# antoyang/TubeDETR

Hardware: AMD Instinct MI355X
Metric: training clips/sec (fwd+bwd) at T=100 k=4 res=352, 1/2/4/8 MI355X (higher is better)
Workload: dtype bf16

## Files before the change

include/tubedetr_hip.h:

```cpp
#ifndef TUBEDETR_HIP_H
#define TUBEDETR_HIP_H
#include <stddef.h>
#include <stdint.h>
#ifdef __cplusplus
extern "C" {
#endif

#define TD_F32 0
#define TD_BF16 1
#define TD_U8 2
#define TD_OK 0
#define TD_ERR_INVALID (-1)
#define TD_ERR_LAUNCH (-2)

typedef void* td_stream_t;

const char* td_last_error(void);
int td_abi_version(void);

int td_set_deterministic(int on);
int td_get_deterministic(void);


#define TD_PROF_GEMM_128x128 0
#define TD_PROF_GEMM_128x64 1
#define TD_PROF_WGRAD 2
#define TD_PROF_GEMM_64x128 3
#define TD_PROF_PW_RESIDENT 4
#define TD_PROF_GEMM_256 5
#define TD_PROF_GEMM_256_PW 6
#define TD_PROF_FUSED 7
#define TD_PROF_CROSS_Q1 8
#define TD_PROF_WGRAD_SINGLE 9
#define TD_PROF_CHAIN 10
#define TD_PROF_FAMILIES 11
int td_prof_enable(int on);
int td_prof_collect(int family, int dtype, long long* launches, double* ms, double* flops);
int td_prof_collect_bytes(int family, int dtype, double* bytes);
int td_prof_dump(const char* path);
int td_debug_set_stamp_buffer(unsigned long long* buf);

typedef struct td_conv_desc {
  int N, Hs, Ws, C;
  int Ho, Wo;
  int R, S, stride, pad;
  int mode;
  int Nc;
  int ldc;
  int out_sp;
  int out_H, out_W;
  int aniso;
  int stride_w, pad_w;
} td_conv_desc;

typedef struct td_epilogue {
  const float* bias;
  const void* residual;
  const void* mask_src;
  int relu;
  int sigmoid;
  float dropout_p;
  uint32_t dropout_seed;
  float alpha;
  const uint32_t* dropout_counter;
} td_epilogue;

int td_conv_gemm(const void* src, const void* wmat, void* out, const td_conv_desc* d, const td_epilogue* e,
                 int dtype, td_stream_t stream);

typedef struct td_linear_ex_desc {
  int M, N, K1, K2;
  int lda1, lda2, ldc, ldr;
  int w_shared;
  long long rows1, rows2;
  const int* a1_map;
  const int* a2_map;
  const int* out_map;
  const int* res_map;
} td_linear_ex_desc;
int td_linear_ex(const void* a1, const void* a2, const void* wmat, void* out, const td_linear_ex_desc* x, const td_epilogue* e,
                 int dtype, td_stream_t stream);

int td_conv_wgrad(const void* g, const void* src, float* dw, const td_conv_desc* d, int ldg, int dtype, int splits,
                  td_stream_t stream);
int td_conv_wgrad_bias(const void* g, const void* src, float* dw, float* dbias, const td_conv_desc* d, int ldg, int dtype,
                       int splits, td_stream_t stream);

typedef struct td_wgrad_job {
  const void* g;
  const void* src;
  float* dW;
  const float* scale;
  td_conv_desc d;
  int ldg;
  int ci_real;
  float* dbias;
  int accumulate;
  int prezeroed;
} td_wgrad_job;
size_t td_conv_wgrad_batch_table_bytes(int n_jobs);
int td_conv_wgrad_batch(const td_wgrad_job* jobs, int n_jobs, int dtype, void* table_host, void* table_dev, size_t table_bytes,
                        td_stream_t stream);

typedef struct td_frame_source {
  const void* data;
  int dtype;
  int n;
  const int* index;
  const int* valid_hw;
} td_frame_source;
int td_frames_to_nhwc(const td_frame_source* srcs, int n_srcs, int C, int H, int W, int Cpad, const float* mean,
                      const float* inv_std, void* y, int dtype, td_stream_t stream);

size_t td_resnet_fwd_ws_bytes(int N, int H, int W, const int* nblocks, int dtype, int save);
int td_resnet_num_convs(const int* nblocks);
int td_resnet_fwd(const td_frame_source* srcs, int n_srcs, const float* mean, const float* inv_std, int N, int H, int W,
                  const int* nblocks, const void* const* w_fwd, const float* const* bias, int save, void* ws, size_t ws_bytes,
                  void** feat, int* feat_hw, int stem_pairs, int first_train_stage, int dtype, td_stream_t stream);
int td_bottleneck_fused(const void* x, void* out, const void* w1, const float* b1, const void* w2, const float* b2, const void* w3,
                        const float* b3, const void* wd, const float* bd, int N, int H, int W, int Cin, int dtype, td_stream_t stream);
int td_pw_chain2(const void* y2, const void* w3, const float* b3, const void* residual, void* out, const void* w1, const float* b1,
                 void* h1, int M, int planes, int dtype, td_stream_t stream);
int td_stem_pair_weights(const void* w_fwd_8, void* w_pairs, int Co, int dtype, td_stream_t stream);
int td_stem_pool(const void* x_pairs, const void* w_pairs, const float* bias, void* pooled, int N, int H, int W, int dtype,
                 td_stream_t stream);
size_t td_resnet_bwd_ws_bytes(int N, int H, int W, const int* nblocks, int first_train_stage, int dtype);
size_t td_resnet_bwd_table_bytes(const int* nblocks, int first_train_stage);
int td_resnet_bwd(const void* dfeat, int N, int N_fwd, int H, int W, const int* nblocks, int first_train_stage,
                  const void* const* w_dgrad, const float* const* scale, float* const* dW, const void* fwd_ws, void* ws,
                  size_t ws_bytes, void* table_host, void* table_dev, size_t table_bytes, int dW_prezeroed, int dtype, int only_stage, td_stream_t stream);

int td_weight_prep(const float* W, const float* bn_w, const float* bn_b, const float* bn_rm, const float* bn_rv,
                   const float* bias, int Co, int Ci, int R, int S, int Cpad, void* w_fwd, void* w_dgrad,
                   float* bias_out, float* scale_out, int dtype, td_stream_t stream);

typedef struct td_prep_item {
  const float* W;
  const float *bn_w, *bn_b, *bn_rm, *bn_rv, *bias;
  void *w_fwd, *w_dgrad;
  float *bias_out, *scale_out;
  int Co, Ci, RS, Cpad, Co_alloc, blk0;
} td_prep_item;
int td_weight_prep_batch(const td_prep_item* items_dev, int n, int total_blocks, int dtype, td_stream_t stream);

int td_wgrad_finalize(const float* dw_k, const float* scale, float* dW, int Co, int Ci, int R, int S, int Cpad,
                      int accumulate, td_stream_t stream);

int td_nchw_to_nhwc(const float* x, void* y, int N, int C, int H, int W, int Cpad, int dtype, td_stream_t stream);
int td_nhwc_to_nchw(const void* x, float* y, int N, int C, int H, int W, int dtype, td_stream_t stream);
int td_cast(const void* x, void* y, size_t n, int src_dtype, int dst_dtype, td_stream_t stream);

int td_maxpool3x3s2(const void* x, void* y, int N, int H, int W, int C, int dtype, td_stream_t stream);

int td_add_layernorm_fwd(const void* x, const void* r, const float* gamma, const float* beta, void* y, void* s_out,
                         float* mean, float* rstd, int rows, int cols, float eps, int dtype, td_stream_t stream);
int td_add_layernorm_bwd(const void* dy, const void* s, const float* mean, const float* rstd, const float* gamma,
                         const void* extra, void* ds, float* dgamma, float* dbeta, int rows, int cols, int dtype,
                         td_stream_t stream);

int td_colsum(const void* g, float* out, int rows, int cols, int ld, int dtype, td_stream_t stream);
int td_add(const void* a, const void* b, void* y, size_t n, int dtype, td_stream_t stream);

int td_relu_bwd(const void* dy, const void* y, void* g, size_t n, float scale, int dtype, td_stream_t stream);

int td_gelu_fwd(const void* x, void* y, size_t n, int dtype, td_stream_t stream);
int td_gelu_bwd(const void* dy, const void* x, void* dx, size_t n, int dtype, td_stream_t stream);

int td_dropout(const void* x, void* y, size_t n, float p, uint32_t seed, const uint32_t* dropout_counter, int dtype,
               td_stream_t stream);

int td_pos_sine(const uint8_t* mask, void* pos, int N, int h, int w, int npf, float temperature, int rows_per_image, int dtype,
                td_stream_t stream);

int td_rows_copy(const void* src, const int* src_map, const void* add, void* dst, const int* dst_map, int n_rows, int cols, int ld_src,
                 int ld_add, int ld_dst, int dtype, td_stream_t stream);
int td_rows_segment_sum(const void* in, const int* idx, const int* ptr, void* out, const int* out_map, int n_out, int cols, int ld_in,
                        int ld_out, int dtype, td_stream_t stream);

int td_mha_fwd(const void* q, const void* k, const void* v, const uint8_t* key_pad, void* out, float* probs,
               float* wavg, int B, int H, int Lq, int Lk, int hd, int ldq, int ldk, int ldv, int ldo, float scale,
               float dropout_p, uint32_t dropout_seed, const uint32_t* dropout_counter, int dtype, td_stream_t stream);
int td_mha_bwd(const void* q, const void* k, const void* v, const void* dout, const float* probs, const float* dwavg,
               void* dq, void* dk, void* dv, float* ds_ws, int B, int H, int Lq, int Lk, int hd, int ldq, int ldk,
               int ldv, int ldo, float scale, float dropout_p, uint32_t dropout_seed, const uint32_t* dropout_counter,
               int dtype, td_stream_t stream);

int td_cross_q1_fwd(const void* u, const void* mem, const void* pos, const uint8_t* key_pad, float* probs, float* wavg, void* zext,
                    int F, int S, int H, int E, int ldz, float dropout_p, uint32_t dropout_seed, const uint32_t* dropout_counter,
                    int dtype, td_stream_t stream);
int td_cross_q1_bwd(const void* u, const void* mem, const void* pos, const float* probs, const void* d_zext, const float* dwavg,
                    void* d_u, float* d_mem, int accumulate, int F, int S, int H, int E, int ldz, float dropout_p, uint32_t dropout_seed,
                    const uint32_t* dropout_counter, int dtype, td_stream_t stream);
int td_cross_q1_bwd_coef(const void* u, const void* mem, const void* pos, const float* probs, const void* d_zext, const float* dwavg,
                         void* d_u, void* coef, int coef_ld, int coef_col, int F, int S, int H, int E, int ldz, float dropout_p,
                         uint32_t dropout_seed, const uint32_t* dropout_counter, int dtype, td_stream_t stream);
int td_cross_q1_dmem(const void* coef, int coef_ld, const void* const* u, const void* const* d_zext, int n_layers, void* d_mem, int F, int S,
                     int H, int E, int ldz, int dtype, td_stream_t stream);
int td_head_blocks_expand(const float* W, const float* bias, float alpha, void* w_n, void* w_t, int E, int H, int dtype, td_stream_t stream);
int td_head_blocks_extract(const float* G, float alpha, float* dW, float* db, int E, int H, td_stream_t stream);

size_t td_mha_lean_stats_bytes(int B, int H, int Lq);
int td_mha_lean_fwd(const void* q, const void* k, const void* v, const uint8_t* key_pad, void* out, float* stats, int B, int H,
                    int Lq, int Lk, int hd, int ldq, int ldk, int ldv, int ldo, float scale, float dropout_p,
                    uint32_t dropout_seed, const uint32_t* dropout_counter, int dtype, td_stream_t stream);
int td_mha_lean_bwd(const void* q, const void* k, const void* v, const uint8_t* key_pad, const void* out, const void* dout,
                    float* stats, void* dq, void* dk, void* dv, int B, int H, int Lq, int Lk, int hd, int ldq, int ldk, int ldv,
                    int ldo, float scale, float dropout_p, uint32_t dropout_seed, const uint32_t* dropout_counter, int dtype,
                    td_stream_t stream);


// ... 47 lines not shown
```

tubedetr_amd/_hip.py:

```python
from __future__ import annotations

import ctypes as C
import os

import torch

TD_F32, TD_BF16 = 0, 1
EXPECTED_ABI = 11
_LIB_PATH = os.environ.get("TD_HIP_LIB") or os.path.join(os.path.dirname(os.path.abspath(__file__)), "lib", "libtubedetr_hip.so")
_lib = None


class ConvDesc(C.Structure):
    _fields_ = [(n, C.c_int) for n in ("N", "Hs", "Ws", "C", "Ho", "Wo", "R", "S", "stride", "pad", "mode", "Nc", "ldc", "out_sp", "out_H", "out_W",
                                       "aniso", "stride_w", "pad_w")]


class PrepItem(C.Structure):
    _fields_ = [(n, C.c_void_p) for n in ("W", "bn_w", "bn_b", "bn_rm", "bn_rv", "bias", "w_fwd", "w_dgrad", "bias_out", "scale_out")] + \
               [(n, C.c_int) for n in ("Co", "Ci", "RS", "Cpad", "Co_alloc", "blk0")]


class WgradJob(C.Structure):
    _fields_ = [("g", C.c_void_p), ("src", C.c_void_p), ("dW", C.c_void_p), ("scale", C.c_void_p), ("d", ConvDesc), ("ldg", C.c_int), ("ci_real", C.c_int), ("dbias", C.c_void_p), ("accumulate", C.c_int), ("prezeroed", C.c_int)]


TD_U8 = 2


class FrameSource(C.Structure):
    _fields_ = [("data", C.c_void_p), ("dtype", C.c_int), ("n", C.c_int), ("index", C.c_void_p), ("valid_hw", C.c_void_p)]


class LinearExDesc(C.Structure):
    _fields_ = [(n, C.c_int) for n in ("M", "N", "K1", "K2", "lda1", "lda2", "ldc", "ldr", "w_shared")] + \
               [("rows1", C.c_longlong), ("rows2", C.c_longlong)] + [(n, C.c_void_p) for n in ("a1_map", "a2_map", "out_map", "res_map")]


class OptimSegment(C.Structure):
    _fields_ = [("begin", C.c_longlong), ("end", C.c_longlong), ("group", C.c_int), ("active", C.c_int)]


class ResampleJob(C.Structure):
    _fields_ = [("src", C.c_void_p), ("src_frame_stride", C.c_longlong)] + [(n, C.c_int) for n in ("src_pitch", "T", "sh", "sw", "flip", "rh", "rw", "wy", "wx", "wh", "ww")] + \
               [("dst", C.c_void_p)] + [(n, C.c_int) for n in ("planar", "frame_off", "H", "W")] + [("mask", C.c_void_p)]


class Epilogue(C.Structure):
    _fields_ = [
        ("bias", C.c_void_p),
        ("residual", C.c_void_p),
        ("mask_src", C.c_void_p),
        ("relu", C.c_int),
        ("sigmoid", C.c_int),
        ("dropout_p", C.c_float),
        ("dropout_seed", C.c_uint32),
        ("alpha", C.c_float),
        ("dropout_counter", C.c_void_p),
    ]


_P, _I, _F, _U32, _SZ = C.c_void_p, C.c_int, C.c_float, C.c_uint32, C.c_size_t
_SIGS = {
    "td_prof_enable": [_I],
    "td_prof_dump": [C.c_char_p],
    "td_debug_set_stamp_buffer": [_P],
    "td_prof_collect": [_I, _I, C.POINTER(C.c_longlong), C.POINTER(C.c_double), C.POINTER(C.c_double)],
    "td_prof_collect_bytes": [_I, _I, C.POINTER(C.c_double)],
    "td_conv_gemm": [_P, _P, _P, C.POINTER(ConvDesc), C.POINTER(Epilogue), _I, _P],
    "td_conv_wgrad": [_P, _P, _P, C.POINTER(ConvDesc), _I, _I, _I, _P],
    "td_conv_wgrad_bias": [_P, _P, _P, _P, C.POINTER(ConvDesc), _I, _I, _I, _P],
    "td_conv_wgrad_batch": [C.POINTER(WgradJob), _I, _I, _P, _P, _SZ, _P],
    "td_resnet_num_convs": [C.POINTER(C.c_int)],
    "td_resnet_fwd": [C.POINTER(FrameSource), _I, C.POINTER(C.c_float), C.POINTER(C.c_float), _I, _I, _I, C.POINTER(C.c_int), C.POINTER(_P), C.POINTER(_P), _I, _P, _SZ,
                      C.POINTER(_P), C.POINTER(C.c_int), _I, _I, _I, _P],
    "td_bottleneck_fused": [_P, _P, _P, _P, _P, _P, _P, _P, _P, _P, _I, _I, _I, _I, _I, _P],
    "td_stem_pair_weights": [_P, _P, _I, _I, _P],
    "td_stem_pool": [_P, _P, _P, _P, _I, _I, _I, _I, _P],
    "td_pw_chain2": [_P, _P, _P, _P, _P, _P, _P, _P, _I, _I, _I, _P],
    "td_set_deterministic": [_I],
    "td_get_deterministic": [],
    "td_frames_to_nhwc": [C.POINTER(FrameSource), _I, _I, _I, _I, _I, C.POINTER(C.c_float), C.POINTER(C.c_float), _P, _I, _P],
    "td_resnet_bwd": [_P, _I, _I, _I, _I, C.POINTER(C.c_int), _I, C.POINTER(_P), C.POINTER(_P), C.POINTER(_P), _P, _P, _SZ, _P, _P, _SZ, _I, _I, _I, _P],
    "td_weight_prep_batch": [_P, _I, _I, _I, _P],
    "td_weight_prep": [_P, _P, _P, _P, _P, _P, _I, _I, _I, _I, _I, _P, _P, _P, _P, _I, _P],
    "td_wgrad_finalize": [_P, _P, _P, _I, _I, _I, _I, _I, _I, _P],
    "td_nchw_to_nhwc": [_P, _P, _I, _I, _I, _I, _I, _I, _P],
    "td_nhwc_to_nchw": [_P, _P, _I, _I, _I, _I, _I, _P],
    "td_cast": [_P, _P, _SZ, _I, _I, _P],
    "td_maxpool3x3s2": [_P, _P, _I, _I, _I, _I, _I, _P],
    "td_add_layernorm_fwd": [_P, _P, _P, _P, _P, _P, _P, _P, _I, _I, _F, _I, _P],
    "td_add_layernorm_bwd": [_P, _P, _P, _P, _P, _P, _P, _P, _P, _I, _I, _I, _P],
    "td_colsum": [_P, _P, _I, _I, _I, _I, _P],
    "td_add": [_P, _P, _P, _SZ, _I, _P],
    "td_relu_bwd": [_P, _P, _P, _SZ, _F, _I, _P],
    "td_gelu_fwd": [_P, _P, _SZ, _I, _P],
    "td_gelu_bwd": [_P, _P, _P, _SZ, _I, _P],
    "td_dropout": [_P, _P, _SZ, _F, _U32, _P, _I, _P],
    "td_pos_sine": [_P, _P, _I, _I, _I, _I, _F, _I, _I, _P],
    "td_linear_ex": [_P, _P, _P, _P, C.POINTER(LinearExDesc), C.POINTER(Epilogue), _I, _P],
    "td_rows_copy": [_P, _P, _P, _P, _P, _I, _I, _I, _I, _I, _I, _P],
    "td_rows_segment_sum": [_P, _P, _P, _P, _P, _I, _I, _I, _I, _I, _P],
    "td_criterion_fwd": [_P, _P, _P, _P, _P, _P, _P, _P, _P, _F, _F, _I, _I, _I, _I, _P, _P, _P, _P, _P, _P],
    "td_criterion_bwd": [_P, _P, _P, _P, _P, _P, _P, _P, _I, _I, _I, _P],
    "td_sted_decode": [_P, _P, _I, _I, _P],
    "td_grad_norm_clip": [_P, _SZ, C.POINTER(OptimSegment), _I, _F, _P, _SZ, _P, _P, _P],
    "td_adamw_ema_step": [_P, _P, _P, _P, _P, _SZ, C.POINTER(OptimSegment), _I, _P, _P, _P, _F, _F, _F, _F, _F, _P],
    "td_mha_fwd": [_P, _P, _P, _P, _P, _P, _P, _I, _I, _I, _I, _I, _I, _I, _I, _I, _F, _F, _U32, _P, _I, _P],
    "td_mha_bwd": [_P, _P, _P, _P, _P, _P, _P, _P, _P, _P, _I, _I, _I, _I, _I, _I, _I, _I, _I, _F, _F, _U32, _P, _I, _P],
    "td_cross_q1_fwd": [_P, _P, _P, _P, _P, _P, _P, _I, _I, _I, _I, _I, _F, _U32, _P, _I, _P],
    "td_cross_q1_bwd": [_P, _P, _P, _P, _P, _P, _P, _P, _I, _I, _I, _I, _I, _I, _F, _U32, _P, _I, _P],
    "td_cross_q1_bwd_coef": [_P, _P, _P, _P, _P, _P, _P, _P, _I, _I, _I, _I, _I, _I, _I, _F, _U32, _P, _I, _P],
    "td_cross_q1_dmem": [_P, _I, _P, _P, _I, _P, _I, _I, _I, _I, _I, _I, _P],
    "td_head_blocks_expand": [_P, _P, _F, _P, _P, _I, _I, _I, _P],
    "td_head_blocks_extract": [_P, _F, _P, _P, _I, _I, _P],
    "td_mha_lean_fwd": [_P, _P, _P, _P, _P, _P, _I, _I, _I, _I, _I, _I, _I, _I, _I, _F, _F, _U32, _P, _I, _P],
    "td_mha_lean_bwd": [_P, _P, _P, _P, _P, _P, _P, _P, _P, _P, _I, _I, _I, _I, _I, _I, _I, _I, _I, _F, _F, _U32, _P, _I, _P],
    "td_clip_resample": [C.POINTER(ResampleJob), _I, _P, _P, _SZ, _P],
}
_SIZE_SIGS = {
    "td_grad_norm_ws_bytes": [],
    "td_mha_lean_stats_bytes": [_I, _I, _I],
    "td_conv_wgrad_batch_table_bytes": [_I],
    "td_clip_resample_table_bytes": [_I],
    "td_resnet_bwd_table_bytes": [C.POINTER(C.c_int), _I],
    "td_resnet_fwd_ws_bytes": [_I, _I, _I, C.POINTER(C.c_int), _I, _I],
    "td_resnet_bwd_ws_bytes": [_I, _I, _I, C.POINTER(C.c_int), _I, _I],
}
EXPORTS = ["td_last_error", "td_abi_version"] + list(_SIGS) + list(_SIZE_SIGS)


def lib_path() -> str:
    return _LIB_PATH


def lib() -> C.CDLL:
    global _lib
    if _lib is None:
        if not os.path.exists(_LIB_PATH):
            raise RuntimeError(
                f"{_LIB_PATH} is missing: build it with `python -m tubedetr_amd.build` (or __graft_entry__.build()); "
                "tubedetr_amd has no CPU / eager fallback"
            )
        L = C.CDLL(_LIB_PATH)
        L.td_last_error.restype = C.c_char_p
        L.td_last_error.argtypes = []
        L.td_abi_version.restype = C.c_int
        L.td_abi_version.argtypes = []
        got = L.td_abi_version()
        if got != EXPECTED_ABI:
            raise RuntimeError(f"{_LIB_PATH} has ABI version {got}, this binding needs {EXPECTED_ABI}: rebuild it with "
                               "`python -m tubedetr_amd.build --force`")
        for name, sig in _SIGS.items():
            fn = getattr(L, name)
            fn.restype = C.c_int
            fn.argtypes = sig
        for name, sig in _SIZE_SIGS.items():
            fn = getattr(L, name)
            fn.restype = C.c_size_t
            fn.argtypes = sig
        _lib = L
    return _lib


def check(rc: int, what: str = ""):
    if rc != 0:
        raise RuntimeError(f"libtubedetr_hip {what} failed ({rc}): {lib().td_last_error().decode()}")


def stream_ptr() -> int:
    return torch._C._cuda_getCurrentRawStream(torch._C._cuda_getDevice())


def dtype_code(dt: torch.dtype) -> int:
    if dt == torch.float32:
        return TD_F32
    if dt == torch.bfloat16:
        return TD_BF16
    raise TypeError(f"unsupported compute dtype {dt}")


def ptr(t) -> int:
    if t is None:
        return None
    assert t.is_cuda, "tubedetr_amd kernels only run on the GPU"
    return t.data_ptr()
```

tubedetr_amd/csrc/api.cpp:

```cpp
#include <stdarg.h>

#include <atomic>
#include <mutex>
#include <vector>

#include "td_common.h"

namespace td {

static thread_local char g_err[512] = "";

void set_error(const char* fmt, ...) {
  va_list ap;
  va_start(ap, fmt);
  vsnprintf(g_err, sizeof(g_err), fmt, ap);
  va_end(ap);
}

int check_launch(const char* what) {
  hipError_t e = hipGetLastError();
  if (e != hipSuccess) {
    set_error("%s: launch failed: %s", what, hipGetErrorString(e));
    return TD_ERR_LAUNCH;
  }
// ... 48 lines not shown
  return TD_OK;
}
extern "C" int td_get_deterministic(void) { return td::deterministic() ? 1 : 0; }

extern "C" int td_prof_enable(int on) {
  std::lock_guard<std::mutex> lk(td::g_prof_mu);
  td::g_prof.store(on != 0);
  if (on) {
    for (auto& r : td::g_recs) { td::g_pool.push_back(r.a); td::g_pool.push_back(r.b); }
    td::g_recs.clear();
  }
  return TD_OK;
}
extern "C" int td_prof_collect(int family, int dtype, long long* launches, double* ms, double* flops) {
  long long n = 0; double t = 0, f = 0;
  std::lock_guard<std::mutex> lk(td::g_prof_mu);
  for (auto& r : td::g_recs) {
    if (r.family != family || r.dtype != dtype) continue;
    if (hipEventSynchronize(r.b) != hipSuccess) { td::set_error("td_prof_collect: event sync failed"); return TD_ERR_LAUNCH; }
    float e = 0.f;
    hipEventElapsedTime(&e, r.a, r.b);
    n++; t += e; f += r.flops;
  }
  if (launches) *launches = n;
  if (ms) *ms = t;
  if (flops) *flops = f;
  return TD_OK;
}

extern "C" int td_prof_collect_bytes(int family, int dtype, double* bytes) {
  double b = 0;
  std::lock_guard<std::mutex> lk(td::g_prof_mu);
  for (auto& r : td::g_recs)
    if (r.family == family && r.dtype == dtype) b += r.bytes;
  if (bytes) *bytes = b;
  return TD_OK;
}

extern "C" int td_prof_dump(const char* path) {
  FILE* f = fopen(path, "w");
  if (!f) { td::set_error("td_prof_dump: cannot open %s", path); return TD_ERR_INVALID; }
  fprintf(f, "family,dtype,M,N,K,R,stride,mode,ms\n");
  std::lock_guard<std::mutex> lk(td::g_prof_mu);
  for (auto& r : td::g_recs) {
    hipEventSynchronize(r.b);
    float e = 0.f;
    hipEventElapsedTime(&e, r.a, r.b);
    fprintf(f, "%d,%d,%d,%d,%d,%d,%d,%d,%.5f\n", r.family, r.dtype, r.M, r.N, r.K, r.R, r.stride, r.mode, e);
  }
  fclose(f);
  return TD_OK;
}

extern "C" const char* td_last_error(void) { return td::g_err; }
extern "C" int td_abi_version(void) { return 11; }
```

tubedetr_amd/csrc/elementwise.hip:

```cpp
#include "td_common.h"

namespace td {

template <typename T>
__global__ void maxpool3x3s2_kernel(const T* x, T* y, int N, int H, int W, int C, int Ho, int Wo) {
  constexpr int VEC = 16 / sizeof(T);
  const int cv = C / VEC;
  const size_t n = (size_t)N * Ho * Wo * cv;
  const size_t idx = (size_t)blockIdx.x * blockDim.x + threadIdx.x;
  if (idx >= n) return;
  int c = (idx % cv) * VEC;
  size_t t = idx / cv;
  int wo = t % Wo; t /= Wo;
  int ho = t % Ho;
  int img = t / Ho;
  float m[VEC];
#pragma unroll
  for (int i = 0; i < VEC; ++i) m[i] = -INFINITY;
  for (int r = 0; r < 3; ++r) {
    int h = ho * 2 - 1 + r;
    if ((unsigned)h >= (unsigned)H) continue;
    for (int s = 0; s < 3; ++s) {
      int w = wo * 2 - 1 + s;
      if ((unsigned)w >= (unsigned)W) continue;
// ... 69 lines not shown
}
static bool aligned8(const void* a, const void* b, const void* c, const void* d) {
  return (((uintptr_t)a | (uintptr_t)b | (uintptr_t)c | (uintptr_t)d) & 7) == 0;
}

template <int NJ>
__global__ __launch_bounds__(256) void add_layernorm_fwd_v4_kernel(const u16* __restrict__ x, const u16* __restrict__ r, const float* __restrict__ gamma,
                                                                   const float* __restrict__ beta, u16* __restrict__ y, u16* __restrict__ s_out,
                                                                   float* __restrict__ mean, float* __restrict__ rstd, int rows, float eps) {
  constexpr int cols = NJ * 256;
  const int lane = threadIdx.x & 63;
  const int row = blockIdx.x * 4 + (threadIdx.x >> 6);
  if (row >= rows) return;
  const size_t base = (size_t)row * cols + lane * 4;
  float v[NJ][4];
  float sum = 0.f;
#pragma unroll
  for (int j = 0; j < NJ; ++j) {
    unpack4v(*(const uint2*)(x + base + 256 * j), v[j]);
    if (r) {
      float a[4];
      unpack4v(*(const uint2*)(r + base + 256 * j), a);
#pragma unroll
      for (int e = 0; e < 4; ++e) v[j][e] += a[e];
    }
#pragma unroll
    for (int e = 0; e < 4; ++e) sum += v[j][e];
  }
  const float mu = wave_sum(sum) * (1.f / cols);
  float var = 0.f;
#pragma unroll
  for (int j = 0; j < NJ; ++j)
#pragma unroll
    for (int e = 0; e < 4; ++e) {
      const float d = v[j][e] - mu;
      var += d * d;
    }
  var = wave_sum(var) * (1.f / cols);
  const float rs = rsqrtf(var + eps);
  if (lane == 0) {
    if (mean) mean[row] = mu;
    if (rstd) rstd[row] = rs;
  }
#pragma unroll
  for (int j = 0; j < NJ; ++j) {
    const float4 gm = *(const float4*)(gamma + lane * 4 + 256 * j), bt = *(const float4*)(beta + lane * 4 + 256 * j);
    if (s_out) *(uint2*)(s_out + base + 256 * j) = pack4_bf16(v[j]);
    float o[4] = {(v[j][0] - mu) * rs * gm.x + bt.x, (v[j][1] - mu) * rs * gm.y + bt.y, (v[j][2] - mu) * rs * gm.z + bt.z,
                  (v[j][3] - mu) * rs * gm.w + bt.w};
    *(uint2*)(y + base + 256 * j) = pack4_bf16(o);
  }
}

template <int NJ>
__global__ __launch_bounds__(256) void add_layernorm_bwd_v4_kernel(const u16* __restrict__ dy, const u16* __restrict__ s, const float* __restrict__ mean,
                                                                   const float* __restrict__ rstd, const float* __restrict__ gamma,
                                                                   const u16* __restrict__ extra, u16* __restrict__ ds, float* dgamma, float* dbeta,
                                                                   int rows) {
  constexpr int cols = NJ * 256;
  const int lane = threadIdx.x & 63;
  const int wid = blockIdx.x * 4 + (threadIdx.x >> 6);
  const int nw = gridDim.x * 4;
  float pg[NJ][4], pb[NJ][4], gm[NJ][4];
#pragma unroll
  for (int j = 0; j < NJ; ++j) {
    const float4 g4 = *(const float4*)(gamma + lane * 4 + 256 * j);
    gm[j][0] = g4.x; gm[j][1] = g4.y; gm[j][2] = g4.z; gm[j][3] = g4.w;
#pragma unroll
    for (int e = 0; e < 4; ++e) pg[j][e] = pb[j][e] = 0.f;
  }
  for (int row = wid; row < rows; row += nw) {
    const size_t base = (size_t)row * cols + lane * 4;
    const float mu = mean[row], rs = rstd[row];
    float xh[NJ][4], dg[NJ][4];
    float c1 = 0.f, c2 = 0.f;
#pragma unroll
    for (int j = 0; j < NJ; ++j) {
      float d[4], sv[4];
      unpack4v(*(const uint2*)(dy + base + 256 * j), d);
      unpack4v(*(const uint2*)(s + base + 256 * j), sv);
#pragma unroll
      for (int e = 0; e < 4; ++e) {
        xh[j][e] = (sv[e] - mu) * rs;
        dg[j][e] = d[e] * gm[j][e];
        c1 += dg[j][e];
        c2 += dg[j][e] * xh[j][e];
        pg[j][e] += d[e] * xh[j][e];
        pb[j][e] += d[e];
      }
    }
    c1 = wave_sum(c1) * (1.f / cols);
    c2 = wave_sum(c2) * (1.f / cols);
#pragma unroll
    for (int j = 0; j < NJ; ++j) {
      float o[4];
#pragma unroll
      for (int e = 0; e < 4; ++e) o[e] = rs * (dg[j][e] - c1 - xh[j][e] * c2);
      if (extra) {
        float ex[4];
        unpack4v(*(const uint2*)(extra + base + 256 * j), ex);
#pragma unroll
        for (int e = 0; e < 4; ++e) o[e] += ex[e];
      }
      *(uint2*)(ds + base + 256 * j) = pack4_bf16(o);
    }
  }
  __shared__ float redg[4][cols], redb[4][cols];
  const int wv = threadIdx.x >> 6;
#pragma unroll
  for (int j = 0; j < NJ; ++j)
#pragma unroll
    for (int e = 0; e < 4; ++e) {
      redg[wv][lane * 4 + 256 * j + e] = pg[j][e];
      redb[wv][lane * 4 + 256 * j + e] = pb[j][e];
    }
  __syncthreads();
  for (int c = threadIdx.x; c < cols; c += 256) {
    if (dgamma) atomicAdd(dgamma + c, redg[0][c] + redg[1][c] + redg[2][c] + redg[3][c]);
    if (dbeta) atomicAdd(dbeta + c, redb[0][c] + redb[1][c] + redb[2][c] + redb[3][c]);
  }
}

template <typename T>
__global__ __launch_bounds__(256) void add_layernorm_bwd_kernel(const T* dy, const T* s, const float* mean, const float* rstd,
                                                                const float* gamma, const T* extra, T* ds, float* dgamma,
                                                                float* dbeta, int rows, int cols) {
  const int lane = threadIdx.x & 63;
  const int wid = blockIdx.x * 4 + (threadIdx.x >> 6);
  const int nw = gridDim.x * 4;
  const int nj = (cols + 63) / 64;
  float pg[LN_MAXJ], pb[LN_MAXJ];
#pragma unroll
  for (int j = 0; j < LN_MAXJ; ++j) pg[j] = pb[j] = 0.f;
  for (int row = wid; row < rows; row += nw) {
    const size_t base = (size_t)row * cols;
    const float mu = mean[row], rs = rstd[row];
    float xh[LN_MAXJ], dg[LN_MAXJ];
    float c1 = 0.f, c2 = 0.f;
#pragma unroll
    for (int j = 0; j < LN_MAXJ; ++j) {
      xh[j] = dg[j] = 0.f;
      int c = lane + 64 * j;
      if (j < nj && c < cols) {
        float d = Elem<T>::load(dy, base + c);
        xh[j] = (Elem<T>::load(s, base + c) - mu) * rs;
        dg[j] = d * gamma[c];
        c1 += dg[j];
        c2 += dg[j] * xh[j];
        pg[j] += d * xh[j];
        pb[j] += d;
      }
    }
    c1 = wave_sum(c1) / cols;
    c2 = wave_sum(c2) / cols;
#pragma unroll
    for (int j = 0; j < LN_MAXJ; ++j) {
      int c = lane + 64 * j;
// ... 226 lines not shown
      o.z = (uint32_t)f32_to_bf16(acc[4 % EPL]) | ((uint32_t)f32_to_bf16(acc[5 % EPL]) << 16);
      o.w = (uint32_t)f32_to_bf16(acc[6 % EPL]) | ((uint32_t)f32_to_bf16(acc[7 % EPL]) << 16);
    } else {
      o = make_uint4(__float_as_uint(acc[0]), __float_as_uint(acc[1]), __float_as_uint(acc[2]), __float_as_uint(acc[3]));
    }
    *(uint4*)(out + ((size_t)(out_map ? out_map[r] : r) * ld_out + (size_t)c * EPL) * sizeof(T)) = o;
  }
}

}
using namespace td;

static inline unsigned nblk(size_t n, int bs = 256) { return (unsigned)((n + bs - 1) / bs); }
#define TD_DISPATCH(dtype, CALL_BF16, CALL_F32, who)  \
  if (dtype == TD_BF16) { CALL_BF16; }                \
  else if (dtype == TD_F32) { CALL_F32; }             \
  else TD_REQUIRE(false, who ": bad dtype")

extern "C" int td_maxpool3x3s2(const void* x, void* y, int N, int H, int W, int C, int dtype, td_stream_t stream) {
  TD_REQUIRE(x && y, "td_maxpool3x3s2: null pointer");
  const int vec = dtype == TD_BF16 ? 8 : 4;
  TD_REQUIRE(C % vec == 0, "td_maxpool3x3s2: C must be a multiple of %d", vec);
  const int Ho = (H + 2 - 3) / 2 + 1, Wo = (W + 2 - 3) / 2 + 1;
  size_t n = (size_t)N * Ho * Wo * (C / vec);
  hipStream_t st = (hipStream_t)stream;
  TD_DISPATCH(dtype, (maxpool3x3s2_kernel<u16><<<nblk(n), 256, 0, st>>>((const u16*)x, (u16*)y, N, H, W, C, Ho, Wo)),
              (maxpool3x3s2_kernel<float><<<nblk(n), 256, 0, st>>>((const float*)x, (float*)y, N, H, W, C, Ho, Wo)),
              "td_maxpool3x3s2");
  return check_launch("td_maxpool3x3s2");
}

extern "C" int td_add_layernorm_fwd(const void* x, const void* r, const float* gamma, const float* beta, void* y,
                                    void* s_out, float* mean, float* rstd, int rows, int cols, float eps, int dtype,
                                    td_stream_t stream) {
  TD_REQUIRE(x && gamma && beta && y, "td_add_layernorm_fwd: null pointer");
  TD_REQUIRE(cols <= 64 * LN_MAXJ, "td_add_layernorm_fwd: cols > %d", 64 * LN_MAXJ);
  if (rows == 0) return TD_OK;
  hipStream_t st = (hipStream_t)stream;
  unsigned g = (rows + 3) / 4;
  if (dtype == TD_BF16 && (cols == 256 || cols == 768) && aligned8(x, r, y, s_out)) {
    if (cols == 256) add_layernorm_fwd_v4_kernel<1><<<g, 256, 0, st>>>((const u16*)x, (const u16*)r, gamma, beta, (u16*)y, (u16*)s_out, mean, rstd, rows, eps);
    else add_layernorm_fwd_v4_kernel<3><<<g, 256, 0, st>>>((const u16*)x, (const u16*)r, gamma, beta, (u16*)y, (u16*)s_out, mean, rstd, rows, eps);
    return check_launch("td_add_layernorm_fwd");
  }
  TD_DISPATCH(dtype,
              (add_layernorm_fwd_kernel<u16><<<g, 256, 0, st>>>((const u16*)x, (const u16*)r, gamma, beta, (u16*)y, (u16*)s_out, mean, rstd, rows, cols, eps)),
              (add_layernorm_fwd_kernel<float><<<g, 256, 0, st>>>((const float*)x, (const float*)r, gamma, beta, (float*)y, (float*)s_out, mean, rstd, rows, cols, eps)),
              "td_add_layernorm_fwd");
  return check_launch("td_add_layernorm_fwd");
}

extern "C" int td_add_layernorm_bwd(const void* dy, const void* s, const float* mean, const float* rstd,
                                    const float* gamma, const void* extra, void* ds, float* dgamma, float* dbeta,
                                    int rows, int cols, int dtype, td_stream_t stream) {
  TD_REQUIRE(dy && s && mean && rstd && gamma && ds, "td_add_layernorm_bwd: null pointer");
  TD_REQUIRE(cols <= 64 * LN_MAXJ, "td_add_layernorm_bwd: cols > %d", 64 * LN_MAXJ);
  if (rows == 0) return TD_OK;
  hipStream_t st = (hipStream_t)stream;
  unsigned g = (rows + 3) / 4;
  if (dtype == TD_BF16 && (cols == 256 || cols == 768) && aligned8(dy, s, ds, extra)) {
    unsigned gv = (rows + 31) / 32;
    if (gv > 1024) gv = 1024;
    if (deterministic()) gv = 1;
    if (cols == 256) add_layernorm_bwd_v4_kernel<1><<<gv, 256, 0, st>>>((const u16*)dy, (const u16*)s, mean, rstd, gamma, (const u16*)extra, (u16*)ds, dgamma, dbeta, rows);
    else add_layernorm_bwd_v4_kernel<3><<<gv, 256, 0, st>>>((const u16*)dy, (const u16*)s, mean, rstd, gamma, (const u16*)extra, (u16*)ds, dgamma, dbeta, rows);
    return check_launch("td_add_layernorm_bwd");
  }
  if (g > 256) g = 256;
  if (deterministic()) g = 1;
  TD_DISPATCH(dtype,
              (add_layernorm_bwd_kernel<u16><<<g, 256, 0, st>>>((const u16*)dy, (const u16*)s, mean, rstd, gamma, (const u16*)extra, (u16*)ds, dgamma, dbeta, rows, cols)),
              (add_layernorm_bwd_kernel<float><<<g, 256, 0, st>>>((const float*)dy, (const float*)s, mean, rstd, gamma, (const float*)extra, (float*)ds, dgamma, dbeta, rows, cols)),
              "td_add_layernorm_bwd");
  return check_launch("td_add_layernorm_bwd");
}

extern "C" int td_colsum(const void* g, float* out, int rows, int cols, int ld, int dtype, td_stream_t stream) {
  TD_REQUIRE(g && out, "td_colsum: null pointer");
  if (rows == 0 || cols == 0) return TD_OK;
  hipStream_t st = (hipStream_t)stream;
  const int vec = dtype == TD_BF16 ? 8 : 4;
  if (cols % vec == 0 && ld % vec == 0) {
    const int gx = (cols + 32 * vec - 1) / (32 * vec);
    int rpb = (int)(((long long)rows * gx + 511) / 512);
    if (rpb < 64) rpb = 64;
    if (deterministic()) rpb = rows;
    dim3 grid(gx, (rows + rpb - 1) / rpb);
    TD_DISPATCH(dtype, (colsum_vec_kernel<u16><<<grid, 256, 0, st>>>((const u16*)g, out, rows, cols, ld, rpb)),
                (colsum_vec_kernel<float><<<grid, 256, 0, st>>>((const float*)g, out, rows, cols, ld, rpb)), "td_colsum");
    return check_launch("td_colsum");
  }
  int rpb = (int)(((long long)rows * ((cols + 255) / 256) + 1023) / 1024);
  if (rpb < 8) rpb = 8;
  if (deterministic()) rpb = rows;
  dim3 grid((cols + 255) / 256, (rows + rpb - 1) / rpb);
  TD_DISPATCH(dtype, (colsum_kernel<u16><<<grid, 256, 0, st>>>((const u16*)g, out, rows, cols, ld, rpb)),
              (colsum_kernel<float><<<grid, 256, 0, st>>>((const float*)g, out, rows, cols, ld, rpb)), "td_colsum");
  return check_launch("td_colsum");
}

extern "C" int td_add(const void* a, const void* b, void* y, size_t n, int dtype, td_stream_t stream) {
  TD_REQUIRE(a && y, "td_add: null pointer");
  if (n == 0) return TD_OK;
  hipStream_t st = (hipStream_t)stream;
  unsigned g = nblk(n / 4 + 1);
  if (g > 4096) g = 4096;
  TD_REQUIRE(((uintptr_t)a | (uintptr_t)y | (uintptr_t)b) % 16 == 0, "td_add: pointers must be 16-byte aligned");
  TD_DISPATCH(dtype, (ew_kernel<u16, 0><<<g, 256, 0, st>>>((const u16*)a, (const u16*)b, (u16*)y, n, 1.f, 0, 0, nullptr)),
              (ew_kernel<float, 0><<<g, 256, 0, st>>>((const float*)a, (const float*)b, (float*)y, n, 1.f, 0, 0, nullptr)), "td_add");
  return check_launch("td_add");
}

extern "C" int td_relu_bwd(const void* dy, const void* y, void* g, size_t n, float scale, int dtype, td_stream_t stream) {
  TD_REQUIRE(dy && y && g, "td_relu_bwd: null pointer");
  if (n == 0) return TD_OK;
  hipStream_t st = (hipStream_t)stream;
// ... 100 lines not shown
```

tubedetr_amd/csrc/gemm_conv.hip:

```cpp
#include <stdlib.h>

#include <type_traits>

#include "td_common.h"
#include <algorithm>
#include <vector>

#ifndef TD_WGRAD_EARLY_ISSUE
#define TD_WGRAD_EARLY_ISSUE 1
#endif
#ifndef TD_BIG_XCD_CONTIG
#define TD_BIG_XCD_CONTIG 1
#endif
namespace td {

struct GemmParams {
  const char* src;
  const char* w;
  char* out;
  td_conv_desc d;
  int M, K;
  uint32_t src_bytes, w_bytes;
  unsigned long long* dbg;
  const float* bias;
  const char* residual;
  const char* mask_src;
  int relu, sigmoid;
  float alpha;
  uint32_t drop_thresh;
  float drop_scale;
  uint32_t seed;
  const uint32_t* seed_dev;
  const char* src2;
  uint32_t src2_bytes;
  int K1, lda1, lda2, ldr;
  int w_shared;
  const int* a1_map;
  const int* a2_map;
  const int* out_map;
  const int* res_map;
  int tap_inner;
  int w_ld;
  int wtap[4];
  int use_wtap;
};

template <typename T>
struct Mfma;
template <>
struct Mfma<u16> {
  static __device__ __forceinline__ void run(const uint4& wf, const uint4& af, f32x4& acc) {
    acc = __builtin_amdgcn_mfma_f32_16x16x32_bf16(*(const bf16x8*)&wf, *(const bf16x8*)&af, acc, 0, 0, 0);
  }
};
template <>
struct Mfma<float> {
  static __device__ __forceinline__ void run(const uint4& wf, const uint4& af, f32x4& acc) {
    const float* a = (const float*)&wf;
    const float* b = (const float*)&af;
#pragma unroll
    for (int s = 0; s < 4; ++s) acc = __builtin_amdgcn_mfma_f32_16x16x4f32(a[s], b[s], acc, 0, 0, 0);
  }
};

template <typename T>
__device__ __forceinline__ void load4(const char* base, size_t off, float (&o)[4]);
template <>
__device__ __forceinline__ void load4<float>(const char* base, size_t off, float (&o)[4]) {
  float4 v = *(const float4*)(base + off * 4);
  o[0] = v.x; o[1] = v.y; o[2] = v.z; o[3] = v.w;
}
template <>
__device__ __forceinline__ void load4<u16>(const char* base, size_t off, float (&o)[4]) {
  uint2 v = *(const uint2*)(base + off * 2);
  o[0] = __uint_as_float(v.x << 16); o[1] = __uint_as_float(v.x & 0xffff0000u);
  o[2] = __uint_as_float(v.y << 16); o[3] = __uint_as_float(v.y & 0xffff0000u);
}
template <typename T, typename V>
__device__ __forceinline__ void unpack4(const V& v, float (&o)[4]);
template <>
__device__ __forceinline__ void unpack4<float, float4>(const float4& v, float (&o)[4]) {
  o[0] = v.x; o[1] = v.y; o[2] = v.z; o[3] = v.w;
}
template <>
__device__ __forceinline__ void unpack4<u16, uint2>(const uint2& v, float (&o)[4]) {
  o[0] = __uint_as_float(v.x << 16); o[1] = __uint_as_float(v.x & 0xffff0000u);
  o[2] = __uint_as_float(v.y << 16); o[3] = __uint_as_float(v.y & 0xffff0000u);
}
typedef __bf16 bf16x2_t __attribute__((ext_vector_type(2)));
__device__ __forceinline__ uint32_t pack_bf16x2(float lo, float hi) {
  bf16x2_t v = {(__bf16)lo, (__bf16)hi};
  return *(uint32_t*)&v;
}
template <typename T>
// ... 224 lines not shown
        while (kc >= d.C) {
          kc -= d.C;
          if (++ks_ == d.S) { ks_ = 0; ++kr; }
        }
      }
    }
  };

  const int wy = wave >> 1, wx = wave & 1;
  const int lr = lane & 15, lg = lane >> 4;

  f32x4 acc[TN][TM];
#pragma unroll
  for (int i = 0; i < TN; ++i)
#pragma unroll
    for (int j = 0; j < TM; ++j) acc[i][j] = f32x4{0.f, 0.f, 0.f, 0.f};

  auto compute_tile = [&](const char* stage) {
    const char* stA = stage;
    const char* stB = stage + BM * 128;
#pragma unroll
    for (int ks = 0; ks < 2; ++ks) {
      const int cidx = ks * 4 + lg;
      uint4 af[TM], wf[TN];
#pragma unroll
      for (int j = 0; j < TM; ++j) {
        int row = wy * WM + j * 16 + lr;
        af[j] = *(const uint4*)(stA + row * 128 + ((cidx ^ (row & 7)) << 4));
      }
#pragma unroll
      for (int i = 0; i < TN; ++i) {
        int row = wx * WN + i * 16 + lr;
        wf[i] = *(const uint4*)(stB + row * 128 + ((cidx ^ (row & 7)) << 4));
      }
#pragma unroll
      for (int i = 0; i < TN; ++i)
#pragma unroll
        for (int j = 0; j < TM; ++j) Mfma<T>::run(wf[i], af[j], acc[i][j]);
    }
  };

  constexpr int CPRW = WN / 4;
  constexpr int EPL = 16 / ES;
  constexpr int LPR = WN / EPL;
  constexpr int RPI = 64 / LPR;
  constexpr int NIT = WM / RPI;
  static_assert(2 * WM * WN * 4 <= (BM + BN) * 128, "staging region does not fit the stage buffer");
  const int cc = lane % LPR, rsub = lane / LPR;
  const int n = n0 + wx * WN + cc * EPL;
  const bool vec_ok = ((d.ldc % EPL) == 0) && (!GX || (p.ldr % EPL) == 0) && (n + EPL - 1 < d.Nc);
  size_t offs[NIT];
  size_t roffs[GX ? NIT : 1];
  bool live[NIT];
  uint4 res[NIT], msk[NIT];
  auto fetch_epilogue_operands = [&]() {
#pragma unroll
    for (int it = 0; it < NIT; ++it) {
      const int m = m0 + wy * WM + it * RPI + rsub;
      live[it] = (m < p.M) && (n < d.Nc);
      size_t orow = live[it] ? m : 0;
      if (!PW && d.out_sp > 1) {
        int ni = (int)orow / HoWo;
        int rem = (int)orow - ni * HoWo;
        int ho = rem / d.Wo, wo = rem - ho * d.Wo;
        orow = ((size_t)ni * d.out_H + (size_t)ho * d.out_sp) * d.out_W + (size_t)wo * d.out_sp;
      }
      if constexpr (GX) {
        const size_t mm = orow;
        if (p.out_map) orow = (size_t)p.out_map[mm];
        roffs[it] = (p.res_map ? (size_t)p.res_map[mm] : orow) * (size_t)p.ldr + n;
      }
      offs[it] = orow * d.ldc + n;
      if (vec_ok && live[it]) {
        if (p.residual) res[it] = ld16(p.residual + (GX ? roffs[it] : offs[it]) * ES);
        if (p.mask_src) msk[it] = ld16(p.mask_src + offs[it] * ES);
      }
    }
  };

  const int nk = (p.K + BK - 1) / BK;
#define TD_STAMP(i) do { if (p.dbg && t == 0) p.dbg[(size_t)blockIdx.x * 8 + (i)] = __builtin_readcyclecounter(); } while (0)
  TD_STAMP(0);
  if constexpr (NST == 2) {
    issue_tile(smem0);
    for (int kt = 0; kt < nk; kt += 2) {
      __syncthreads();
      if (kt == 0) TD_STAMP(1);
      if (kt + 1 < nk) issue_tile(smem1);
      compute_tile(smem0);
      if (kt + 1 >= nk) break;
      __syncthreads();
      if (kt + 2 < nk) issue_tile(smem0);
      compute_tile(smem1);
    }
    TD_STAMP(2);
    fetch_epilogue_operands();
  } else {
#define TD_CG_STEP(cur, nxt, j)                                                     \
  asm volatile("s_waitcnt vmcnt(%0)" ::"n"(AI + BI) : "memory");                    \
  __builtin_amdgcn_s_barrier();                                                     \
  issue_tile(nxt);                                                                  \
  if ((j) >= 0) compute_tile(cur);
    for (int it = -2; it < nk; it += 3) {
      TD_CG_STEP(smem1, smem0, it)
      if (it + 1 >= nk) break;
      TD_CG_STEP(smem2, smem1, it + 1)
      if (it + 2 >= nk) break;
      TD_CG_STEP(smem0, smem2, it + 2)
    }
#undef TD_CG_STEP
    asm volatile("s_waitcnt vmcnt(0)" ::: "memory");
    TD_STAMP(2);
    fetch_epilogue_operands();
  }

  asm volatile("s_waitcnt lgkmcnt(0)" ::: "memory");
  __builtin_amdgcn_s_barrier();
  TD_STAMP(3);
  float* stg = (float*)((wave < 2 ? smem0 : smem1) + (wave & 1) * (WM * WN * 4));
  const float alpha = p.alpha;
#pragma unroll
  for (int j = 0; j < TM; ++j) {
    const int row = j * 16 + lr;
#pragma unroll
    for (int i = 0; i < TN; ++i) {
      const int c = (i * 4 + lg) ^ (row & (CPRW - 1));
      f32x4 a = acc[i][j];
      *(float4*)(stg + row * WN + c * 4) = make_float4(a[0] * alpha, a[1] * alpha, a[2] * alpha, a[3] * alpha);
    }
  }
  asm volatile("s_waitcnt lgkmcnt(0)" ::: "memory");
  float bias[EPL];
#pragma unroll
  for (int r = 0; r < EPL; ++r) bias[r] = (p.bias && n + r < d.Nc) ? p.bias[n + r] : 0.f;
  TD_STAMP(4);
  const uint32_t eff_seed = effective_seed(p.seed, p.drop_thresh ? p.seed_dev : nullptr);
#pragma unroll
  for (int it = 0; it < NIT; ++it) {
    if (!live[it]) continue;
    const int row = it * RPI + rsub;
    const int sw = row & (CPRW - 1);
    float v[EPL];
#pragma unroll
    for (int q = 0; q < EPL / 4; ++q) {
      float4 f = *(const float4*)(stg + row * WN + (((cc * (EPL / 4) + q) ^ sw) * 4));
      v[4 * q + 0] = f.x + bias[4 * q + 0]; v[4 * q + 1] = f.y + bias[4 * q + 1];
      v[4 * q + 2] = f.z + bias[4 * q + 2]; v[4 * q + 3] = f.w + bias[4 * q + 3];
    }
    const size_t off = offs[it];
    if (vec_ok) {
      if (p.residual) {
        float r8[EPL];
        unpack16<T>(res[it], r8);
#pragma unroll
        for (int r = 0; r < EPL; ++r) v[r] += r8[r];
      }
      if (p.relu) {
#pragma unroll
        for (int r = 0; r < EPL; ++r) v[r] = fmaxf(v[r], 0.f);
      }
      if (p.sigmoid) {
#pragma unroll
        for (int r = 0; r < EPL; ++r) v[r] = sigmoidf_(v[r]);
      }
      if (p.mask_src) {
        float m8[EPL];
        unpack16<T>(msk[it], m8);
#pragma unroll
        for (int r = 0; r < EPL; ++r) v[r] = m8[r] > 0.f ? v[r] : 0.f;
      }
      if (p.drop_thresh) {
#pragma unroll
        for (int r = 0; r < EPL; ++r) v[r] = dropout_keep(eff_seed, (uint32_t)(off + r), p.drop_thresh) ? v[r] * p.drop_scale : 0.f;
      }
      st16(p.out + off * ES, pack16<T>(v));
    } else {
      const int cnt = min(EPL, d.Nc - n);
      for (int r = 0; r < cnt; ++r) {
        float x = v[r];
        if (p.residual) x += Elem<T>::load(p.residual, (GX ? roffs[it] : off) + r);
        if (p.relu) x = fmaxf(x, 0.f);
        if (p.sigmoid) x = sigmoidf_(x);
        if (p.mask_src) x = Elem<T>::load(p.mask_src, off + r) > 0.f ? x : 0.f;
        if (p.drop_thresh) x = dropout_keep(eff_seed, (uint32_t)(off + r), p.drop_thresh) ? x * p.drop_scale : 0.f;
        Elem<T>::store(p.out, off + r, x);
      }
    }
  }
  TD_STAMP(5);
#undef TD_STAMP
}

#ifndef TD_ABL
#define TD_ABL 0
#endif
template <int OFF>
__device__ __forceinline__ u32x4_t lds_read16(uint32_t addr) {
  u32x4_t r;
#if TD_ABL & 4
  asm volatile("" : "=v"(r) : "v"(addr));
#else
  asm volatile("ds_read_b128 %0, %1 offset:%2" : "=v"(r) : "v"(addr), "n"(OFF));
#endif
  return r;
}
template <int N>
__device__ __forceinline__ void wait_vmcnt() {
  asm volatile("s_waitcnt vmcnt(%0)" ::"n"(N) : "memory");
}
template <int I>
using ic = std::integral_constant<int, I>;

#ifndef TD_BIG8_AUX_W
#define TD_BIG8_AUX_W 0
#endif
#ifndef TD_BIG8_AUX_X
#define TD_BIG8_AUX_X 0
#endif
template <bool TU, bool RES>
__global__ __launch_bounds__(512, 1) void conv_gemm_big8_kernel(GemmParams p) {
  using T = u16;
  constexpr int ES = 2, BM = 256, BN = 256, BK = 64, NW = 8, VEC = 8;
  constexpr int WM = 128, WN = 64, TM = 8, TN = 4;
  constexpr int STAGE = (BM + BN) * 128, WREG = BM * 128;
  constexpr uint32_t OOB = 0xFFFFFFF0u;
  constexpr int MAXT = 160;
  constexpr int STG = 16 * WN * ES;
  __shared__ __attribute__((aligned(16))) char smem[2 * STAGE];
  __shared__ __attribute__((aligned(16))) uint4 ktab[MAXT];
  __shared__ __attribute__((aligned(16))) char stg_all[NW * STG];

  const td_conv_desc& d = p.d;
  const int t = threadIdx.x;
  const int wave = __builtin_amdgcn_readfirstlane(t >> 6), lane = t & 63;
  const int NT = d.Nc / BN;
  const int lrow = lane >> 3;
  const int chunk = (lane & 7) ^ lrow;
  const int HoWo = d.Ho * d.Wo;
  const __amdgpu_buffer_rsrc_t rs_src = __builtin_amdgcn_make_buffer_rsrc((void*)p.src, 0, p.src_bytes, 0x00020000);
  const __amdgpu_buffer_rsrc_t rs_w = __builtin_amdgcn_make_buffer_rsrc((void*)p.w, 0, p.w_bytes, 0x00020000);
  const uint32_t out_bytes = (uint32_t)p.M * (uint32_t)d.ldc * ES;
  const __amdgpu_buffer_rsrc_t rs_out = __builtin_amdgcn_make_buffer_rsrc((void*)p.out, 0, out_bytes, 0x00020000);
  const int wy = wave >> 2, wx = wave & 3;
  const int RS = d.R * d.S;
  const int lane_c = chunk * VEC;
  const int nk = p.K / BK;
  const bool tap_inner = TU && p.tap_inner;
  if (t < nk + 4) {
    uint32_t xo, tap = 0, wo;
    if constexpr (TU) {
      const int cpt = d.C / BK;
      const int chunkc = tap_inner ? t / RS : t % cpt;
      tap = tap_inner ? t - chunkc * RS : t / cpt;
      const int r = (int)tap / d.S, sx = (int)tap - r * d.S;
      const int pix = d.mode == 0 ? r * d.Ws + sx : -(r * d.Ws + sx);
      xo = (uint32_t)(pix * d.C + chunkc * BK) * ES;
      wo = (uint32_t)((int)tap * d.C + chunkc * BK) * ES;
    } else {
      xo = wo = (uint32_t)t * BK * ES;
    }
    ktab[t] = make_uint4(xo, t < nk ? tap : 0u, wo, t < nk ? 0xFFFFFFFFu : 0u);
  }
#if TD_ABL & 16
  for (int i = t; i < 2 * STAGE / 4; i += 512) ((uint32_t*)smem)[i] = 0x3F803F80u ^ (mix32((uint32_t)i * 0x9E3779B1u + blockIdx.x) & 0x007F007Fu);
#endif
  const int nvb = 8 * ((cdiv(p.M, BM) + 7) / 8) * NT;
  const float rcp_howo = 1.f / (float)HoWo, rcp_wo = 1.f / (float)d.Wo;
  auto divmod = [](int a, int dv, float rcp, int& q, int& r) {
    q = (int)((float)a * rcp);
    r = a - q * dv;
    const int up = r >= dv, dn = r < 0;
    q += up - dn;
// ... 93 lines not shown
      wreg[0][2] = lds_read16<2 * 2048>(wa[S][0]); wreg[0][3] = lds_read16<3 * 2048>(wa[S][0]);
    }
    xreg[0][0] = lds_read16<(2 * P + 0) * 2048>(xa[S][0]);
    xreg[1][0] = lds_read16<(2 * P + 1) * 2048>(xa[S][0]);
    if constexpr (P == 0) {
      wreg[1][0] = lds_read16<0 * 2048>(wa[S][1]); wreg[1][1] = lds_read16<1 * 2048>(wa[S][1]);
      wreg[1][2] = lds_read16<2 * 2048>(wa[S][1]); wreg[1][3] = lds_read16<3 * 2048>(wa[S][1]);
    }
    xreg[0][1] = lds_read16<(2 * P + 0) * 2048>(xa[S][1]);
    xreg[1][1] = lds_read16<(2 * P + 1) * 2048>(xa[S][1]);
    if constexpr (P == 0) { ew = lds_read16<0>(taddr); taddr += 16; issue_x(oth, 0, ex); issue_x(oth, 1, ex); wait_vmcnt<8>(); }
    if constexpr (P == 1) { issue_x(oth, 2, ex); issue_x(oth, 3, ex); wait_vmcnt<9>(); }
    if constexpr (P == 2) { issue_w(cur, 0, ew); issue_w(cur, 1, ew); wait_vmcnt<10>(); }
    if constexpr (P == 3) { issue_w(cur, 2, ew); issue_w(cur, 3, ew); wait_vmcnt<7>(); }
    __builtin_amdgcn_s_barrier();
    asm volatile("s_waitcnt lgkmcnt(0)" ::: "memory");
    __builtin_amdgcn_sched_barrier(0);
#if !(TD_ABL & 8)
    __builtin_amdgcn_s_setprio(1);
#endif
#pragma unroll
    for (int ks = 0; ks < 2; ++ks)
#pragma unroll
      for (int j = 0; j < 2; ++j)
#pragma unroll
        for (int i = 0; i < TN; ++i)
          asm volatile("v_mfma_f32_16x16x32_bf16 %0, %1, %2, %0" : "+v"(acc[i][2 * P + j]) : "v"(wreg[ks][i]), "v"(xreg[j][ks]));
#if !(TD_ABL & 8)
    __builtin_amdgcn_s_setprio(0);
#endif
    __builtin_amdgcn_sched_barrier(0);
    __builtin_amdgcn_s_barrier();
  };
  auto prologue_issue = [&]() {
    u32x4_t e0 = lds_read16<0>(tab0);
    ea = lds_read16<16>(tab0);
    asm volatile("s_waitcnt lgkmcnt(0)" : "+v"(e0), "+v"(ea) : : "memory");
    __builtin_amdgcn_sched_barrier(0);
#pragma unroll
    for (int i = 0; i < 4; ++i) issue_w(smem, i, e0);
#pragma unroll
    for (int q = 0; q < 4; ++q) issue_x(smem, q, e0);
#pragma unroll
    for (int i = 0; i < 4; ++i) issue_w(smem + STAGE, i, ea);
  };

  const uint32_t stg0 = (uint32_t)(uintptr_t)(lds_ptr_t)stg_all + (uint32_t)wave * STG;
  uint32_t swa[TN];
#pragma unroll
  for (int i = 0; i < TN; ++i) swa[i] = stg0 + (uint32_t)(lr * 128 + (((2 * i + (lg >> 1)) ^ (lr & 7)) << 4) + (lg & 1) * 8);
  const int cc = lane & 7, rsub = lane >> 3;
  const uint32_t sra = stg0 + (uint32_t)(rsub * 128 + ((cc ^ rsub) << 4));
  const float alpha = p.alpha;

#define TD_STAMP(i) do { if (p.dbg && t == 0) p.dbg[(size_t)vb * 8 + (i)] = __builtin_readcyclecounter(); } while (0)
  int vb = blockIdx.x;
  if (!tile_ok(vb)) return;
  tile_addr(tile_m0(vb), tile_n0(vb));
  asm volatile("s_waitcnt lgkmcnt(0)" ::: "memory");
  __builtin_amdgcn_s_barrier();
  prologue_issue();
#pragma unroll 1
  for (;;) {
    const int m0 = tile_m0(vb), n0 = tile_n0(vb);
    TD_STAMP(0);
    if (p.dbg && t == 0) p.dbg[(size_t)vb * 8 + 6] = wall_clock64();
#pragma unroll
    for (int i = 0; i < TN; ++i)
#pragma unroll
      for (int j = 0; j < TM; ++j) acc[i][j] = f32x4{0.f, 0.f, 0.f, 0.f};
    taddr = tab0 + 2 * 16;
    f32x4 bs[TN];
#pragma unroll
    for (int i = 0; i < TN; ++i) bs[i] = p.bias ? *(const f32x4*)(p.bias + n0 + wx * WN + i * 16 + lg * 4) : f32x4{0.f, 0.f, 0.f, 0.f};
    wait_vmcnt<7>();
    __builtin_amdgcn_s_barrier();
    if (wy == 1) __builtin_amdgcn_s_barrier();
    TD_STAMP(1);
    const int npair = (nk + 1) / 2;
#pragma unroll 1
    for (int it = 0; it < npair; ++it) {
      phase(ic<0>{}, ic<0>{}); phase(ic<0>{}, ic<1>{}); phase(ic<0>{}, ic<2>{}); phase(ic<0>{}, ic<3>{});
      phase(ic<1>{}, ic<0>{}); phase(ic<1>{}, ic<1>{}); phase(ic<1>{}, ic<2>{}); phase(ic<1>{}, ic<3>{});
    }
    if (wy == 0) __builtin_amdgcn_s_barrier();
    TD_STAMP(2);
    asm volatile("s_waitcnt vmcnt(0) lgkmcnt(0)" ::: "memory");
    asm volatile("s_nop 15\n\ts_nop 15" ::: "memory");
#pragma unroll
    for (int i = 0; i < TN; ++i)
#pragma unroll
      for (int j = 0; j < TM; ++j) asm volatile("" : "+v"(acc[i][j]));
#pragma unroll
    for (int i = 0; i < TN; ++i) asm volatile("" : "+v"(bs[i]));
    const int vb_next = vb + (int)gridDim.x;
    const bool more = tile_ok(vb_next);
    if (more) {
      tile_addr(tile_m0(vb_next), tile_n0(vb_next));
      prologue_issue();
    }
    TD_STAMP(3);
    uint4 mk[2][2];
    auto seg_off = [&](int j, int h) -> uint32_t {
      const int m = m0 + wy * WM + j * 16 + h * 8 + rsub;
      return m < p.M ? ((uint32_t)m * (uint32_t)d.ldc + (uint32_t)(n0 + wx * WN + cc * 8)) * ES : OOB;
    };
    auto fetch_mask = [&](int j, int b) {
#pragma unroll
      for (int h = 0; h < 2; ++h) {
        const uint32_t off = seg_off(j, h);
        mk[b][h] = off != OOB ? ld16(p.mask_src + off) : make_uint4(0, 0, 0, 0);
      }
    };
    auto put = [&](int j) {
#pragma unroll
      for (int i = 0; i < TN; ++i) {
        const f32x4 a = acc[i][j];
        float v[4] = {a[0] * alpha + bs[i][0], a[1] * alpha + bs[i][1], a[2] * alpha + bs[i][2], a[3] * alpha + bs[i][3]};
        if constexpr (RES) {
          const int m = m0 + wy * WM + j * 16 + lr;
          if (m < p.M) {
            const uint2 rr = *(const uint2*)(p.residual + ((size_t)m * d.ldc + n0 + wx * WN + i * 16 + lg * 4) * ES);
            v[0] += __uint_as_float(rr.x << 16); v[1] += __uint_as_float(rr.x & 0xffff0000u);
            v[2] += __uint_as_float(rr.y << 16); v[3] += __uint_as_float(rr.y & 0xffff0000u);
          }
        }
        if (p.relu) {
#pragma unroll
          for (int r = 0; r < 4; ++r) v[r] = fmaxf(v[r], 0.f);
        }
        const uint32_t lo = pack_bf16x2(v[0], v[1]), hi = pack_bf16x2(v[2], v[3]);
        asm volatile("ds_write_b64 %0, %1" ::"v"(swa[i]), "v"(u32x2_t{lo, hi}) : "memory");
      }
    };
    if (p.mask_src) fetch_mask(0, 0);
    put(0);
    u32x4_t o0, o1;
    asm volatile("ds_read_b128 %0, %1" : "=v"(o0) : "v"(sra) : "memory");
    asm volatile("ds_read_b128 %0, %1 offset:1024" : "=v"(o1) : "v"(sra) : "memory");
#pragma unroll
    for (int j = 0; j < TM; ++j) {
      const int b = j & 1;
      if (j + 1 < TM) {
        if (p.mask_src) fetch_mask(j + 1, b ^ 1);
        put(j + 1);
        asm volatile("s_waitcnt lgkmcnt(4)" : "+v"(o0), "+v"(o1) : : "memory");
      } else {
        asm volatile("s_waitcnt lgkmcnt(0)" : "+v"(o0), "+v"(o1) : : "memory");
      }
      u32x4_t s0 = o0, s1 = o1;
      if (j + 1 < TM) {
        asm volatile("ds_read_b128 %0, %1" : "=v"(o0) : "v"(sra) : "memory");
        asm volatile("ds_read_b128 %0, %1 offset:1024" : "=v"(o1) : "v"(sra) : "memory");
      }
      if (p.mask_src) {
        float x8[8], m8[8];
        unpack16<T>(make_uint4(s0.x, s0.y, s0.z, s0.w), x8);
        unpack16<T>(mk[b][0], m8);
#pragma unroll
        for (int r = 0; r < 8; ++r) x8[r] = m8[r] > 0.f ? x8[r] : 0.f;
        const uint4 q0 = pack16<T>(x8);
        s0 = u32x4_t{q0.x, q0.y, q0.z, q0.w};
        unpack16<T>(make_uint4(s1.x, s1.y, s1.z, s1.w), x8);
        unpack16<T>(mk[b][1], m8);
#pragma unroll
        for (int r = 0; r < 8; ++r) x8[r] = m8[r] > 0.f ? x8[r] : 0.f;
        const uint4 q1 = pack16<T>(x8);
        s1 = u32x4_t{q1.x, q1.y, q1.z, q1.w};
      }
      __builtin_amdgcn_raw_buffer_store_b128(s0, rs_out, (int)seg_off(j, 0), 0, 0);
      __builtin_amdgcn_raw_buffer_store_b128(s1, rs_out, (int)seg_off(j, 1), 0, 0);
    }
    TD_STAMP(5);
    if (p.dbg && t == 0) p.dbg[(size_t)vb * 8 + 7] = wall_clock64();
    if (!more) break;
    vb = vb_next;
  }
#undef TD_STAMP
}

template <bool TU>
__global__ __launch_bounds__(512, 1) void conv_gemm_big8n_kernel(GemmParams p) {
  using T = u16;
  constexpr int ES = 2, BM = 256, BN = 128, BK = 64, NW = 8, VEC = 8;
  constexpr int WM = 64, WN = 64, TM = 4, TN = 4;
  constexpr int WREG = BM * 128, STAGE = (BM + BN) * 128;
  constexpr uint32_t OOB = 0xFFFFFFF0u;
  constexpr int MAXT = 160;
  __shared__ __attribute__((aligned(16))) char smem[3 * STAGE];
  __shared__ __attribute__((aligned(16))) uint4 ktab[MAXT];

  const td_conv_desc& d = p.d;
  const int t = threadIdx.x;
  const int wave = __builtin_amdgcn_readfirstlane(t >> 6), lane = t & 63;
  const int NT = d.Nc / BN;
  const int xcd = blockIdx.x & 7, seq = blockIdx.x >> 3;
#if TD_BIG_XCD_CONTIG
  const int mtx = (cdiv(p.M, BM) + 7) / 8;
  const int mt = xcd * mtx + seq / NT, nt = seq - (seq / NT) * NT;
#else
  const int mt = (seq / NT) * 8 + xcd, nt = seq - (seq / NT) * NT;
#endif
  const int m0 = mt * BM, n0 = nt * BN;
  if (m0 >= p.M) return;
  const int lrow = lane >> 3;
  const int chunk = (lane & 7) ^ lrow;
  const int lane_c = chunk * VEC;
  const int HoWo = d.Ho * d.Wo;
  const int RS = d.R * d.S;
  const __amdgpu_buffer_rsrc_t rs_src = __builtin_amdgcn_make_buffer_rsrc((void*)p.src, 0, p.src_bytes, 0x00020000);
  const __amdgpu_buffer_rsrc_t rs_w = __builtin_amdgcn_make_buffer_rsrc((void*)p.w, 0, p.w_bytes, 0x00020000);
  const int wy = wave >> 1, wx = wave & 1;
  const int grp = wave >> 2;

  uint32_t a_off[4], a_mask[4];
  const float rcp_howo = 1.f / (float)HoWo, rcp_wo = 1.f / (float)d.Wo;
  auto divmod = [](int a, int dv, float rcp, int& q, int& r) {
    q = (int)((float)a * rcp);
    r = a - q * dv;
    const int up = r >= dv, dn = r < 0;
    q += up - dn;
    r += (dn - up) * dv;
  };
#pragma unroll
  for (int q = 0; q < 4; ++q) {
    const int m = m0 + (wave >> 1) * WM + (q >> 1) * 32 + ((wave & 1) * 2 + (q & 1)) * 8 + lrow;
    const bool ok = m < p.M;
    if constexpr (!TU) {
      a_off[q] = ((uint32_t)m * (uint32_t)p.K + (uint32_t)lane_c) * ES;
      a_mask[q] = ok ? 1u : 0u;
    } else {
      const int mm = ok ? m : 0;
      int n, rem, ho, wo;
      divmod(mm, HoWo, rcp_howo, n, rem);
// ... 52 lines not shown
  for (int s_ = 0; s_ < 3; ++s_) {
    xa[s_][0] = xa0 + s_ * STAGE; xa[s_][1] = (xa0 ^ 64u) + s_ * STAGE;
    wa[s_][0] = wa0 + s_ * STAGE; wa[s_][1] = (wa0 ^ 64u) + s_ * STAGE;
  }
  u32x4_t wreg[2][TN], xreg[2][2];
  const uint32_t tab0 = (uint32_t)(uintptr_t)(lds_ptr_t)ktab;
  uint32_t taddr = tab0 + 3 * 16;
  u32x4_t e[3];
  auto phase = [&](auto S_, auto P_) {
    constexpr int S = decltype(S_)::value, P = decltype(P_)::value, S2 = (S + 2) % 3;
    char* const nxt = smem + S2 * STAGE;
    if constexpr (P == 0) {
      wreg[0][0] = lds_read16<0 * 2048>(wa[S][0]); wreg[0][1] = lds_read16<1 * 2048>(wa[S][0]);
      wreg[0][2] = lds_read16<2 * 2048>(wa[S][0]); wreg[0][3] = lds_read16<3 * 2048>(wa[S][0]);
    }
    xreg[0][0] = lds_read16<(2 * P + 0) * 2048>(xa[S][0]);
    xreg[1][0] = lds_read16<(2 * P + 1) * 2048>(xa[S][0]);
    if constexpr (P == 0) {
      wreg[1][0] = lds_read16<0 * 2048>(wa[S][1]); wreg[1][1] = lds_read16<1 * 2048>(wa[S][1]);
      wreg[1][2] = lds_read16<2 * 2048>(wa[S][1]); wreg[1][3] = lds_read16<3 * 2048>(wa[S][1]);
    }
    xreg[0][1] = lds_read16<(2 * P + 0) * 2048>(xa[S][1]);
    xreg[1][1] = lds_read16<(2 * P + 1) * 2048>(xa[S][1]);
    if constexpr (P == 0) {
      issue_w(nxt, 0, e[S2]); issue_w(nxt, 1, e[S2]); issue_x(nxt, 0, e[S2]); issue_x(nxt, 1, e[S2]);
      wait_vmcnt<10>();
    } else {
      e[S] = lds_read16<0>(taddr);
      taddr += 16;
      issue_x(nxt, 2, e[S2]); issue_x(nxt, 3, e[S2]);
      wait_vmcnt<8>();
    }
    __builtin_amdgcn_s_barrier();
    asm volatile("s_waitcnt lgkmcnt(0)" ::: "memory");
    __builtin_amdgcn_sched_barrier(0);
    __builtin_amdgcn_s_setprio(1);
#pragma unroll
    for (int ks = 0; ks < 2; ++ks)
#pragma unroll
      for (int j = 0; j < 2; ++j)
#pragma unroll
        for (int i = 0; i < TN; ++i)
          asm volatile("v_mfma_f32_16x16x32_bf16 %0, %1, %2, %0" : "+v"(acc[i][2 * P + j]) : "v"(wreg[ks][i]), "v"(xreg[j][ks]));
    __builtin_amdgcn_s_setprio(0);
    __builtin_amdgcn_sched_barrier(0);
    __builtin_amdgcn_s_barrier();
  };

  constexpr int CR = 16, NCH = WM / CR, EPL = 8, LPR = WN / EPL, RPI = 64 / LPR, NIT = CR / RPI, CPRW = WN / 4;
  const int cc = lane % LPR, rsub = lane / LPR;
  const int n = n0 + wx * WN + cc * EPL;
  uint32_t offs[2][NIT];
  bool live[2][NIT];
  uint4 res[2][NIT], msk[2][NIT];
  auto fetch_chunk = [&](int c, int b) {
#pragma unroll
    for (int it = 0; it < NIT; ++it) {
      const int m = m0 + wy * WM + c * CR + it * RPI + rsub;
      live[b][it] = m < p.M;
      offs[b][it] = (uint32_t)min(m, p.M - 1) * (uint32_t)d.ldc + (uint32_t)n;
      if (p.residual) res[b][it] = ld16(p.residual + offs[b][it] * ES);
      if (p.mask_src) msk[b][it] = ld16(p.mask_src + offs[b][it] * ES);
    }
  };

#define TD_STAMP(i) do { if (p.dbg && t == 0) p.dbg[(size_t)blockIdx.x * 8 + (i)] = __builtin_readcyclecounter(); } while (0)
  TD_STAMP(0);
  __syncthreads();
  {
    const u32x4_t e0 = lds_read16<0>(tab0);
    const u32x4_t e1 = lds_read16<16>(tab0);
    e[2] = lds_read16<32>(tab0);
    asm volatile("s_waitcnt lgkmcnt(0)" ::: "memory");
    __builtin_amdgcn_sched_barrier(0);
    issue_w(smem, 0, e0); issue_w(smem, 1, e0); issue_x(smem, 0, e0); issue_x(smem, 1, e0); issue_x(smem, 2, e0); issue_x(smem, 3, e0);
    issue_w(smem + STAGE, 0, e1); issue_w(smem + STAGE, 1, e1); issue_x(smem + STAGE, 0, e1); issue_x(smem + STAGE, 1, e1);
    issue_x(smem + STAGE, 2, e1); issue_x(smem + STAGE, 3, e1);
  }
  wait_vmcnt<8>();
  __builtin_amdgcn_s_barrier();
  if (grp == 1) __builtin_amdgcn_s_barrier();
  TD_STAMP(1);
  const int ntri = (nk + 2) / 3;
#pragma unroll 1
  for (int it = 0; it < ntri; ++it) {
    phase(ic<0>{}, ic<0>{}); phase(ic<0>{}, ic<1>{});
    phase(ic<1>{}, ic<0>{}); phase(ic<1>{}, ic<1>{});
    phase(ic<2>{}, ic<0>{}); phase(ic<2>{}, ic<1>{});
  }
  if (grp == 0) __builtin_amdgcn_s_barrier();
  TD_STAMP(2);
  asm volatile("s_waitcnt vmcnt(0) lgkmcnt(0)" ::: "memory");
  asm volatile("s_nop 15\n\ts_nop 15" ::: "memory");
#pragma unroll
  for (int i = 0; i < TN; ++i)
#pragma unroll
    for (int j = 0; j < TM; ++j) asm volatile("" : "+v"(acc[i][j]));
  fetch_chunk(0, 0);
  __builtin_amdgcn_s_barrier();
  TD_STAMP(3);
  float* stg = (float*)(smem + wave * (CR * WN * 4));
  const float alpha = p.alpha;
  float bias[EPL];
#pragma unroll
  for (int r = 0; r < EPL; ++r) bias[r] = p.bias ? p.bias[n + r] : 0.f;
#pragma unroll
  for (int c = 0; c < NCH; ++c) {
    const int b = c & 1;
    {
      const int row = lr;
#pragma unroll
      for (int i = 0; i < TN; ++i) {
        const int cx = (i * 4 + lg) ^ (row & (CPRW - 1));
        const f32x4 a = acc[i][c];
        *(float4*)(stg + row * WN + cx * 4) = make_float4(a[0] * alpha, a[1] * alpha, a[2] * alpha, a[3] * alpha);
      }
    }
    if (c + 1 < NCH) fetch_chunk(c + 1, b ^ 1);
    asm volatile("s_waitcnt lgkmcnt(0)" ::: "memory");
#pragma unroll
    for (int it = 0; it < NIT; ++it) {
      const int row = it * RPI + rsub;
      const int sw = row & (CPRW - 1);
      float v[EPL];
#pragma unroll
      for (int q = 0; q < EPL / 4; ++q) {
        const float4 f = *(const float4*)(stg + row * WN + (((cc * (EPL / 4) + q) ^ sw) * 4));
        v[4 * q + 0] = f.x + bias[4 * q + 0]; v[4 * q + 1] = f.y + bias[4 * q + 1];
        v[4 * q + 2] = f.z + bias[4 * q + 2]; v[4 * q + 3] = f.w + bias[4 * q + 3];
      }
      if (p.residual) {
        float r8[EPL];
        unpack16<T>(res[b][it], r8);
#pragma unroll
        for (int r = 0; r < EPL; ++r) v[r] += r8[r];
      }
      if (p.relu) {
#pragma unroll
        for (int r = 0; r < EPL; ++r) v[r] = fmaxf(v[r], 0.f);
      }
      if (p.mask_src) {
        float m8[EPL];
        unpack16<T>(msk[b][it], m8);
#pragma unroll
        for (int r = 0; r < EPL; ++r) v[r] = m8[r] > 0.f ? v[r] : 0.f;
      }
      if (live[b][it]) st16(p.out + offs[b][it] * ES, pack16<T>(v));
    }
    asm volatile("s_waitcnt lgkmcnt(0)" ::: "memory");
  }
  TD_STAMP(5);
#undef TD_STAMP
}

template <int NKT, bool RES, bool MSK>
__global__ __launch_bounds__(256, 2) void pw_resident2_kernel(GemmParams p, int MT, int P) {
  using T = u16;
  constexpr int ES = 2;
  constexpr uint32_t OOB = 0xFFFFFFF0u;
  constexpr int WM = 32, WN = 64, TM = 2, TN = 4;
  constexpr int CPRW = WN / 4, EPL = 8, LPR = WN / EPL, RPI = 64 / LPR, NIT = WM / RPI;
  constexpr int NOPS = NIT * ((RES ? 1 : 0) + (MSK ? 1 : 0));
  constexpr bool AHEAD = NOPS > 0 && !(RES && MSK && NKT == 4);
  constexpr int NA = 2 * NKT;
  constexpr int AUX_NT = (TD_NT & 2) ? 2 : 0;
  __shared__ __attribute__((aligned(16))) char sA0[32768];
  __shared__ __attribute__((aligned(16))) char sA1[32768];
  __shared__ __attribute__((aligned(16))) char sT[4 * 16 * WN * 4];
  const td_conv_desc& d = p.d;
  const int t = threadIdx.x;
  const int wave = __builtin_amdgcn_readfirstlane(t >> 6), lane = t & 63;
  const int NT = d.Nc >> 7;
  const int xcd = blockIdx.x & 7, local = blockIdx.x >> 3;
  const int GPX = P / NT;
  const int nt = local % NT, gl = local / NT;
  if (gl >= GPX) return;
  const int gid = xcd * GPX + gl, G = 8 * GPX;
  const int lrow = lane >> 3, chunk = (lane & 7) ^ lrow;
  const uint32_t out_bytes = (uint32_t)p.M * (uint32_t)d.ldc * ES;
  const __amdgpu_buffer_rsrc_t rs_src = __builtin_amdgcn_make_buffer_rsrc((void*)p.src, 0, p.src_bytes, 0x00020000);
  const __amdgpu_buffer_rsrc_t rs_out = __builtin_amdgcn_make_buffer_rsrc((void*)p.out, 0, out_bytes, 0x00020000);
  const __amdgpu_buffer_rsrc_t rs_res = __builtin_amdgcn_make_buffer_rsrc((void*)(RES ? p.residual : p.out), 0, out_bytes, 0x00020000);
  const __amdgpu_buffer_rsrc_t rs_msk = __builtin_amdgcn_make_buffer_rsrc((void*)(MSK ? p.mask_src : p.out), 0, out_bytes, 0x00020000);
  const int n0 = nt * 128;
  const int HoWo = d.Ho * d.Wo;
  const bool strided = d.stride != 1;
  auto issue_A = [&](char* buf, int mt) {
    const int m0 = mt * 64;
    uint32_t row[2];
#pragma unroll
    for (int i = 0; i < 2; ++i) {
      const int m = m0 + (i * 4 + wave) * 8 + lrow;
      int src_row = m;
      if (strided) {
        const int img = m / HoWo, rem = m - img * HoWo;
        const int ho = rem / d.Wo, wo = rem - ho * d.Wo;
        src_row = (img * d.Hs + ho * d.stride) * d.Ws + wo * d.stride;
      }
      row[i] = (mt < MT && m < p.M) ? (uint32_t)src_row * (uint32_t)p.K * ES : OOB;
    }
#pragma unroll
    for (int kt = 0; kt < NKT; ++kt)
#pragma unroll
      for (int i = 0; i < 2; ++i) {
        const uint32_t off = row[i] != OOB ? row[i] + (uint32_t)(kt * 64 + chunk * 8) * ES : OOB;
        __builtin_amdgcn_raw_ptr_buffer_load_lds(rs_src, (lds_ptr_t)(buf + kt * 8192 + (i * 4 + wave) * 1024), 16, off, 0, 0, 0);
      }
  };
  const int wy = wave >> 1, wx = wave & 1;
  const int lr = lane & 15, lg = lane >> 4;
  const int cc = lane % LPR, rsub = lane / LPR;
  const int n = n0 + wx * WN + cc * EPL;
  float bias[EPL];
#pragma unroll
  for (int r = 0; r < EPL; ++r) bias[r] = p.bias ? p.bias[n + r] : 0.f;
  uint4 wfr[NKT][2][TN];
#pragma unroll
  for (int kt = 0; kt < NKT; ++kt)
#pragma unroll
    for (int ks = 0; ks < 2; ++ks)
#pragma unroll
      for (int i = 0; i < TN; ++i)
        wfr[kt][ks][i] = *(const uint4*)(p.w + ((size_t)(n0 + wx * WN + i * 16 + lr) * p.K + kt * 64 + ks * 32 + lg * 8) * ES);
  const uint32_t drop_seed = p.drop_thresh ? effective_seed(p.seed, p.seed_dev) : 0u;
  float* const stg = (float*)(sT + wave * (16 * WN * 4));

  auto seg_off = [&](int mt, int it) -> uint32_t {
    const int m = mt * 64 + wy * WM + it * RPI + rsub;
    return (mt < MT && m < p.M) ? ((uint32_t)m * (uint32_t)d.ldc + (uint32_t)n) * ES : OOB;
  };
  u32x4_t res[2][NIT], msk[2][NIT];
  auto fetch_ops = [&](int mt, int b) {
#pragma unroll
    for (int it = 0; it < NIT; ++it) {
      const uint32_t off = seg_off(mt, it);
      if constexpr (RES) asm volatile("buffer_load_dwordx4 %0, %1, %2, 0 offen nt" : "=v"(res[b][it]) : "v"(off), "s"(rs_res) : "memory");
      if constexpr (MSK) asm volatile("buffer_load_dwordx4 %0, %1, %2, 0 offen nt" : "=v"(msk[b][it]) : "v"(off), "s"(rs_msk) : "memory");
    }
  };

  auto step = [&](char* cur, char* nxt, int mt, auto B_) {
    constexpr int B = decltype(B_)::value;
    if constexpr (NOPS > 0 && !AHEAD) fetch_ops(mt, 0);
    wait_vmcnt<NA + NOPS>();
    __builtin_amdgcn_s_barrier();
    f32x4 acc[TN][TM];
#pragma unroll
    for (int i = 0; i < TN; ++i)
#pragma unroll
      for (int j = 0; j < TM; ++j) acc[i][j] = f32x4{0.f, 0.f, 0.f, 0.f};
#pragma unroll
    for (int kt = 0; kt < NKT; ++kt)
#pragma unroll
      for (int ks = 0; ks < 2; ++ks) {
        const int cidx = ks * 4 + lg;
        uint4 af[TM];
#pragma unroll
        for (int j = 0; j < TM; ++j) {
          const int row = wy * WM + j * 16 + lr;
          af[j] = *(const uint4*)(cur + kt * 8192 + row * 128 + ((cidx ^ (row & 7)) << 4));
        }
#pragma unroll
        for (int i = 0; i < TN; ++i)
#pragma unroll
          for (int j = 0; j < TM; ++j) Mfma<T>::run(wfr[kt][ks][i], af[j], acc[i][j]);
      }
    asm volatile("s_waitcnt lgkmcnt(0)" ::: "memory");
    __builtin_amdgcn_s_barrier();
    issue_A(cur, mt + 2 * G);
    if constexpr (AHEAD) fetch_ops(mt + G, B ^ 1);
    if constexpr (NOPS > 0) {
      wait_vmcnt<NA + (AHEAD ? NOPS : 0)>();
      __builtin_amdgcn_sched_barrier(0);
    }
    constexpr int RB = AHEAD ? B : 0;
#pragma unroll
    for (int j = 0; j < TM; ++j) {
#pragma unroll
      for (int i = 0; i < TN; ++i) {
        const int c = (i * 4 + lg) ^ (lr & (CPRW - 1));
        const f32x4 a = acc[i][j];
        *(float4*)(stg + lr * WN + c * 4) = make_float4(a[0], a[1], a[2], a[3]);
      }
      asm volatile("s_waitcnt lgkmcnt(0)" ::: "memory");
#pragma unroll
      for (int h = 0; h < 16 / RPI; ++h) {
        const int it = j * (16 / RPI) + h;
        const int row = h * RPI + rsub;
        const int sw = row & (CPRW - 1);
        float v[EPL];
#pragma unroll
        for (int q = 0; q < EPL / 4; ++q) {
          const float4 f = *(const float4*)(stg + row * WN + (((cc * (EPL / 4) + q) ^ sw) * 4));
          v[4 * q + 0] = f.x + bias[4 * q + 0]; v[4 * q + 1] = f.y + bias[4 * q + 1];
          v[4 * q + 2] = f.z + bias[4 * q + 2]; v[4 * q + 3] = f.w + bias[4 * q + 3];
        }
        const uint32_t off = seg_off(mt, it);
        if constexpr (RES) {
          float r8[EPL];
          unpack16<T>(make_uint4(res[RB][it].x, res[RB][it].y, res[RB][it].z, res[RB][it].w), r8);
#pragma unroll
          for (int r = 0; r < EPL; ++r) v[r] += r8[r];
        }
        if (p.relu) {
#pragma unroll
          for (int r = 0; r < EPL; ++r) v[r] = fmaxf(v[r], 0.f);
        }
        if constexpr (MSK) {
          float m8[EPL];
          unpack16<T>(make_uint4(msk[RB][it].x, msk[RB][it].y, msk[RB][it].z, msk[RB][it].w), m8);
#pragma unroll
          for (int r = 0; r < EPL; ++r) v[r] = m8[r] > 0.f ? v[r] : 0.f;
        }
        if (p.drop_thresh) {
#pragma unroll
          for (int r = 0; r < EPL; ++r) v[r] = dropout_keep(drop_seed, off / ES + (uint32_t)r, p.drop_thresh) ? v[r] * p.drop_scale : 0.f;
        }
        const uint4 o = pack16<T>(v);
        __builtin_amdgcn_raw_buffer_store_b128(u32x4_t{o.x, o.y, o.z, o.w}, rs_out, (int)off, 0, AUX_NT);
      }
      asm volatile("s_waitcnt lgkmcnt(0)" ::: "memory");
    }
  };

  int mt = gid;
  issue_A(sA0, mt);
  issue_A(sA1, mt + G);
  if constexpr (AHEAD) fetch_ops(mt, 0);
  while (mt < MT) {
    step(sA0, sA1, mt, ic<0>{});
    mt += G;
    if (mt >= MT) break;
    step(sA1, sA0, mt, ic<1>{});
    mt += G;
  }
  asm volatile("s_waitcnt vmcnt(0)" ::: "memory");
}

struct WgradParams {
  const char* g;
  const char* src;
  float* dw;
  const float* scale;
  float* dbias;
  td_conv_desc d;
  int M, K, ldg, mper;
  uint32_t g_bytes, src_bytes;
  int out_mode;
  int ci_real;
  int tn, tk, first;
  int cls;
  unsigned long long* stamps;
};

typedef __bf16 bf16x4 __attribute__((ext_vector_type(4)));

template <int ES>
__device__ __forceinline__ int wg_swz(int row) {
  return ES == 2 ? ((row & 3) | (((row >> 3) & 1) << 2)) : (row & 7);
}

template <typename T, int NSTG, bool PW>
__device__ __forceinline__ void wgrad_body(const WgradParams& p, const int bx, const int by, const int bz, const int lin) {
  constexpr int ES = sizeof(T);
  constexpr int VEC = 16 / ES;
  constexpr int MK = 128 / ES;
  constexpr int ROWB = 128 * ES;
  constexpr int CPR = ROWB / 16;
  constexpr int RPI = 64 / CPR;
  constexpr int LI = MK / (4 * RPI);
  constexpr int SWS = ES == 2 ? 1 : 2;
// ... 725 lines not shown

static int validate(const td_conv_desc* d, int dtype, const char* who) {
  const int vec = dtype == TD_BF16 ? 8 : 4;
  TD_REQUIRE(dtype == TD_F32 || dtype == TD_BF16, "%s: bad dtype %d", who, dtype);
  TD_REQUIRE(d->C % vec == 0, "%s: source channels C=%d must be a multiple of %d (pad them)", who, d->C, vec);
  TD_REQUIRE(d->N > 0 && d->Hs > 0 && d->Ws > 0 && d->Ho > 0 && d->Wo > 0 && d->R > 0 && d->S > 0 && d->stride > 0,
             "%s: bad geometry", who);
  TD_REQUIRE((double)d->N * d->Hs * d->Ws * d->C < 2147483647.0, "%s: source tensor exceeds 2^31 elements", who);
  TD_REQUIRE(!d->aniso || (d->mode == 0 && d->stride_w >= 1 && d->pad_w >= 0 && d->out_sp <= 1), "%s: anisotropic stride / padding is a forward-only geometry", who);
  return TD_OK;
}

}

using namespace td;

static thread_local unsigned long long* g_dbg = nullptr;
static int persist_min_tiles() {
  static const int v = [] { const char* e = getenv("TD_PW_PERSIST_MIN"); return e ? atoi(e) : 4; }();
  return v;
}
extern "C" int td_debug_set_stamp_buffer(unsigned long long* buf) { g_dbg = buf; return TD_OK; }

struct WeightSubset {
  int w_ld;
  int ntap;
  int wtap[4];
  size_t w_bytes;
};
static int conv_gemm_launch(const void* src, const void* wmat, void* out, const td_conv_desc* d, const td_epilogue* e, int dtype,
                            td_stream_t stream, const WeightSubset* sub);

static int conv_dgrad_s2_by_parity(const void* g, const void* w_dgrad, void* dx, const td_conv_desc* d, const td_epilogue* e, int dtype,
                                   td_stream_t stream) {
  const int Hg = d->Hs, Wg = d->Ws, Co = d->C, H = d->Ho, W = d->Wo;
  const size_t es = 2, wbytes = (size_t)d->Nc * 9 * Co * es;
  for (int ph = 0; ph < 2; ++ph)
    for (int pw = 0; pw < 2; ++pw) {
      const int nr = ph ? 2 : 1, ns = pw ? 2 : 1;
      const int rmap[2] = {ph ? 2 : 1, 0}, smap[2] = {pw ? 2 : 1, 0};
      td_conv_desc c = {d->N, Hg, Wg, Co, Hg, Wg, nr, ns, 1, 0, 0, d->Nc, d->ldc, 2, H, W};
      WeightSubset sub;
      memset(&sub, 0, sizeof(sub));
      sub.w_ld = 9 * Co;
      sub.ntap = nr * ns;
      for (int r = 0; r < nr; ++r)
        for (int s_ = 0; s_ < ns; ++s_) sub.wtap[r * ns + s_] = rmap[r] * 3 + smap[s_];
      const size_t ooff = ((size_t)ph * W + pw) * d->ldc * es;
      td_epilogue ec;
      memset(&ec, 0, sizeof(ec));
      if (e) ec = *e;
      if (ec.residual) ec.residual = (const char*)ec.residual + ooff;
      if (ec.mask_src) ec.mask_src = (const char*)ec.mask_src + ooff;
      const char* wp = (const char*)w_dgrad;
      if (sub.ntap == 1) {
        wp += (size_t)sub.wtap[0] * Co * es;
        sub.wtap[0] = 0;
      }
      sub.w_bytes = wbytes - (size_t)(wp - (const char*)w_dgrad);
      const int rc = conv_gemm_launch(g, wp, (char*)dx + ooff, &c, &ec, dtype, stream, &sub);
      if (rc) return rc;
    }
  return TD_OK;
}

extern "C" int td_conv_gemm(const void* src, const void* wmat, void* out, const td_conv_desc* d, const td_epilogue* e,
                            int dtype, td_stream_t stream) {
  TD_REQUIRE(src && wmat && out && d, "td_conv_gemm: null pointer");
  static const int parity = [] { const char* e_ = getenv("TD_DGRAD_S2_PARITY"); return e_ ? atoi(e_) : 1; }();
  if (parity && dtype == TD_BF16 && d->mode == 1 && d->stride == 2 && d->R == 3 && d->S == 3 && d->pad == 1 && !d->aniso && d->out_sp <= 1 &&
      d->Ho == 2 * d->Hs && d->Wo == 2 * d->Ws && d->C % 64 == 0 && d->ldc >= d->Nc && !(e && (e->dropout_p > 0.f || e->sigmoid))) {
    int rc = validate(d, dtype, "td_conv_gemm");
    if (rc) return rc;
    return conv_dgrad_s2_by_parity(src, wmat, out, d, e, dtype, stream);
  }
  return conv_gemm_launch(src, wmat, out, d, e, dtype, stream, nullptr);
}

static int conv_gemm_launch(const void* src, const void* wmat, void* out, const td_conv_desc* d, const td_epilogue* e, int dtype,
                            td_stream_t stream, const WeightSubset* sub) {
  TD_REQUIRE(src && wmat && out && d, "td_conv_gemm: null pointer");
  int rc = validate(d, dtype, "td_conv_gemm");
  if (rc) return rc;
  GemmParams p;
  memset(&p, 0, sizeof(p));
  p.src = (const char*)src;
  p.w = (const char*)wmat;
  p.out = (char*)out;
  p.d = *d;
  if (p.d.out_sp < 1) p.d.out_sp = 1;
  p.M = d->N * d->Ho * d->Wo;
  p.K = d->R * d->S * d->C;
  {
    const double es = dtype == TD_BF16 ? 2.0 : 4.0;
    const double sb = (double)d->N * d->Hs * d->Ws * d->C * es, wb = (double)d->Nc * p.K * es;
    TD_REQUIRE(sb < 4294967000.0 && wb < 4294967000.0, "td_conv_gemm: operand exceeds the 4 GiB buffer-descriptor range");
    p.src_bytes = (uint32_t)sb;
    p.w_bytes = (uint32_t)wb;
  }
  if (sub) {
    p.w_ld = sub->w_ld;
    p.w_bytes = (uint32_t)sub->w_bytes;
    p.use_wtap = sub->ntap > 1;
    for (int i = 0; i < 4; ++i) p.wtap[i] = sub->wtap[i];
  }
  p.alpha = 1.f;
  p.dbg = g_dbg;
  if (e) {
    p.bias = e->bias;
    p.residual = (const char*)e->residual;
    p.mask_src = (const char*)e->mask_src;
    p.relu = e->relu;
    p.sigmoid = e->sigmoid;
    if (e->alpha != 0.f) p.alpha = e->alpha;
    if (e->dropout_p > 0.f) {
      TD_REQUIRE(e->dropout_p < 1.f, "td_conv_gemm: dropout_p must be < 1");
      p.drop_thresh = (uint32_t)((double)e->dropout_p * 4294967296.0);
      if (p.drop_thresh == 0) p.drop_thresh = 1;
      p.drop_scale = 1.f / (1.f - e->dropout_p);
      p.seed = e->dropout_seed;
      p.seed_dev = e->dropout_counter;
    }
  }
  TD_REQUIRE(d->ldc >= d->Nc, "td_conv_gemm: ldc < Nc");
  hipStream_t st = (hipStream_t)stream;
  static const int n_cu = [] {
    int dev = 0, cus = 256;
    if (hipGetDevice(&dev) == hipSuccess) (void)hipDeviceGetAttribute(&cus, hipDeviceAttributeMultiprocessorCount, dev);
    return cus;
  }();
  {
    static const int persist = [] { const char* e_ = getenv("TD_PW_PERSIST"); return e_ ? atoi(e_) : 1; }();
    static const int persist_dropout = [] { const char* e_ = getenv("TD_PW_PERSIST_DROPOUT"); return e_ ? atoi(e_) : 1; }();
    const bool pw0 = d->R == 1 && d->S == 1 && d->pad == 0 && p.d.out_sp == 1 && !d->aniso &&
                     ((d->stride == 1 && d->Hs == d->Ho && d->Ws == d->Wo) ||
                      (d->stride > 1 && d->mode == 0 && (d->Ho - 1) * d->stride < d->Hs && (d->Wo - 1) * d->stride < d->Ws));
    const int NTp = d->Nc / 128, Pp = 2 * n_cu / 8;
    const bool shape_ok = pw0 && !p.w_ld && dtype == TD_BF16 && p.K % 64 == 0 && p.K <= 256 && d->Nc % 128 == 0 &&
                          (NTp == 1 || NTp == 2 || NTp == 4 || NTp == 8 || NTp == 16) && Pp >= NTp && d->ldc % 8 == 0 && !p.sigmoid &&
                          p.alpha == 1.f && n_cu % 8 == 0 && (!p.drop_thresh || persist_dropout) && (double)p.M * d->ldc < 2147483000.0;
    const int MTp = cdiv(p.M, 64);
    const int groups = shape_ok ? 8 * (Pp / NTp) : 1;
    if (persist && shape_ok && MTp >= persist_min_tiles() * groups && !(persist == 2 && p.mask_src) && !(persist == 3 && d->mode != 0)) {
      const bool prof_ = prof_on();
      if (prof_) {
        prof_begin(TD_PROF_PW_RESIDENT, dtype, 2.0 * p.M * d->Nc * p.K, st, p.M, d->Nc, p.K, d->R, d->stride, d->mode);
        const double es_ = 2.0;
        double by = ((double)p.M * p.K + (double)d->Nc * p.K + (double)p.M * d->Nc) * es_;
        if (p.residual) by += (double)p.M * d->Nc * es_;
        if (p.mask_src) by += (double)p.M * d->Nc * es_;
        prof_set_bytes(by);
      }
      const int nkt = p.K / 64;
      const bool hr = p.residual != nullptr, hm = p.mask_src != nullptr;
      dim3 g2(2 * n_cu);
#define TD_PWR(NK)                                                                               \
  do {                                                                                           \
    if (hr && hm) pw_resident2_kernel<NK, true, true><<<g2, 256, 0, st>>>(p, MTp, Pp);          \
    else if (hr) pw_resident2_kernel<NK, true, false><<<g2, 256, 0, st>>>(p, MTp, Pp);          \
    else if (hm) pw_resident2_kernel<NK, false, true><<<g2, 256, 0, st>>>(p, MTp, Pp);          \
    else pw_resident2_kernel<NK, false, false><<<g2, 256, 0, st>>>(p, MTp, Pp);                 \
  } while (0)
      if (nkt == 1) TD_PWR(1);
      else if (nkt == 2) TD_PWR(2);
      else if (nkt == 3) TD_PWR(3);
      else TD_PWR(4);
#undef TD_PWR
      if (prof_) prof_end(st);
      return check_launch("td_conv_gemm(pw_resident)");
    }
  }
  const bool narrow = d->Nc <= 64;
  const int tiles128 = cdiv(p.M, 128) * cdiv(d->Nc, 128);
  const bool small_m = !narrow && (tiles128 < 512 || p.K <= 512);
  const int BMsel = small_m ? 64 : 128, BNsel = narrow ? 64 : 128;
  const int MT = cdiv(p.M, BMsel), NTl = cdiv(d->Nc, BNsel);
  dim3 grid(8 * cdiv(MT, 8) * NTl);
  const bool prof = prof_on();
  const bool pw = d->R == 1 && d->S == 1 && d->stride == 1 && d->pad == 0 && p.d.out_sp == 1 && d->Hs == d->Ho && d->Ws == d->Wo;
  static const int tu_on = [] { const char* e_ = getenv("TD_CONV_TAP_UNIFORM"); return e_ ? atoi(e_) : 1; }();
  const int bk = dtype == TD_BF16 ? 64 : 32;
  const bool tu = (tu_on || p.use_wtap) && !pw && !d->aniso && (d->R * d->S > 1 || (d->stride > 1 && d->mode == 0)) && d->R * d->S <= 32 && d->C % bk == 0 &&
                  (p.d.out_sp == 1 || d->mode == 0) && (d->mode == 0 || d->stride == 1);
  TD_REQUIRE(tu || !p.use_wtap, "td_conv_gemm: a weight-column subset needs the tap-uniform addressing (C %% %d == 0, at most 32 taps)", bk);
  {
    static const int big_on = [] { const char* e_ = getenv("TD_CONV_BIG"); return e_ ? atoi(e_) : 1; }();
    static const int big_min = [] { const char* e_ = getenv("TD_CONV_BIG_MIN_WG"); return e_ ? atoi(e_) : 160; }();
    const int bnb = d->Nc % 256 == 0 ? 256 : 128;
    const int wgs = cdiv(p.M, 256) * (d->Nc / bnb);
    if (big_on && dtype == TD_BF16 && (pw || tu) && p.d.out_sp == 1 && !p.use_wtap && !p.w_ld && d->Nc % 128 == 0 && p.K % 64 == 0 && p.K >= 512 && d->ldc % 8 == 0 && !p.sigmoid &&
        !p.drop_thresh && wgs >= big_min && (double)p.M * d->ldc < 2147483000.0 &&
        p.K <= 64 * 154 && p.M < (1 << 24)) {
      if (prof) {
        prof_begin(tu ? TD_PROF_GEMM_256 : TD_PROF_GEMM_256_PW, dtype, 2.0 * p.M * d->Nc * p.K, st, p.M, d->Nc, p.K, d->R, d->stride, d->mode);
        double by = ((double)d->N * d->Hs * d->Ws * d->C + (double)d->Nc * p.K + (double)p.M * d->Nc) * 2.0;
        if (p.residual) by += (double)p.M * d->Nc * 2.0;
        if (p.mask_src) by += (double)p.M * d->Nc * 2.0;
        prof_set_bytes(by);
      }
      static const int tap_inner = [] { const char* e_ = getenv("TD_CONV_TAP_INNER"); return e_ ? atoi(e_) : 1; }();
      p.tap_inner = tu && tap_inner && d->R * d->S > 1;
      dim3 gb(8 * cdiv(cdiv(p.M, 256), 8) * (d->Nc / bnb));
      static const int persist8 = [] { const char* e_ = getenv("TD_CONV_BIG_PERSIST"); return e_ ? atoi(e_) : 1; }();
      if (bnb == 256) {
        const dim3 gp(persist8 && n_cu % 8 == 0 ? std::min((unsigned)n_cu, gb.x) : gb.x);
        if (tu && p.residual) conv_gemm_big8_kernel<true, true><<<gp, 512, 0, st>>>(p);
        else if (tu) conv_gemm_big8_kernel<true, false><<<gp, 512, 0, st>>>(p);
        else if (p.residual) conv_gemm_big8_kernel<false, true><<<gp, 512, 0, st>>>(p);
        else conv_gemm_big8_kernel<false, false><<<gp, 512, 0, st>>>(p);
      } else {
        if (tu) conv_gemm_big8n_kernel<true><<<gb, 512, 0, st>>>(p);
        else conv_gemm_big8n_kernel<false><<<gb, 512, 0, st>>>(p);
      }
      if (prof) prof_end(st);
      return check_launch("td_conv_gemm(256-row tiles)");
    }
  }
  if (prof) prof_begin(narrow ? TD_PROF_GEMM_128x64 : (small_m ? TD_PROF_GEMM_64x128 : TD_PROF_GEMM_128x128), dtype, 2.0 * p.M * d->Nc * p.K, st, p.M, d->Nc, p.K, d->R, d->stride, d->mode);
  if (prof) {
    const double es = dtype == TD_BF16 ? 2.0 : 4.0;
    const double rows_out = d->out_sp > 1 ? (double)d->N * d->out_H * d->out_W : (double)p.M;
    double by = ((double)d->N * d->Hs * d->Ws * d->C + (double)d->Nc * p.K + (double)p.M * d->Nc) * es;
    if (e && e->residual) by += rows_out * d->Nc * es;
    if (e && e->mask_src) by += rows_out * d->Nc * es;
    prof_set_bytes(by);
  }
#define TD_LAUNCH(TT, BMv, BNv)                                                                   \
  do {                                                                                            \
    if (pw) conv_gemm_kernel<TT, BMv, BNv, 2, true><<<grid, 256, 0, st>>>(p);                    \
    else if (tu) conv_gemm_kernel<TT, BMv, BNv, 2, false, true><<<grid, 256, 0, st>>>(p);        \
    else conv_gemm_kernel<TT, BMv, BNv, 2, false><<<grid, 256, 0, st>>>(p);                      \
  } while (0)
  static const int deep = [] { const char* e_ = getenv("TD_CONV_DEEP"); return e_ ? atoi(e_) : 1; }();
  const bool deep_ok = deep && small_m && (int)grid.x <= 2 * 256 && p.K >= 1024;
  if (dtype == TD_BF16) {
    if (narrow) TD_LAUNCH(u16, 128, 64);
    else if (deep_ok && pw) conv_gemm_kernel<u16, 64, 128, 3, true><<<grid, 256, 0, st>>>(p);
    else if (deep_ok && tu) conv_gemm_kernel<u16, 64, 128, 3, false, true><<<grid, 256, 0, st>>>(p);
    else if (deep_ok) conv_gemm_kernel<u16, 64, 128, 3, false><<<grid, 256, 0, st>>>(p);
    else if (small_m) TD_LAUNCH(u16, 64, 128);
    else TD_LAUNCH(u16, 128, 128);
  } else {
    if (narrow) TD_LAUNCH(float, 128, 64);
    else if (small_m) TD_LAUNCH(float, 64, 128);
    else TD_LAUNCH(float, 128, 128);
  }
#undef TD_LAUNCH
  if (prof) prof_end(st);
  return check_launch("td_conv_gemm");
}

extern "C" int td_linear_ex(const void* a1, const void* a2, const void* wmat, void* out, const td_linear_ex_desc* x, const td_epilogue* e,
                            int dtype, td_stream_t stream) {
  TD_REQUIRE(a1 && wmat && out && x, "td_linear_ex: null pointer");
  TD_REQUIRE(dtype == TD_F32 || dtype == TD_BF16, "td_linear_ex: bad dtype %d", dtype);
  const int vec = dtype == TD_BF16 ? 8 : 4, bk = dtype == TD_BF16 ? 64 : 32;
  const int es = dtype == TD_BF16 ? 2 : 4;
  const int K2 = a2 ? x->K2 : 0;
  TD_REQUIRE(x->M >= 1 && x->N >= 1 && x->K1 >= vec && K2 >= 0, "td_linear_ex: bad sizes");
  TD_REQUIRE(x->K1 % vec == 0 && K2 % vec == 0 && x->lda1 % vec == 0 && (!a2 || x->lda2 % vec == 0), "td_linear_ex: K1 / K2 / lda must be multiples of %d", vec);
  TD_REQUIRE(!a2 || x->K1 % bk == 0, "td_linear_ex: with a second source K1=%d must be a multiple of the K tile (%d)", x->K1, bk);
  TD_REQUIRE(x->lda1 >= x->K1 && (!a2 || x->lda2 >= K2) && x->ldc >= x->N, "td_linear_ex: row stride smaller than the row");
  TD_REQUIRE(x->rows1 >= 1 && (!a2 || x->rows2 >= 1) && (x->a1_map || x->rows1 >= x->M) && (!a2 || x->a2_map || x->rows2 >= x->M),
             "td_linear_ex: source has fewer rows than M and no row map");
  GemmParams p;
  memset(&p, 0, sizeof(p));
  p.src = (const char*)a1;
  p.src2 = (const char*)a2;
  p.w = (const char*)wmat;
  p.out = (char*)out;
  p.M = x->M;
  p.K = x->K1 + K2;
  p.K1 = x->K1;
  p.lda1 = x->lda1;
  p.lda2 = a2 ? x->lda2 : 0;
  p.ldr = x->ldr > 0 ? x->ldr : x->ldc;
  p.w_shared = (a2 && x->w_shared) ? 1 : 0;
  TD_REQUIRE(!p.w_shared || K2 == x->K1, "td_linear_ex: a shared weight needs K2 == K1");
  p.a1_map = x->a1_map;
  p.a2_map = a2 ? x->a2_map : nullptr;
  p.out_map = x->out_map;
  p.res_map = x->res_map;
  td_conv_desc d;
  memset(&d, 0, sizeof(d));
  d.N = 1; d.Hs = x->M; d.Ws = 1; d.C = p.K; d.Ho = x->M; d.Wo = 1; d.R = d.S = 1; d.stride = 1; d.Nc = x->N; d.ldc = x->ldc; d.out_sp = 1;
  p.d = d;
  {
    const double b1 = (double)x->rows1 * x->lda1 * es, b2 = a2 ? (double)x->rows2 * x->lda2 * es : 16.0, wb = (double)x->N * (p.w_shared ? x->K1 : p.K) * es;
    TD_REQUIRE(b1 < 4294967000.0 && b2 < 4294967000.0 && wb < 4294967000.0, "td_linear_ex: operand exceeds the 4 GiB buffer-descriptor range");
    p.src_bytes = (uint32_t)b1;
    p.src2_bytes = (uint32_t)b2;
    p.w_bytes = (uint32_t)wb;
  }
  p.alpha = 1.f;
  if (e) {
    p.bias = e->bias;
    p.residual = (const char*)e->residual;
    p.mask_src = (const char*)e->mask_src;
    p.relu = e->relu;
    p.sigmoid = e->sigmoid;
    if (e->alpha != 0.f) p.alpha = e->alpha;
    if (e->dropout_p > 0.f) {
      TD_REQUIRE(e->dropout_p < 1.f, "td_linear_ex: dropout_p must be < 1");
      p.drop_thresh = (uint32_t)((double)e->dropout_p * 4294967296.0);
      if (p.drop_thresh == 0) p.drop_thresh = 1;
      p.drop_scale = 1.f / (1.f - e->dropout_p);
      p.seed = e->dropout_seed;
      p.seed_dev = e->dropout_counter;
    }
  }
  hipStream_t st = (hipStream_t)stream;
  const bool narrow = x->N <= 64;
  const int tiles128 = cdiv(p.M, 128) * cdiv(x->N, 128);
  const bool small_m = !narrow && (tiles128 < 512 || p.K <= 512);
  const int BMsel = small_m ? 64 : 128, BNsel = narrow ? 64 : 128;
  dim3 grid(8 * cdiv(cdiv(p.M, BMsel), 8) * cdiv(x->N, BNsel));
  const bool prof = prof_on();
  if (prof) {
    prof_begin(narrow ? TD_PROF_GEMM_128x64 : (small_m ? TD_PROF_GEMM_64x128 : TD_PROF_GEMM_128x128), dtype, 2.0 * p.M * x->N * p.K, st, p.M, x->N, p.K, 1, 1, 2);
    double by = ((double)p.M * p.K + (double)x->N * p.K + (double)p.M * x->N) * es;
    if (p.residual) by += (double)p.M * x->N * es;
    if (p.mask_src) by += (double)p.M * x->N * es;
    prof_set_bytes(by);
  }
#define TD_LX(TT)                                                                                     \
  do {                                                                                                \
    if (narrow) conv_gemm_kernel<TT, 128, 64, 2, true, false, true><<<grid, 256, 0, st>>>(p);         \
    else if (small_m) conv_gemm_kernel<TT, 64, 128, 2, true, false, true><<<grid, 256, 0, st>>>(p);   \
    else conv_gemm_kernel<TT, 128, 128, 2, true, false, true><<<grid, 256, 0, st>>>(p);               \
  } while (0)
  if (dtype == TD_BF16) TD_LX(u16);
  else TD_LX(float);
#undef TD_LX
  if (prof) prof_end(st);
  return check_launch("td_linear_ex");
}

static int wgrad_stages() {
  static const int nstg = [] { const char* e = getenv("TD_WGRAD_STAGES"); return (e && atoi(e) == 2) ? 2 : 4; }();
  return nstg;
}

static int wgrad_fill(WgradParams& p, const void* g, const void* src, const td_conv_desc* d, int ldg, int dtype, int* splits_io,
                      int auto_mode, const char* who) {
  int rc = validate(d, dtype, who);
  if (rc) return rc;
  const int vec = dtype == TD_BF16 ? 8 : 4;
  TD_REQUIRE(d->mode == 0 && !d->aniso, "%s: isotropic forward geometry expected", who);
  TD_REQUIRE(d->Nc % vec == 0 && ldg % vec == 0, "%s: Nc=%d / ldg=%d must be multiples of %d", who, d->Nc, ldg, vec);
  memset(&p, 0, sizeof(p));
  p.g = (const char*)g;
  p.src = (const char*)src;
  p.d = *d;
  p.M = d->N * d->Ho * d->Wo;
  p.K = d->R * d->S * d->C;
  p.ldg = ldg;
  p.ci_real = d->C;
  {
    const double es = dtype == TD_BF16 ? 2.0 : 4.0;
    const double gb = (double)p.M * ldg * es, sb = (double)d->N * d->Hs * d->Ws * d->C * es;
    TD_REQUIRE(gb < 4294967000.0 && sb < 4294967000.0, "%s: operand exceeds the 4 GiB buffer-descriptor range", who);
    p.g_bytes = (uint32_t)gb;
    p.src_bytes = (uint32_t)sb;
  }
  const int mk = dtype == TD_BF16 ? 64 : 32;
  p.tn = cdiv(d->Nc, 128);
  p.tk = cdiv(p.K, 128);
  int splits = *splits_io;
  if (splits < 1) {
    if (auto_mode == 0) {
      static const int target_blocks = [] { const char* e = getenv("TD_WGRAD_BLOCKS"); return e ? atoi(e) : 256; }();
      const int tiles = p.tn * p.tk;
      splits = wgrad_stages() == 4 ? target_blocks / tiles : cdiv(target_blocks, tiles);
      const int maxs = cdiv(p.M, 8 * mk);
      if (splits > maxs) splits = maxs;
// ... 215 lines not shown
```

tubedetr_amd/functional.py:

```python
from __future__ import annotations

import math
from typing import Optional

import torch
from torch.autograd import Function

from . import ops

Tensor = torch.Tensor

_EPOCH = [0]


def invalidate_prepared():
    _EPOCH[0] += 1


class _PrepEntry:
    __slots__ = ("base_ref", "offset", "shape", "bn", "dtype", "need_dgrad", "cpad", "co_alloc", "res", "ver", "dims")


class _PrepRegistry:

# ... 229 lines not shown

    @staticmethod
    def backward(ctx, dy):
        _arm()
        x, y, wd = ctx.saved_tensors
        relu, p, seed, N, Np, has_b = ctx.cfg
        dy = dy.contiguous()
        if Np != N:
            g = dy.new_zeros((dy.shape[0], Np))
            g[:, :N] = dy
            dy = g
        if relu:
            g = ops.relu_bwd(dy, y, 1.0 / (1.0 - p) if p > 0 else 1.0)
        elif p > 0:
            g = ops.dropout(dy, p, seed)
        else:
            g = dy
        dx = ops.linear_fwd(g, wd) if ctx.needs_input_grad[0] else None
        want_w, want_b = ctx.needs_input_grad[1], has_b and ctx.needs_input_grad[2]
        dW = db = None
        if want_w:
            dW_full, db_full = _wgrad(g, x, _can_defer(*ctx.params), want_bias=want_b)
            dW = dW_full[:N]
            db = db_full[:N] if want_b else None
        elif want_b:
            db = ops.colsum(g)[:N]
        return dx, dW, db, None, None, None


def linear(x, W, b=None, relu=False, dropout_p=0.0, training=False):
    p = dropout_p if training else 0.0
    return LinearFn.apply(x, W, b, relu, p, _seed() if p > 0 else 0)


class FFNFn(Function):

    @staticmethod
    def forward(ctx, x, W1, b1, W2, b2, p: float, seed1: int, seed2: int):
        _note_use(ctx.needs_input_grad[1], W1, b1, W2, b2)
        w1f, w1d, _, _ = prepared(W1, x.dtype)
        w2f, w2d, _, _ = prepared(W2, x.dtype)
        h = ops.linear_fwd(x, w1f, b1.detach(), relu=True, dropout_p=p, seed=seed1)
        y = ops.linear_fwd(h, w2f, b2.detach(), dropout_p=p, seed=seed2)
        ctx.save_for_backward(x, h, w1d, w2d)
        ctx.cfg = (p, seed1, seed2)
        ctx.params = (W1, b1, W2, b2)
        return y

    @staticmethod
    def backward(ctx, dy):
        _arm()
        x, h, w1d, w2d = ctx.saved_tensors
        p, seed1, seed2 = ctx.cfg
        defer = _can_defer(*ctx.params)
        g2 = ops.dropout(dy.contiguous(), p, seed2) if p > 0 else dy.contiguous()
        dW2, db2 = _wgrad(g2, h, defer, want_bias=True)
        dh = ops.linear_fwd(g2, w2d, mask_src=h, alpha=1.0 / (1.0 - p) if p > 0 else 1.0)
        dW1, db1 = _wgrad(dh, x, defer, want_bias=True)
        dx = ops.linear_fwd(dh, w1d) if ctx.needs_input_grad[0] else None
        return dx, dW1, db1, dW2, db2, None, None, None


def ffn(x, W1, b1, W2, b2, dropout_p=0.0, training=False):
    p = dropout_p if training else 0.0
    return FFNFn.apply(x, W1, b1, W2, b2, p, _seed() if p > 0 else 0, _seed() if p > 0 else 0)


class AddLayerNormFn(Function):

    @staticmethod
    def forward(ctx, x, r, gamma, beta, eps: float):
        y, s, mean, rstd = ops.add_layernorm_fwd(x, r, gamma.detach(), beta.detach(), eps)
        ctx.save_for_backward(s, mean, rstd, gamma.detach())
        ctx.has_r = r is not None
        return y

    @staticmethod
    def backward(ctx, dy):
        s, mean, rstd, gamma = ctx.saved_tensors
        ds, dg, db = ops.add_layernorm_bwd(dy.contiguous(), s, mean, rstd, gamma)
        return ds, (ds if ctx.has_r else None), dg, db, None


def add_layernorm(x, r, gamma, beta, eps=1e-5):
    return AddLayerNormFn.apply(x, r, gamma, beta, eps)


class AddFn(Function):

    @staticmethod
    def forward(ctx, a, b):
        return ops.add(a, b)

    @staticmethod
    def backward(ctx, g):
        return g, g


class MHAFn(Function):

    @staticmethod
    def forward(ctx, q_in, q_pos, k_in, v_in, W_in, b_in, W_out, b_out, key_pad, B, Lq, Lk, H, need_w, p_attn, seed_attn, p_out, seed_out):
        _note_use(ctx.needs_input_grad[4], W_in, b_in, W_out, b_out)
        E = q_in.shape[1]
        dt = q_in.dtype
        same_qk = k_in is None
        bi = b_in.detach()

        def proj(x_, w_, b_):
            return ops.linear_ex(x_, w_, b_, a2=q_pos, w_shared=True) if q_pos is not None else ops.linear_fwd(x_, w_, b_)

        if same_qk:
            wqk_f, wqk_d, _, _ = prepared(W_in[: 2 * E], dt)
            qk = proj(q_in, wqk_f, bi[: 2 * E]).view(B, Lq, 2 * E)
            q, k = qk[..., :E], qk[..., E:]
            wd_list = (wqk_d,)
        else:
            wq_f, wq_d, _, _ = prepared(W_in[:E], dt)
            wk_f, wk_d, _, _ = prepared(W_in[E : 2 * E], dt)
            q = proj(q_in, wq_f, bi[:E]).view(B, Lq, E)
            k = ops.linear_fwd(k_in, wk_f, bi[E : 2 * E]).view(B, Lk, E)
            wd_list = (wq_d, wk_d)
        wv_f, wv_d, _, _ = prepared(W_in[2 * E :], dt)
        v = ops.linear_fwd(v_in, wv_f, bi[2 * E :]).view(B, Lk, E)
        scale = 1.0 / math.sqrt(E // H)
        lean = not need_w and ops.mha_lean_ok(q, k, v, H)
        if lean:
            ctxv, probs, kp = ops.mha_lean_fwd(q, k, v, key_pad, H, scale, dropout_p=p_attn, seed=seed_attn)
            wavg = None
        else:
            ctxv, probs, wavg = ops.mha_fwd(q, k, v, key_pad, H, scale, need_wavg=need_w, dropout_p=p_attn, seed=seed_attn)
            kp = None
        wo_f, wo_d, _, _ = prepared(W_out, dt)
        out = ops.linear_fwd(ctxv.view(B * Lq, E), wo_f, b_out.detach(), dropout_p=p_out, seed=seed_out)
        ctx.save_for_backward(q_in, q_pos, k_in, v_in, q, k, v, probs, ctxv, wv_d, wo_d, *wd_list)
        ctx.lean, ctx.kp = lean, kp
        ctx.cfg = (B, Lq, Lk, H, E, same_qk, scale, p_attn, seed_attn, p_out, seed_out)
        ctx.params = (W_in, b_in, W_out, b_out)
        return out, (wavg if need_w else None)

    @staticmethod
    def backward(ctx, dout, dwavg):
        _arm()
        q_in, q_pos, k_in, v_in, q, k, v, probs, ctxv, wv_d, wo_d, *wd_list = ctx.saved_tensors
        B, Lq, Lk, H, E, same_qk, scale, p_attn, seed_attn, p_out, seed_out = ctx.cfg
        dt = q_in.dtype
        dev = q_in.device
        defer = _can_defer(*ctx.params)
        g = ops.dropout(dout.contiguous(), p_out, seed_out) if p_out > 0 else dout.contiguous()
        if defer:
            dW_in = torch.empty((3 * E, E), dtype=torch.float32, device=dev)
            db_in = torch.empty(3 * E, dtype=torch.float32, device=dev)
        else:
            dW_in = ops.zeros_f32((3 * E, E), dev)
            db_in = ops.zeros_f32(3 * E, dev)
        dW_out, db_out = _wgrad(g, ctxv.view(B * Lq, E), defer, want_bias=True)
        dctx = ops.linear_fwd(g, wo_d).view(B, Lq, E)
        if same_qk:
            dqk = torch.empty((B, Lq, 2 * E), dtype=dt, device=dev)
            dq, dk = dqk[..., :E], dqk[..., E:]
        else:
            dq = torch.empty((B, Lq, E), dtype=dt, device=dev)
            dk = torch.empty((B, Lk, E), dtype=dt, device=dev)
        dv = torch.empty((B, Lk, E), dtype=dt, device=dev)
        dwa = dwavg.contiguous().float() if dwavg is not None else None
        if ctx.lean:
            ops.mha_lean_bwd(q, k, v, ctx.kp, ctxv, dctx, probs, H, scale, dq, dk, dv, dropout_p=p_attn, seed=seed_attn)
        else:
            ops.mha_bwd(q, k, v, dctx, probs, dwa, H, scale, dq, dk, dv, dropout_p=p_attn, seed=seed_attn)
        dv2 = dv.view(B * Lk, E)
        _wgrad(dv2, v_in, defer, want_bias=True, out=dW_in[2 * E :], dbias=db_in[2 * E :])
        d_v_in = ops.linear_fwd(dv2, wv_d) if ctx.needs_input_grad[3] else None
        d_q_in = d_k_in = None
        need_q = ctx.needs_input_grad[0] or (q_pos is not None and ctx.needs_input_grad[1])
        if same_qk:
            dqk2 = dqk.view(B * Lq, 2 * E)
            _wgrad(dqk2, q_in, defer, want_bias=True, out=dW_in[: 2 * E], dbias=db_in[: 2 * E], x2=q_pos)
            if need_q:
                d_q_in = ops.linear_fwd(dqk2, wd_list[0])
        else:
            dq2, dk2 = dq.view(B * Lq, E), dk.view(B * Lk, E)
            _wgrad(dq2, q_in, defer, want_bias=True, out=dW_in[:E], dbias=db_in[:E], x2=q_pos)
            _wgrad(dk2, k_in, defer, want_bias=True, out=dW_in[E : 2 * E], dbias=db_in[E : 2 * E])
            if need_q:
                d_q_in = ops.linear_fwd(dq2, wd_list[0])
            if ctx.needs_input_grad[2]:
                d_k_in = ops.linear_fwd(dk2, wd_list[1])
        return (d_q_in if ctx.needs_input_grad[0] else None, d_q_in if (q_pos is not None and ctx.needs_input_grad[1]) else None, d_k_in, d_v_in,
                dW_in, db_in, dW_out, db_out) + (None,) * 10


class _CrossKVShared:

    def __init__(self, mem, pos, n_layers, E):
        self.mem, self.pos, self.n_layers, self.E = mem, pos, n_layers, E
        self.dK = self.dV = None
        self.written = set()
        self.wk_d = self.wv_d = None

    def grads(self, like):
        if self.dK is None:
            self.dK = torch.empty((self.mem.shape[0], self.n_layers * self.E), dtype=like.dtype, device=like.device)
            self.dV = torch.empty_like(self.dK)
        return self.dK, self.dV


class CrossKVFn(Function):

    @staticmethod
    def forward(ctx, mem, pos, shared, *w_and_b):
        E, dt = shared.E, mem.dtype
        Ws, bs = w_and_b[0::2], w_and_b[1::2]
        kf, vf, kd, vd = [], [], [], []
        for W in Ws:
            f, d_, _, _ = prepared(W[E : 2 * E], dt)
            kf.append(f); kd.append(d_)
            f, d_, _, _ = prepared(W[2 * E :], dt)
            vf.append(f); vd.append(d_)
        bk = torch.cat([b.detach()[E : 2 * E] for b in bs])
        bv = torch.cat([b.detach()[2 * E :] for b in bs])
        wk = torch.cat(kf, dim=0)
        K_all = ops.linear_ex(mem, wk, bk, a2=pos, w_shared=True) if pos is not None else ops.linear_fwd(mem, wk, bk)
        V_all = ops.linear_fwd(mem, torch.cat(vf, dim=0), bv)
        shared.wk_d, shared.wv_d = torch.cat(kd, dim=1), torch.cat(vd, dim=1)
        ctx.shared = shared
        ctx.set_materialize_grads(False)
        return K_all, V_all

    @staticmethod
    def backward(ctx, gK, gV):
        sh = ctx.shared
        assert gK is None and gV is None, "the consumers of CrossKVFn hand their gradients over through the shared buffers"
        if sh.dK is None:
            return (None,) * (3 + 2 * sh.n_layers)
        for l in range(sh.n_layers):
            if l not in sh.written:
                sh.dK[:, l * sh.E : (l + 1) * sh.E].zero_()
                sh.dV[:, l * sh.E : (l + 1) * sh.E].zero_()
        d_mem = d_pos = None
        need_pos = sh.pos is not None and ctx.needs_input_grad[1]
        if ctx.needs_input_grad[0] or need_pos:
            d_k = ops.linear_fwd(sh.dK, sh.wk_d)
# ... 401 lines not shown
```

tubedetr_amd/models/transformer.py:

```python
from __future__ import annotations

import copy
import math
import os
from typing import List, Optional

import torch
from torch import Tensor, nn

from .. import functional as Fk
from .. import ops as _ops
from ..util.misc import LRUCache
from .position_encoding import TimeEmbeddingLearned, TimeEmbeddingSine

FAST_MODES_IN_HIP = ("",)
FAST_MODES = ("", "gating", "transformer", "pool", "noslow")


class MultiheadAttention(nn.Module):

    def __init__(self, embed_dim: int, num_heads: int, dropout: float = 0.0):
        super().__init__()
        self.embed_dim, self.num_heads, self.dropout = embed_dim, num_heads, dropout
        self.in_proj_weight = nn.Parameter(torch.empty(3 * embed_dim, embed_dim))
        self.in_proj_bias = nn.Parameter(torch.zeros(3 * embed_dim))
        self.out_proj = nn.Linear(embed_dim, embed_dim)
        nn.init.xavier_uniform_(self.in_proj_weight)
        nn.init.constant_(self.out_proj.bias, 0.0)

    def run_prekv(self, q_in, kv, layer, key_pad, B, Lq, Lk, need_weights, out_dropout, training, q_pos=None):
        return Fk.multihead_attention_prekv(q_in, kv, layer, self.in_proj_weight, self.in_proj_bias, self.out_proj.weight, self.out_proj.bias, key_pad,
                                            B, Lq, Lk, self.num_heads, need_weights, attn_dropout=self.dropout, out_dropout=out_dropout, training=training,
                                            q_pos=q_pos)

    def run_q1(self, q_in, anchor, key_pad, F, S, need_weights, out_dropout, training, q_pos=None):
        return Fk.multihead_attention_q1(q_in, anchor, self.in_proj_weight, self.in_proj_bias, self.out_proj.weight, self.out_proj.bias, key_pad,
                                         F, S, self.num_heads, need_weights, attn_dropout=self.dropout, out_dropout=out_dropout, training=training,
                                         q_pos=q_pos)

    def run(self, q_in, k_in, v_in, key_pad, B, Lq, Lk, need_weights, out_dropout, training, q_pos=None):
        return Fk.multihead_attention(q_in, k_in, v_in, self.in_proj_weight, self.in_proj_bias, self.out_proj.weight,
                                      self.out_proj.bias, key_pad, B, Lq, Lk, self.num_heads, need_weights,
                                      attn_dropout=self.dropout, out_dropout=out_dropout, training=training, q_pos=q_pos)


class TransformerEncoderLayer(nn.Module):
    def __init__(self, d_model, nhead, dim_feedforward=2048, dropout=0.1, activation="relu"):
        super().__init__()
        if activation != "relu":
            raise NotImplementedError("only the reference default activation (relu) is fused in the HIP FFN")
        self.self_attn = MultiheadAttention(d_model, nhead, dropout=dropout)
        self.linear1 = nn.Linear(d_model, dim_feedforward)
        self.linear2 = nn.Linear(dim_feedforward, d_model)
        self.norm1 = nn.LayerNorm(d_model)
        self.norm2 = nn.LayerNorm(d_model)
        self.p = dropout

    def forward(self, src: Tensor, pos: Optional[Tensor], key_pad: Optional[Tensor], B: int, S: int) -> Tensor:
        a, _ = self.self_attn.run(src, None, src, key_pad, B, S, S, False, self.p, self.training, q_pos=pos)
        src = Fk.add_layernorm(a, src, self.norm1.weight, self.norm1.bias, self.norm1.eps)
        f = Fk.ffn(src, self.linear1.weight, self.linear1.bias, self.linear2.weight, self.linear2.bias, self.p, self.training)
        return Fk.add_layernorm(f, src, self.norm2.weight, self.norm2.bias, self.norm2.eps)


class TransformerEncoder(nn.Module):
    def __init__(self, encoder_layer, num_layers, norm=None, return_weights=False):
        super().__init__()
        self.layers = nn.ModuleList([copy.deepcopy(encoder_layer) for _ in range(num_layers)])
        self.num_layers = num_layers
        self.norm = norm
        self.return_weights = return_weights

    def forward(self, src, key_pad, pos, B, S):
        out = src
        for layer in self.layers:
            out = layer(out, pos, key_pad, B, S)
        if self.norm is not None:
            out = Fk.add_layernorm(out, None, self.norm.weight, self.norm.bias, self.norm.eps)
        return out


class TransformerDecoderLayer(nn.Module):
    def __init__(self, d_model, nhead, dim_feedforward=2048, dropout=0.1, activation="relu", no_tsa=False):
        super().__init__()
        if activation != "relu":
            raise NotImplementedError("only relu")
        self.self_attn = MultiheadAttention(d_model, nhead, dropout=dropout)
        self.cross_attn_image = MultiheadAttention(d_model, nhead, dropout=dropout)
        self.linear1 = nn.Linear(d_model, dim_feedforward)
        self.linear2 = nn.Linear(dim_feedforward, d_model)
        self.norm1 = nn.LayerNorm(d_model)
        self.norm3 = nn.LayerNorm(d_model)
        self.norm4 = nn.LayerNorm(d_model)
        self.p = dropout
        self.no_tsa = no_tsa

    def forward(self, tgt, query_pos, mem, pos, query_mask, memory_mask, b: int, t: int, S: int, kv=None, index: int = 0):
        if self.no_tsa:
            a, w = self.self_attn.run(tgt, None, tgt, None, b * t, 1, 1, True, self.p, self.training, q_pos=query_pos)
        else:
            a, w = self.self_attn.run(tgt, None, tgt, query_mask, b, t, t, True, self.p, self.training, q_pos=query_pos)
        tgt = Fk.add_layernorm(a, tgt, self.norm1.weight, self.norm1.bias, self.norm1.eps)
        if isinstance(kv, tuple) and len(kv) == 2:
            a, cw = self.cross_attn_image.run_q1(tgt, kv, memory_mask, b * t, S, True, self.p, self.training, q_pos=query_pos)
        elif kv is not None:
            a, cw = self.cross_attn_image.run_prekv(tgt, kv, index, memory_mask, b * t, 1, S, True, self.p, self.training, q_pos=query_pos)
        else:
            mem_k = Fk.AddFn.apply(mem, pos) if pos is not None else mem
            a, cw = self.cross_attn_image.run(tgt, mem_k, mem, memory_mask, b * t, 1, S, True, self.p, self.training, q_pos=query_pos)
        tgt = Fk.add_layernorm(a, tgt, self.norm3.weight, self.norm3.bias, self.norm3.eps)
        f = Fk.ffn(tgt, self.linear1.weight, self.linear1.bias, self.linear2.weight, self.linear2.bias, self.p, self.training)
        tgt = Fk.add_layernorm(f, tgt, self.norm4.weight, self.norm4.bias, self.norm4.eps)
        return tgt, w, cw


class TransformerDecoder(nn.Module):
    def __init__(self, decoder_layer, num_layers, norm=None, return_intermediate=False, return_weights=False):
        super().__init__()
        self.layers = nn.ModuleList([copy.deepcopy(decoder_layer) for _ in range(num_layers)])
        self.num_layers = num_layers
        self.norm = norm
        self.return_intermediate = return_intermediate
        self.return_weights = return_weights

    def forward(self, tgt, query_pos, mem, pos, query_mask, memory_mask, b, t, S):
        inter, ws, cws = [], [], []
        out = tgt
        att = self.layers[0].cross_attn_image
        if (os.environ.get("TD_CROSS_Q1", "1") != "0" and att.embed_dim == 256 and att.num_heads == 8 and S <= 320
                and not (pos is not None and pos.requires_grad)):
            kv = Fk.cross_q1_memory(mem, pos)
        else:
            kv = Fk.cross_kv(mem, pos, [l.cross_attn_image for l in self.layers]) if os.environ.get("TD_KV_HOIST", "1") != "0" else None
        for i, layer in enumerate(self.layers):
            out, w, cw = layer(out, query_pos, mem, pos, query_mask, memory_mask, b, t, S, kv=kv, index=i)
            if self.return_intermediate:
                inter.append(Fk.add_layernorm(out, None, self.norm.weight, self.norm.bias, self.norm.eps))
                ws.append(w)
                cws.append(cw)
        if not self.return_intermediate:
            out = Fk.add_layernorm(out, None, self.norm.weight, self.norm.bias, self.norm.eps) if self.norm is not None else out
            return (out, w, cw) if self.return_weights else out
        hs = torch.stack(inter)
        if not self.return_weights:
            return hs
        return hs, torch.stack(ws), torch.stack(cws)


class FeatureResizer(nn.Module):

    def __init__(self, input_feat_size, output_feat_size, dropout, do_ln=True):
        super().__init__()
        self.do_ln = do_ln
        self.fc = nn.Linear(input_feat_size, output_feat_size, bias=True)
        self.layer_norm = nn.LayerNorm(output_feat_size, eps=1e-12)
        self.p = dropout

    def forward(self, rows: Tensor) -> Tensor:
        x = Fk.linear(rows, self.fc.weight, self.fc.bias)
        if self.do_ln:
            x = Fk.add_layernorm(x, None, self.layer_norm.weight, self.layer_norm.bias, self.layer_norm.eps)
        return Fk.dropout(x, self.p, self.training)


class HashTokenizer:
# ... 322 lines not shown
```

tubedetr_amd/ops.py:

```python
from __future__ import annotations

import os

import ctypes as C
from typing import Optional, Tuple

import torch

from . import _hip
from ._hip import ConvDesc, Epilogue, check, dtype_code, ptr, stream_ptr

Tensor = torch.Tensor


class _ZeroArena:

    def __init__(self, chunk: int):
        self.chunk = chunk
        self.buf = None
        self.off = 0

    def take(self, shape, device) -> torch.Tensor:
        n = 1
        for d_ in shape:
# ... 19 lines not shown


def zeros_f32(shape, device) -> torch.Tensor:
    if not _USE_ARENA:
        return torch.zeros(shape, dtype=torch.float32, device=device)
    shape = tuple(shape) if not isinstance(shape, int) else (shape,)
    if device.type == "cuda" and torch.cuda.is_current_stream_capturing():
        sp = stream_ptr()
        if sp not in _CAPTURE_ARENAS:
            _CAPTURE_ARENAS[sp] = _ZeroArena(256 * 1024)
        return _CAPTURE_ARENAS[sp].take(shape, device)
    if _CAPTURE_ARENAS:
        _CAPTURE_ARENAS.clear()
    key = (str(device), stream_ptr() if device.type == "cuda" else 0)
    arena = _ARENAS.get(key)
    if arena is None:
        arena = _ARENAS[key] = _ZeroArena(32 * 1024 * 1024)
    return arena.take(shape, device)


def vec_of(dt: torch.dtype) -> int:
    return 8 if dt == torch.bfloat16 else 4


def pad_to(n: int, m: int) -> int:
    return (n + m - 1) // m * m


def conv_out(h: int, k: int, stride: int, pad: int) -> int:
    return (h + 2 * pad - k) // stride + 1


def _desc(N, Hs, Ws, Cs, Ho, Wo, R, S, stride, pad, mode, Nc, ldc, out_sp=1, out_H=0, out_W=0, stride_w=None, pad_w=None) -> ConvDesc:
    if stride_w is None and pad_w is None:
        return ConvDesc(N, Hs, Ws, Cs, Ho, Wo, R, S, stride, pad, mode, Nc, ldc, out_sp, out_H, out_W)
    return ConvDesc(N, Hs, Ws, Cs, Ho, Wo, R, S, stride, pad, mode, Nc, ldc, out_sp, out_H, out_W, 1, stride if stride_w is None else stride_w,
                    pad if pad_w is None else pad_w)


_DROPOUT_COUNTER = [None]


def set_dropout_counter(counter: Optional[torch.Tensor]) -> None:
    if counter is not None:
        assert counter.is_cuda and counter.numel() == 1 and counter.element_size() == 4
    _DROPOUT_COUNTER[0] = counter


def _ctr():
    c = _DROPOUT_COUNTER[0]
    return c.data_ptr() if c is not None else None


def _epi(bias=None, residual=None, mask_src=None, relu=False, sigmoid=False, dropout_p=0.0, seed=0, alpha=1.0) -> Epilogue:
    return Epilogue(ptr(bias), ptr(residual), ptr(mask_src), int(relu), int(sigmoid), float(dropout_p), int(seed) & 0xFFFFFFFF, float(alpha),
                    _ctr() if dropout_p > 0 else None)


def conv_gemm_raw(src: Tensor, w: Tensor, out: Tensor, desc: ConvDesc, epi: Optional[Epilogue]):
    check(_hip.lib().td_conv_gemm(ptr(src), ptr(w), ptr(out), C.byref(desc), C.byref(epi) if epi is not None else None,
                                  dtype_code(src.dtype), stream_ptr()), "td_conv_gemm")


def conv_fwd(x: Tensor, w_fwd: Tensor, bias: Optional[Tensor], R: int, S: int, stride: int, pad: int, *,
             residual: Optional[Tensor] = None, relu: bool = False, out: Optional[Tensor] = None) -> Tensor:
    N, H, W, Cs = x.shape
    Co = w_fwd.shape[0]
    assert w_fwd.shape[1] == R * S * Cs and w_fwd.dtype == x.dtype and x.is_contiguous() and w_fwd.is_contiguous()
    Ho, Wo = conv_out(H, R, stride, pad), conv_out(W, S, stride, pad)
    y = out if out is not None else torch.empty((N, Ho, Wo, Co), dtype=x.dtype, device=x.device)
    conv_gemm_raw(x, w_fwd, y, _desc(N, H, W, Cs, Ho, Wo, R, S, stride, pad, 0, Co, Co), _epi(bias, residual, None, relu))
    return y


def conv_dgrad(g: Tensor, w_dgrad: Tensor, in_hw: Tuple[int, int], R: int, S: int, stride: int, pad: int, *,
               residual: Optional[Tensor] = None, mask_src: Optional[Tensor] = None, out: Optional[Tensor] = None) -> Tensor:
    N, Hg, Wg, Co = g.shape
    H, W = in_hw
    Ci = w_dgrad.shape[0]
    assert w_dgrad.shape[1] == R * S * Co and g.is_contiguous()
    dx = out if out is not None else torch.empty((N, H, W, Ci), dtype=g.dtype, device=g.device)
    conv_gemm_raw(g, w_dgrad, dx, _desc(N, Hg, Wg, Co, H, W, R, S, stride, pad, 1, Ci, Ci), _epi(None, residual, mask_src))
    return dx


def conv1x1s_dgrad_scatter(g: Tensor, w_dgrad: Tensor, dx: Tensor, stride: int, *, mask_src: Optional[Tensor] = None):
    N, Hg, Wg, Co = g.shape
    _, H, W, Ci = dx.shape
    d = _desc(N, Hg, Wg, Co, Hg, Wg, 1, 1, 1, 0, 0, Ci, Ci, stride, H, W)
    conv_gemm_raw(g, w_dgrad, dx, d, _epi(None, dx, mask_src))
    return dx


def conv_wgrad(g: Tensor, x: Tensor, R: int, S: int, stride: int, pad: int, *, out: Optional[Tensor] = None, splits: int = 0) -> Tensor:
    N, H, W, Cs = x.shape
    _, Ho, Wo, Co = g.shape
    dw = out if out is not None else zeros_f32((Co, R * S * Cs), x.device)
    d = _desc(N, H, W, Cs, Ho, Wo, R, S, stride, pad, 0, Co, Co)
    check(_hip.lib().td_conv_wgrad(ptr(g), ptr(x), ptr(dw), C.byref(d), Co, dtype_code(x.dtype), splits, stream_ptr()), "td_conv_wgrad")
    return dw


class _JobTables:

    RING = 12

    def __init__(self):
        self.slots, self.retired, self.cap, self.next = [], [], 0, 0

# ... 33 lines not shown


def conv_wgrad_batch(jobs) -> list:
    jobs = list(jobs)
    arr = (_hip.WgradJob * len(jobs))()
    outs = []
    for a, (g, x, R, S, stride, pad, scale, ci_real) in zip(arr, jobs):
        N, H, W, Cs = x.shape
        _, Ho, Wo, Co = g.shape
        assert g.is_contiguous() and x.is_contiguous() and g.dtype == x.dtype
        dw = torch.empty((Co, ci_real, R, S), dtype=torch.float32, device=x.device)
        outs.append(dw)
        a.g, a.src, a.dW, a.scale = g.data_ptr(), x.data_ptr(), dw.data_ptr(), (scale.data_ptr() if scale is not None else None)
        a.d = _desc(N, H, W, Cs, Ho, Wo, R, S, stride, pad, 0, Co, Co)
        a.ldg, a.ci_real, a.dbias = Co, ci_real, None
    nbytes = _hip.lib().td_conv_wgrad_batch_table_bytes(len(jobs))
    th, td_, done = job_tables.take(nbytes, jobs[0][0].device)
    check(_hip.lib().td_conv_wgrad_batch(arr, len(jobs), dtype_code(jobs[0][0].dtype), th.data_ptr(), td_.data_ptr(), nbytes, stream_ptr()),
          "td_conv_wgrad_batch")
    done()
    return outs


def linear_wgrad_batch(jobs) -> None:
    if not jobs:
        return
    key0 = (jobs[0][0].dtype, jobs[0][0].device)
    if any((j[0].dtype, j[0].device) != key0 for j in jobs):
        groups: dict = {}
        for j in jobs:
            groups.setdefault((j[0].dtype, j[0].device), []).append(j)
        for sub in groups.values():
            linear_wgrad_batch(sub)
        return
    arr = (_hip.WgradJob * len(jobs))()
    for a, job in zip(arr, jobs):
        g, x, dw_ptr, db_ptr = job[:4]
        M, K = x.shape
        Nn = g.shape[1]
        assert g.shape[0] == M and g.stride(1) == 1 and x.is_contiguous() and g.dtype == x.dtype
        a.g, a.src, a.dW, a.scale, a.dbias = g.data_ptr(), x.data_ptr(), dw_ptr, None, db_ptr
        a.d = _desc(1, M, 1, K, M, 1, 1, 1, 1, 0, 0, Nn, Nn)
        a.ldg, a.ci_real = g.stride(0), K
        a.accumulate = int(len(job) > 4 and bool(job[4]))
    nbytes = _hip.lib().td_conv_wgrad_batch_table_bytes(len(jobs))
    dev = jobs[0][0].device
    th, td_, done = job_tables.take(nbytes, dev)
    check(_hip.lib().td_conv_wgrad_batch(arr, len(jobs), dtype_code(jobs[0][0].dtype), th.data_ptr(), td_.data_ptr(), nbytes, stream_ptr()),
          "td_conv_wgrad_batch(linears)")
    done()


def linear_fwd(x: Tensor, w: Tensor, bias: Optional[Tensor] = None, *, residual=None, relu=False, sigmoid=False,
               mask_src=None, dropout_p=0.0, seed=0, alpha=1.0, out: Optional[Tensor] = None) -> Tensor:
    M, K = x.shape
    Nn = w.shape[0]
    assert w.shape[1] == K and w.dtype == x.dtype and x.is_contiguous() and w.is_contiguous()
    y = out if out is not None else torch.empty((M, Nn), dtype=x.dtype, device=x.device)
    conv_gemm_raw(x, w, y, _desc(1, M, 1, K, M, 1, 1, 1, 1, 0, 0, Nn, Nn), _epi(bias, residual, mask_src, relu, sigmoid, dropout_p, seed, alpha))
    return y


def pw_chain2(y2: Tensor, w3: Tensor, b3: Tensor, residual: Tensor, w1: Tensor, b1: Tensor, *, out: Optional[Tensor] = None,
              h1: Optional[Tensor] = None) -> Tuple[Tensor, Tensor]:
    M, P = y2.shape
    assert y2.dtype == torch.bfloat16 and w3.shape == (4 * P, P) and w1.shape == (P, 4 * P) and residual.shape == (M, 4 * P)
    assert y2.is_contiguous() and w3.is_contiguous() and w1.is_contiguous() and residual.is_contiguous()
    assert b3.dtype == torch.float32 and b1.dtype == torch.float32 and b3.numel() == 4 * P and b1.numel() == P
    out = out if out is not None else torch.empty((M, 4 * P), dtype=y2.dtype, device=y2.device)
    h1 = h1 if h1 is not None else torch.empty((M, P), dtype=y2.dtype, device=y2.device)
    check(_hip.lib().td_pw_chain2(ptr(y2), ptr(w3), ptr(b3), ptr(residual), ptr(out), ptr(w1), ptr(b1), ptr(h1), M, P, dtype_code(y2.dtype),
                                  stream_ptr()), "td_pw_chain2")
    return out, h1


def _rows2d(t: Tensor):
    assert t.dim() == 2 and t.stride(1) == 1, "row-major 2-D operand expected (unit column stride)"
    return t


def linear_ex(a1: Tensor, w: Tensor, bias: Optional[Tensor] = None, *, a2: Optional[Tensor] = None, a1_map: Optional[Tensor] = None,
              a2_map: Optional[Tensor] = None, w_shared: bool = False, out: Optional[Tensor] = None, out_map: Optional[Tensor] = None,
              out_rows: Optional[int] = None, residual: Optional[Tensor] = None, res_map: Optional[Tensor] = None, relu=False, mask_src=None,
              dropout_p=0.0, seed=0, alpha=1.0) -> Tensor:
    _rows2d(a1)
    K1 = a1.shape[1]
    K2 = _rows2d(a2).shape[1] if a2 is not None else 0
    M = int(a1_map.numel()) if a1_map is not None else a1.shape[0]
    Nn = w.shape[0]
    assert w.is_contiguous() and w.dtype == a1.dtype and w.shape[1] == (K1 if (w_shared or a2 is None) else K1 + K2)
    for m_ in (a1_map, a2_map, out_map, res_map):
        assert m_ is None or (m_.dtype == torch.int32 and m_.is_contiguous() and m_.numel() == M)
    if out is None:
        out = torch.empty((out_rows if out_rows is not None else M, Nn), dtype=a1.dtype, device=a1.device)
    _rows2d(out)
    x = _hip.LinearExDesc()
    x.M, x.N, x.K1, x.K2 = M, Nn, K1, K2
    x.lda1, x.lda2, x.ldc = a1.stride(0), (a2.stride(0) if a2 is not None else 0), out.stride(0)
    x.ldr = _rows2d(residual).stride(0) if residual is not None else 0
    x.w_shared = int(bool(w_shared and a2 is not None))
    x.rows1, x.rows2 = a1.shape[0], (a2.shape[0] if a2 is not None else 0)
    x.a1_map, x.a2_map, x.out_map, x.res_map = ptr(a1_map), ptr(a2_map), ptr(out_map), ptr(res_map)
    epi = _epi(bias, residual, mask_src, relu, False, dropout_p, seed, alpha)
    check(_hip.lib().td_linear_ex(ptr(a1), ptr(a2), ptr(w), ptr(out), C.byref(x), C.byref(epi), dtype_code(a1.dtype), stream_ptr()), "td_linear_ex")
    return out


def rows_copy(src: Tensor, src_map: Optional[Tensor], dst: Tensor, dst_map: Optional[Tensor], n_rows: int, add: Optional[Tensor] = None) -> Tensor:
    _rows2d(src), _rows2d(dst)
    cols = src.shape[1]
    assert dst.shape[1] == cols and dst.dtype == src.dtype and (add is None or (_rows2d(add).shape[1] == cols and add.dtype == src.dtype and add.shape[0] >= n_rows))
    for m_ in (src_map, dst_map):
        assert m_ is None or (m_.dtype == torch.int32 and m_.is_contiguous() and m_.numel() == n_rows)
    check(_hip.lib().td_rows_copy(ptr(src), ptr(src_map), ptr(add), ptr(dst), ptr(dst_map), n_rows, cols, src.stride(0), add.stride(0) if add is not None else 0,
                                  dst.stride(0), dtype_code(src.dtype), stream_ptr()), "td_rows_copy")
    return dst


def rows_segment_sum(inp: Tensor, idx: Tensor, seg_ptr: Tensor, out: Tensor, out_map: Optional[Tensor] = None) -> Tensor:
    _rows2d(inp), _rows2d(out)
    n_out = seg_ptr.numel() - 1
    assert idx.dtype == torch.int32 and seg_ptr.dtype == torch.int32 and out.dtype == inp.dtype and out.shape[1] == inp.shape[1]
    assert out_map is None or (out_map.dtype == torch.int32 and out_map.numel() == n_out)
    check(_hip.lib().td_rows_segment_sum(ptr(inp), ptr(idx), ptr(seg_ptr), ptr(out), ptr(out_map), n_out, inp.shape[1], inp.stride(0), out.stride(0),
                                         dtype_code(inp.dtype), stream_ptr()), "td_rows_segment_sum")
    return out


def linear_wgrad(g: Tensor, x: Tensor, *, out: Optional[Tensor] = None, splits: int = 0, dbias: Optional[Tensor] = None) -> Tensor:
    M, K = x.shape
    Nn = g.shape[1]
    dw = out if out is not None else zeros_f32((Nn, K), x.device)
    d = _desc(1, M, 1, K, M, 1, 1, 1, 1, 0, 0, Nn, Nn)
    if dbias is not None:
        assert dbias.dtype == torch.float32 and dbias.numel() == Nn and dbias.is_contiguous()
    assert g.stride(1) == 1 and x.is_contiguous()
    check(_hip.lib().td_conv_wgrad_bias(ptr(g), ptr(x), ptr(dw), ptr(dbias), C.byref(d), g.stride(0), dtype_code(x.dtype), splits, stream_ptr()),
          "td_conv_wgrad")
    return dw


def weight_prep(W: Tensor, dtype: torch.dtype, *, bn=None, bias: Optional[Tensor] = None, need_dgrad: bool = True, cpad: Optional[int] = None):
    if W.dim() == 2:
        Co, Ci = W.shape
        R = S = 1
    else:
        Co, Ci, R, S = W.shape
    cp = cpad if cpad is not None else pad_to(Ci, vec_of(dtype))
    dev = W.device
    wf = torch.empty((Co, R * S * cp), dtype=dtype, device=dev)
    wd = torch.empty((Ci, R * S * Co), dtype=dtype, device=dev) if need_dgrad else None
    b_out = torch.empty(Co, dtype=torch.float32, device=dev) if (bn is not None or bias is not None) else None
    sc = torch.empty(Co, dtype=torch.float32, device=dev) if bn is not None else None
    bw, bb, brm, brv = bn if bn is not None else (None, None, None, None)
    check(_hip.lib().td_weight_prep(ptr(W), ptr(bw), ptr(bb), ptr(brm), ptr(brv), ptr(bias), Co, Ci, R, S, cp, ptr(wf), ptr(wd),
                                    ptr(b_out), ptr(sc), dtype_code(dtype), stream_ptr()), "td_weight_prep")
    return wf, wd, b_out, sc


def wgrad_finalize(dw_k: Tensor, scale: Optional[Tensor], shape, cpad: int, out: Optional[Tensor] = None, accumulate: bool = False) -> Tensor:
    Co, Ci, R, S = shape
    dW = out if out is not None else torch.empty(shape, dtype=torch.float32, device=dw_k.device)
    check(_hip.lib().td_wgrad_finalize(ptr(dw_k), ptr(scale), ptr(dW), Co, Ci, R, S, cpad, int(accumulate), stream_ptr()), "td_wgrad_finalize")
    return dW


def nchw_to_nhwc(x: Tensor, dtype: torch.dtype, cpad: int) -> Tensor:
    N, Cc, H, W = x.shape
    assert x.dtype == torch.float32 and x.is_contiguous()
    y = torch.empty((N, H, W, cpad), dtype=dtype, device=x.device)
    check(_hip.lib().td_nchw_to_nhwc(ptr(x), ptr(y), N, Cc, H, W, cpad, dtype_code(dtype), stream_ptr()), "td_nchw_to_nhwc")
    return y


def nhwc_to_nchw(x: Tensor) -> Tensor:
    N, H, W, Cc = x.shape
    y = torch.empty((N, Cc, H, W), dtype=torch.float32, device=x.device)
    check(_hip.lib().td_nhwc_to_nchw(ptr(x), ptr(y), N, Cc, H, W, dtype_code(x.dtype), stream_ptr()), "td_nhwc_to_nchw")
    return y


def cast(x: Tensor, dtype: torch.dtype) -> Tensor:
    if x.dtype == dtype:
        return x
    y = torch.empty(x.shape, dtype=dtype, device=x.device)
    check(_hip.lib().td_cast(ptr(x.contiguous()), ptr(y), x.numel(), dtype_code(x.dtype), dtype_code(dtype), stream_ptr()), "td_cast")
    return y


def maxpool3x3s2(x: Tensor) -> Tensor:
    N, H, W, Cc = x.shape
    y = torch.empty((N, conv_out(H, 3, 2, 1), conv_out(W, 3, 2, 1), Cc), dtype=x.dtype, device=x.device)
    check(_hip.lib().td_maxpool3x3s2(ptr(x), ptr(y), N, H, W, Cc, dtype_code(x.dtype), stream_ptr()), "td_maxpool3x3s2")
    return y


def add_layernorm_fwd(x: Tensor, r: Optional[Tensor], gamma: Tensor, beta: Tensor, eps: float, save: bool = True):
    rows, cols = x.shape
    y = torch.empty_like(x)
    s = torch.empty_like(x) if (save and r is not None) else None
    mean = torch.empty(rows, dtype=torch.float32, device=x.device) if save else None
    rstd = torch.empty(rows, dtype=torch.float32, device=x.device) if save else None
    check(_hip.lib().td_add_layernorm_fwd(ptr(x), ptr(r), ptr(gamma), ptr(beta), ptr(y), ptr(s), ptr(mean), ptr(rstd), rows, cols, eps,
                                          dtype_code(x.dtype), stream_ptr()), "td_add_layernorm_fwd")
    return y, (s if r is not None else x), mean, rstd


def add_layernorm_bwd(dy: Tensor, s: Tensor, mean: Tensor, rstd: Tensor, gamma: Tensor, extra: Optional[Tensor] = None):
    rows, cols = dy.shape
    ds = torch.empty_like(dy)
    dgamma = zeros_f32(cols, dy.device)
    dbeta = zeros_f32(cols, dy.device)
    check(_hip.lib().td_add_layernorm_bwd(ptr(dy), ptr(s), ptr(mean), ptr(rstd), ptr(gamma), ptr(extra), ptr(ds), ptr(dgamma), ptr(dbeta),
                                          rows, cols, dtype_code(dy.dtype), stream_ptr()), "td_add_layernorm_bwd")
    return ds, dgamma, dbeta


def colsum(g: Tensor, out: Optional[Tensor] = None) -> Tensor:
    rows, cols = g.shape
    o = out if out is not None else zeros_f32(cols, g.device)
    check(_hip.lib().td_colsum(ptr(g), ptr(o), rows, cols, cols, dtype_code(g.dtype), stream_ptr()), "td_colsum")
    return o


def add(a: Tensor, b: Optional[Tensor]) -> Tensor:
    y = torch.empty_like(a)
    check(_hip.lib().td_add(ptr(a), ptr(b), ptr(y), a.numel(), dtype_code(a.dtype), stream_ptr()), "td_add")
    return y


def relu_bwd(dy: Tensor, y: Tensor, scale: float = 1.0) -> Tensor:
    g = torch.empty_like(dy)
    check(_hip.lib().td_relu_bwd(ptr(dy), ptr(y), ptr(g), dy.numel(), scale, dtype_code(dy.dtype), stream_ptr()), "td_relu_bwd")
    return g


def pos_sine(mask: Tensor, npf: int, dtype: torch.dtype, temperature: float = 10000.0, rows: Optional[int] = None) -> Tensor:
    N, h, w = mask.shape
    m8 = mask.to(torch.uint8).contiguous()
    rows = h * w if rows is None else int(rows)
    pos = torch.empty((N, rows, 2 * npf), dtype=dtype, device=mask.device)
    check(_hip.lib().td_pos_sine(ptr(m8), ptr(pos), N, h, w, npf, temperature, rows, dtype_code(dtype), stream_ptr()), "td_pos_sine")
    return pos


def mha_fwd(q: Tensor, k: Tensor, v: Tensor, key_pad: Optional[Tensor], H: int, scale: float, *, need_wavg: bool = False,
            dropout_p: float = 0.0, seed: int = 0):
    B, Lq, E = q.shape
    Lk = k.shape[1]
    hd = E // H
    for t_ in (q, k, v):
        assert t_.stride(2) == 1 and t_.stride(0) == t_.shape[1] * t_.stride(1)
    out = torch.empty((B, Lq, E), dtype=q.dtype, device=q.device)
    probs = torch.empty((B, H, Lq, Lk), dtype=torch.float32, device=q.device)
    wavg = torch.empty((B, Lq, Lk), dtype=torch.float32, device=q.device) if need_wavg else None
    kp = key_pad.to(torch.uint8).contiguous() if key_pad is not None else None
    check(_hip.lib().td_mha_fwd(ptr(q), ptr(k), ptr(v), ptr(kp), ptr(out), ptr(probs), ptr(wavg), B, H, Lq, Lk, hd, q.stride(1), k.stride(1),
                                v.stride(1), E, scale, dropout_p, seed & 0xFFFFFFFF, _ctr() if dropout_p > 0 else None, dtype_code(q.dtype), stream_ptr()),
          "td_mha_fwd")
    return out, probs, wavg


def mha_lean_ok(q: Tensor, k: Tensor, v: Tensor, H: int) -> bool:
    if os.environ.get("TD_MHA_LEAN", "1") == "0":
        return False
    E = q.shape[2]
    return (q.dtype == torch.bfloat16 and E // H == 32
            and all(t_.stride(1) % 8 == 0 and t_.data_ptr() % 16 == 0 for t_ in (q, k, v)))
# ... 135 lines not shown
```

Before: 106.4.

## Fuse attention/FFN with residual add-layernorm and add accumulate/dropout epilogues

Adds an accumulate operand to the GEMM epilogues (generic, big8, big8n, pw_resident) so a GEMM output can be summed with an existing tensor in the same kernel. It also adds an optional dropout-mask output to the add-layernorm backward kernel and a dropout epilogue to the big GEMM kernels. Encoder and decoder layers now call fused self-attention+add-layernorm and FFN+add-layernorm autograd paths. The aim is to remove separate elementwise add, dropout and layernorm-grad launches and the extra memory passes between them, at the cost of more kernel template variants and register pressure in epilogues.

```diff
diff --git a/include/tubedetr_hip.h b/include/tubedetr_hip.h
--- a/include/tubedetr_hip.h
+++ b/include/tubedetr_hip.h
@@ -17,6 +17,7 @@
 
 const char* td_last_error(void);
 int td_abi_version(void);
+int td_abi_revision(void);
 
 int td_set_deterministic(int on);
 int td_get_deterministic(void);
@@ -63,6 +64,8 @@
   uint32_t dropout_seed;
   float alpha;
   const uint32_t* dropout_counter;
+  const void* accum;
+  int ldacc;
 } td_epilogue;
 
 int td_conv_gemm(const void* src, const void* wmat, void* out, const td_conv_desc* d, const td_epilogue* e,
@@ -155,7 +158,8 @@
 int td_add_layernorm_fwd(const void* x, const void* r, const float* gamma, const float* beta, void* y, void* s_out,
                          float* mean, float* rstd, int rows, int cols, float eps, int dtype, td_stream_t stream);
 int td_add_layernorm_bwd(const void* dy, const void* s, const float* mean, const float* rstd, const float* gamma,
-                         const void* extra, void* ds, float* dgamma, float* dbeta, int rows, int cols, int dtype,
+                         const void* extra, void* ds, float* dgamma, float* dbeta, void* ds_drop, float dropout_p,
+                         uint32_t dropout_seed, const uint32_t* dropout_counter, int rows, int cols, int dtype,
                          td_stream_t stream);
 
 int td_colsum(const void* g, float* out, int rows, int cols, int ld, int dtype, td_stream_t stream);
diff --git a/tubedetr_amd/_hip.py b/tubedetr_amd/_hip.py
--- a/tubedetr_amd/_hip.py
+++ b/tubedetr_amd/_hip.py
@@ -7,6 +7,7 @@
 
 TD_F32, TD_BF16 = 0, 1
 EXPECTED_ABI = 11
+EXPECTED_REVISION = 1
 _LIB_PATH = os.environ.get("TD_HIP_LIB") or os.path.join(os.path.dirname(os.path.abspath(__file__)), "lib", "libtubedetr_hip.so")
 _lib = None
 
@@ -57,11 +58,14 @@
         ("dropout_seed", C.c_uint32),
         ("alpha", C.c_float),
         ("dropout_counter", C.c_void_p),
+        ("accum", C.c_void_p),
+        ("ldacc", C.c_int),
     ]
 
 
 _P, _I, _F, _U32, _SZ = C.c_void_p, C.c_int, C.c_float, C.c_uint32, C.c_size_t
 _SIGS = {
+    "td_abi_revision": [],
     "td_prof_enable": [_I],
     "td_prof_dump": [C.c_char_p],
     "td_debug_set_stamp_buffer": [_P],
@@ -90,7 +94,7 @@
     "td_cast": [_P, _P, _SZ, _I, _I, _P],
     "td_maxpool3x3s2": [_P, _P, _I, _I, _I, _I, _I, _P],
     "td_add_layernorm_fwd": [_P, _P, _P, _P, _P, _P, _P, _P, _I, _I, _F, _I, _P],
-    "td_add_layernorm_bwd": [_P, _P, _P, _P, _P, _P, _P, _P, _P, _I, _I, _I, _P],
+    "td_add_layernorm_bwd": [_P, _P, _P, _P, _P, _P, _P, _P, _P, _P, _F, _U32, _P, _I, _I, _I, _P],
     "td_colsum": [_P, _P, _I, _I, _I, _I, _P],
     "td_add": [_P, _P, _P, _SZ, _I, _P],
     "td_relu_bwd": [_P, _P, _P, _SZ, _F, _I, _P],
@@ -148,6 +152,8 @@
         L.td_abi_version.restype = C.c_int
         L.td_abi_version.argtypes = []
         got = L.td_abi_version()
+        if got == EXPECTED_ABI and (not hasattr(L, "td_abi_revision") or L.td_abi_revision() != EXPECTED_REVISION):
+            got = f"{got} at another revision"
         if got != EXPECTED_ABI:
             raise RuntimeError(f"{_LIB_PATH} has ABI version {got}, this binding needs {EXPECTED_ABI}: rebuild it with "
                                "`python -m tubedetr_amd.build --force`")
diff --git a/tubedetr_amd/csrc/api.cpp b/tubedetr_amd/csrc/api.cpp
--- a/tubedetr_amd/csrc/api.cpp
+++ b/tubedetr_amd/csrc/api.cpp
@@ -124,5 +124,6 @@
   return TD_OK;
 }
 
+extern "C" int td_abi_revision(void) { return 1; }
 extern "C" const char* td_last_error(void) { return td::g_err; }
 extern "C" int td_abi_version(void) { return 11; }
diff --git a/tubedetr_amd/csrc/elementwise.hip b/tubedetr_amd/csrc/elementwise.hip
--- a/tubedetr_amd/csrc/elementwise.hip
+++ b/tubedetr_amd/csrc/elementwise.hip
@@ -145,15 +145,17 @@
   }
 }
 
-template <int NJ>
+template <int NJ, bool DROP = false>
 __global__ __launch_bounds__(256) void add_layernorm_bwd_v4_kernel(const u16* __restrict__ dy, const u16* __restrict__ s, const float* __restrict__ mean,
                                                                    const float* __restrict__ rstd, const float* __restrict__ gamma,
                                                                    const u16* __restrict__ extra, u16* __restrict__ ds, float* dgamma, float* dbeta,
-                                                                   int rows) {
+                                                                   int rows, u16* __restrict__ ds_drop = nullptr, float drop_scale = 1.f,
+                                                                   uint32_t drop_thresh = 0, uint32_t seed_in = 0, const uint32_t* seed_dev = nullptr) {
   constexpr int cols = NJ * 256;
   const int lane = threadIdx.x & 63;
   const int wid = blockIdx.x * 4 + (threadIdx.x >> 6);
   const int nw = gridDim.x * 4;
+  const uint32_t drop_seed = DROP ? effective_seed(seed_in, seed_dev) : 0u;
   float pg[NJ][4], pb[NJ][4], gm[NJ][4];
 #pragma unroll
   for (int j = 0; j < NJ; ++j) {
@@ -195,7 +197,14 @@
 #pragma unroll
         for (int e = 0; e < 4; ++e) o[e] += ex[e];
       }
-      *(uint2*)(ds + base + 256 * j) = pack4_bf16(o);
+      const uint2 od = pack4_bf16(o);
+      *(uint2*)(ds + base + 256 * j) = od;
+      if constexpr (DROP) {
+        unpack4v(od, o);
+#pragma unroll
+        for (int e = 0; e < 4; ++e) o[e] = dropout_keep(drop_seed, (uint32_t)(base + 256 * j + e), drop_thresh) ? o[e] * drop_scale : 0.f;
+        *(uint2*)(ds_drop + base + 256 * j) = pack4_bf16(o);
+      }
     }
   }
   __shared__ float redg[4][cols], redb[4][cols];
@@ -528,8 +537,12 @@
 
 extern "C" int td_add_layernorm_bwd(const void* dy, const void* s, const float* mean, const float* rstd,
                                     const float* gamma, const void* extra, void* ds, float* dgamma, float* dbeta,
+                                    void* ds_drop, float dropout_p, uint32_t dropout_seed, const uint32_t* dropout_counter,
                                     int rows, int cols, int dtype, td_stream_t stream) {
   TD_REQUIRE(dy && s && mean && rstd && gamma && ds, "td_add_layernorm_bwd: null pointer");
+  TD_REQUIRE(!ds_drop || (dropout_p > 0.f && dropout_p < 1.f), "td_add_layernorm_bwd: ds_drop needs 0 < dropout_p < 1");
+  TD_REQUIRE(!ds_drop || (dtype == TD_BF16 && (cols == 256 || cols == 768) && aligned8(dy, s, ds, extra) && ((uintptr_t)ds_drop & 7) == 0),
+             "td_add_layernorm_bwd: ds_drop is a member of the bf16 kernels for 256 / 768 columns (8-byte aligned rows)");
   TD_REQUIRE(cols <= 64 * LN_MAXJ, "td_add_layernorm_bwd: cols > %d", 64 * LN_MAXJ);
   if (rows == 0) return TD_OK;
   hipStream_t st = (hipStream_t)stream;
@@ -538,6 +551,14 @@
     unsigned gv = (rows + 31) / 32;
     if (gv > 1024) gv = 1024;
     if (deterministic()) gv = 1;
+    if (ds_drop) {
+      uint32_t thresh = (uint32_t)((double)dropout_p * 4294967296.0);
+      if (!thresh) thresh = 1;
+      const float scale = 1.f / (1.f - dropout_p);
+      if (cols == 256) add_layernorm_bwd_v4_kernel<1, true><<<gv, 256, 0, st>>>((const u16*)dy, (const u16*)s, mean, rstd, gamma, (const u16*)extra, (u16*)ds, dgamma, dbeta, rows, (u16*)ds_drop, scale, thresh, dropout_seed, dropout_counter);
+      else add_layernorm_bwd_v4_kernel<3, true><<<gv, 256, 0, st>>>((const u16*)dy, (const u16*)s, mean, rstd, gamma, (const u16*)extra, (u16*)ds, dgamma, dbeta, rows, (u16*)ds_drop, scale, thresh, dropout_seed, dropout_counter);
+      return check_launch("td_add_layernorm_bwd");
+    }
     if (cols == 256) add_layernorm_bwd_v4_kernel<1><<<gv, 256, 0, st>>>((const u16*)dy, (const u16*)s, mean, rstd, gamma, (const u16*)extra, (u16*)ds, dgamma, dbeta, rows);
     else add_layernorm_bwd_v4_kernel<3><<<gv, 256, 0, st>>>((const u16*)dy, (const u16*)s, mean, rstd, gamma, (const u16*)extra, (u16*)ds, dgamma, dbeta, rows);
     return check_launch("td_add_layernorm_bwd");
diff --git a/tubedetr_amd/csrc/gemm_conv.hip b/tubedetr_amd/csrc/gemm_conv.hip
--- a/tubedetr_amd/csrc/gemm_conv.hip
+++ b/tubedetr_amd/csrc/gemm_conv.hip
@@ -40,6 +40,8 @@
   const int* out_map;
   const int* res_map;
   int tap_inner;
+  const char* accum;
+  int ldacc;
   int w_ld;
   int wtap[4];
   int use_wtap;
@@ -370,7 +372,8 @@
   size_t offs[NIT];
   size_t roffs[GX ? NIT : 1];
   bool live[NIT];
-  uint4 res[NIT], msk[NIT];
+  constexpr bool ACCT = sizeof(T) == 2;
+  uint4 res[NIT], msk[NIT], acv[ACCT ? NIT : 1];
   auto fetch_epilogue_operands = [&]() {
 #pragma unroll
     for (int it = 0; it < NIT; ++it) {
@@ -396,6 +399,27 @@
     }
   };
 
+  auto acc_off = [&](int it) -> size_t {
+    size_t orow = (size_t)(m0 + wy * WM + it * RPI + rsub);
+    if (!PW && d.out_sp > 1) {
+      const int ni = (int)orow / HoWo, rem = (int)orow - ni * HoWo;
+      const int ho = rem / d.Wo, wo = rem - ho * d.Wo;
+      orow = ((size_t)ni * d.out_H + (size_t)ho * d.out_sp) * d.out_W + (size_t)wo * d.out_sp;
+    }
+    if constexpr (GX) {
+      if (p.out_map) orow = (size_t)p.out_map[orow];
+    }
+    return orow * (size_t)p.ldacc + n;
+  };
+  const bool vec_acc = vec_ok && (p.ldacc % EPL) == 0;
+  auto fetch_accum = [&]() {
+    if constexpr (ACCT) {
+      if (!p.accum) return;
+#pragma unroll
+      for (int it = 0; it < NIT; ++it)
+        if (vec_acc && live[it]) acv[it] = ld16(p.accum + acc_off(it) * ES);
+    }
+  };
   const int nk = (p.K + BK - 1) / BK;
 #define TD_STAMP(i) do { if (p.dbg && t == 0) p.dbg[(size_t)blockIdx.x * 8 + (i)] = __builtin_readcyclecounter(); } while (0)
   TD_STAMP(0);
@@ -413,6 +437,7 @@
     }
     TD_STAMP(2);
     fetch_epilogue_operands();
+    fetch_accum();
   } else {
 #define TD_CG_STEP(cur, nxt, j)                                                     \
   asm volatile("s_waitcnt vmcnt(%0)" ::"n"(AI + BI) : "memory");                    \
@@ -430,6 +455,7 @@
     asm volatile("s_waitcnt vmcnt(0)" ::: "memory");
     TD_STAMP(2);
     fetch_epilogue_operands();
+    fetch_accum();
   }
 
   asm volatile("s_waitcnt lgkmcnt(0)" ::: "memory");
@@ -491,7 +517,24 @@
 #pragma unroll
         for (int r = 0; r < EPL; ++r) v[r] = dropout_keep(eff_seed, (uint32_t)(off + r), p.drop_thresh) ? v[r] * p.drop_scale : 0.f;
       }
-      st16(p.out + off * ES, pack16<T>(v));
+      uint4 o = pack16<T>(v);
+      if constexpr (ACCT) {
+        if (p.accum) {
+          float a8[EPL];
+          unpack16<T>(o, v);
+          if (vec_acc) {
+            unpack16<T>(acv[it], a8);
+          } else {
+            const size_t ao = acc_off(it);
+#pragma unroll
+            for (int r = 0; r < EPL; ++r) a8[r] = Elem<T>::load(p.accum, ao + r);
+          }
+#pragma unroll
+          for (int r = 0; r < EPL; ++r) v[r] += a8[r];
+          o = pack16<T>(v);
+        }
+      }
+      st16(p.out + off * ES, o);
     } else {
       const int cnt = min(EPL, d.Nc - n);
       for (int r = 0; r < cnt; ++r) {
@@ -501,6 +544,11 @@
         if (p.sigmoid) x = sigmoidf_(x);
         if (p.mask_src) x = Elem<T>::load(p.mask_src, off + r) > 0.f ? x : 0.f;
         if (p.drop_thresh) x = dropout_keep(eff_seed, (uint32_t)(off + r), p.drop_thresh) ? x * p.drop_scale : 0.f;
+        if (ACCT && p.accum) {
+          const float av = Elem<T>::load(p.accum, acc_off(it) + r);
+          Elem<T>::store(p.out, off + r, x);
+          x = Elem<T>::load(p.out, off + r) + av;
+        }
         Elem<T>::store(p.out, off + r, x);
       }
     }
@@ -535,7 +583,7 @@
 #ifndef TD_BIG8_AUX_X
 #define TD_BIG8_AUX_X 0
 #endif
-template <bool TU, bool RES>
+template <bool TU, bool RES, int EX = 0>
 __global__ __launch_bounds__(512, 1) void conv_gemm_big8_kernel(GemmParams p) {
   using T = u16;
   constexpr int ES = 2, BM = 256, BN = 256, BK = 64, NW = 8, VEC = 8;
@@ -735,6 +783,8 @@
   const int cc = lane & 7, rsub = lane >> 3;
   const uint32_t sra = stg0 + (uint32_t)(rsub * 128 + ((cc ^ rsub) << 4));
   const float alpha = p.alpha;
+  constexpr bool DROP = (EX & 1) != 0, ACC = (EX & 2) != 0;
+  const uint32_t drop_seed = DROP ? effective_seed(p.seed, p.seed_dev) : 0u;
 
 #define TD_STAMP(i) do { if (p.dbg && t == 0) p.dbg[(size_t)vb * 8 + (i)] = __builtin_readcyclecounter(); } while (0)
   int vb = blockIdx.x;
@@ -784,6 +834,7 @@
     }
     TD_STAMP(3);
     uint4 mk[2][2];
+    uint4 ak[2][ACC ? 2 : 1];
     auto seg_off = [&](int j, int h) -> uint32_t {
       const int m = m0 + wy * WM + j * 16 + h * 8 + rsub;
       return m < p.M ? ((uint32_t)m * (uint32_t)d.ldc + (uint32_t)(n0 + wx * WN + cc * 8)) * ES : OOB;
@@ -812,11 +863,33 @@
 #pragma unroll
           for (int r = 0; r < 4; ++r) v[r] = fmaxf(v[r], 0.f);
         }
+        if constexpr (DROP) {
+          const uint32_t idx = (uint32_t)(m0 + wy * WM + j * 16 + lr) * (uint32_t)d.ldc + (uint32_t)(n0 + wx * WN + i * 16 + lg * 4);
+#pragma unroll
+          for (int r = 0; r < 4; ++r) v[r] = dropout_keep(drop_seed, idx + (uint32_t)r, p.drop_thresh) ? v[r] * p.drop_scale : 0.f;
+        }
         const uint32_t lo = pack_bf16x2(v[0], v[1]), hi = pack_bf16x2(v[2], v[3]);
         asm volatile("ds_write_b64 %0, %1" ::"v"(swa[i]), "v"(u32x2_t{lo, hi}) : "memory");
       }
     };
+    auto fetch_acc = [&](int j, int b) {
+#pragma unroll
+      for (int h = 0; h < 2; ++h) {
+        const int m = m0 + wy * WM + j * 16 + h * 8 + rsub;
+        ak[b][ACC ? h : 0] = m < p.M ? ld16(p.accum + ((size_t)m * p.ldacc + (n0 + wx * WN + cc * 8)) * ES) : make_uint4(0, 0, 0, 0);
+      }
+    };
+    auto add_acc = [&](u32x4_t& sv, const uint4& av) {
+      float x8[8], a8[8];
+      unpack16<T>(make_uint4(sv.x, sv.y, sv.z, sv.w), x8);
+      unpack16<T>(av, a8);
+#pragma unroll
+      for (int r = 0; r < 8; ++r) x8[r] += a8[r];
+      const uint4 q = pack16<T>(x8);
+      sv = u32x4_t{q.x, q.y, q.z, q.w};
+    };
     if (p.mask_src) fetch_mask(0, 0);
+    if constexpr (ACC) fetch_acc(0, 0);
     put(0);
     u32x4_t o0, o1;
     asm volatile("ds_read_b128 %0, %1" : "=v"(o0) : "v"(sra) : "memory");
@@ -826,6 +899,7 @@
       const int b = j & 1;
       if (j + 1 < TM) {
         if (p.mask_src) fetch_mask(j + 1, b ^ 1);
+        if constexpr (ACC) fetch_acc(j + 1, b ^ 1);
         put(j + 1);
         asm volatile("s_waitcnt lgkmcnt(4)" : "+v"(o0), "+v"(o1) : : "memory");
       } else {
@@ -851,6 +925,10 @@
         const uint4 q1 = pack16<T>(x8);
         s1 = u32x4_t{q1.x, q1.y, q1.z, q1.w};
       }
+      if constexpr (ACC) {
+        add_acc(s0, ak[b][0]);
+        add_acc(s1, ak[b][1]);
+      }
       __builtin_amdgcn_raw_buffer_store_b128(s0, rs_out, (int)seg_off(j, 0), 0, 0);
       __builtin_amdgcn_raw_buffer_store_b128(s1, rs_out, (int)seg_off(j, 1), 0, 0);
     }
@@ -862,7 +940,7 @@
 #undef TD_STAMP
 }
 
-template <bool TU>
+template <bool TU, int EX = 0>
 __global__ __launch_bounds__(512, 1) void conv_gemm_big8n_kernel(GemmParams p) {
   using T = u16;
   constexpr int ES = 2, BM = 256, BN = 128, BK = 64, NW = 8, VEC = 8;
@@ -1021,7 +1099,8 @@
   const int n = n0 + wx * WN + cc * EPL;
   uint32_t offs[2][NIT];
   bool live[2][NIT];
-  uint4 res[2][NIT], msk[2][NIT];
+  constexpr bool DROP = (EX & 1) != 0, ACC = (EX & 2) != 0;
+  uint4 res[2][NIT], msk[2][NIT], acv[2][ACC ? NIT : 1];
   auto fetch_chunk = [&](int c, int b) {
 #pragma unroll
     for (int it = 0; it < NIT; ++it) {
@@ -1030,6 +1109,7 @@
       offs[b][it] = (uint32_t)min(m, p.M - 1) * (uint32_t)d.ldc + (uint32_t)n;
       if (p.residual) res[b][it] = ld16(p.residual + offs[b][it] * ES);
       if (p.mask_src) msk[b][it] = ld16(p.mask_src + offs[b][it] * ES);
+      if constexpr (ACC) acv[b][it] = ld16(p.accum + ((size_t)min(m, p.M - 1) * p.ldacc + n) * ES);
     }
   };
 
@@ -1070,6 +1150,7 @@
   TD_STAMP(3);
   float* stg = (float*)(smem + wave * (CR * WN * 4));
   const float alpha = p.alpha;
+  const uint32_t drop_seed = (EX & 1) ? effective_seed(p.seed, p.seed_dev) : 0u;
   float bias[EPL];
 #pragma unroll
   for (int r = 0; r < EPL; ++r) bias[r] = p.bias ? p.bias[n + r] : 0.f;
@@ -1114,6 +1195,17 @@
 #pragma unroll
         for (int r = 0; r < EPL; ++r) v[r] = m8[r] > 0.f ? v[r] : 0.f;
       }
+      if constexpr (DROP) {
+#pragma unroll
+        for (int r = 0; r < EPL; ++r) v[r] = dropout_keep(drop_seed, offs[b][it] + (uint32_t)r, p.drop_thresh) ? v[r] * p.drop_scale : 0.f;
+      }
+      if constexpr (ACC) {
+        float a8[EPL];
+        unpack16<T>(pack16<T>(v), v);
+        unpack16<T>(acv[b][it], a8);
+#pragma unroll
+        for (int r = 0; r < EPL; ++r) v[r] += a8[r];
+      }
       if (live[b][it]) st16(p.out + offs[b][it] * ES, pack16<T>(v));
     }
     asm volatile("s_waitcnt lgkmcnt(0)" ::: "memory");
@@ -1122,7 +1214,7 @@
 #undef TD_STAMP
 }
 
-template <int NKT, bool RES, bool MSK>
+template <int NKT, bool RES, bool MSK, bool ACC = false>
 __global__ __launch_bounds__(256, 2) void pw_resident2_kernel(GemmParams p, int MT, int P) {
   using T = u16;
   constexpr int ES = 2;
@@ -1192,6 +1284,8 @@
       for (int i = 0; i < TN; ++i)
         wfr[kt][ks][i] = *(const uint4*)(p.w + ((size_t)(n0 + wx * WN + i * 16 + lr) * p.K + kt * 64 + ks * 32 + lg * 8) * ES);
   const uint32_t drop_seed = p.drop_thresh ? effective_seed(p.seed, p.seed_dev) : 0u;
+  constexpr bool HAS_ALPHA = !(RES && MSK && NKT == 4);
+  const float alpha = p.alpha;
   float* const stg = (float*)(sT + wave * (16 * WN * 4));
 
   auto seg_off = [&](int mt, int it) -> uint32_t {
@@ -1249,7 +1343,8 @@
       for (int i = 0; i < TN; ++i) {
         const int c = (i * 4 + lg) ^ (lr & (CPRW - 1));
         const f32x4 a = acc[i][j];
-        *(float4*)(stg + lr * WN + c * 4) = make_float4(a[0], a[1], a[2], a[3]);
+        if constexpr (HAS_ALPHA) *(float4*)(stg + lr * WN + c * 4) = make_float4(a[0] * alpha, a[1] * alpha, a[2] * alpha, a[3] * alpha);
+        else *(float4*)(stg + lr * WN + c * 4) = make_float4(a[0], a[1], a[2], a[3]);
       }
       asm volatile("s_waitcnt lgkmcnt(0)" ::: "memory");
 #pragma unroll
@@ -1285,7 +1380,17 @@
 #pragma unroll
           for (int r = 0; r < EPL; ++r) v[r] = dropout_keep(drop_seed, off / ES + (uint32_t)r, p.drop_thresh) ? v[r] * p.drop_scale : 0.f;
         }
-        const uint4 o = pack16<T>(v);
+        uint4 o = pack16<T>(v);
+        if constexpr (ACC) {
+          if (off != OOB) {
+            float a8[EPL];
+            unpack16<T>(o, v);
+            unpack16<T>(ld16(p.accum + ((size_t)(mt * 64 + wy * WM + it * RPI + rsub) * p.ldacc + n) * ES), a8);
+#pragma unroll
+            for (int r = 0; r < EPL; ++r) v[r] += a8[r];
+            o = pack16<T>(v);
+          }
+        }
         __builtin_amdgcn_raw_buffer_store_b128(u32x4_t{o.x, o.y, o.z, o.w}, rs_out, (int)off, 0, AUX_NT);
       }
       asm volatile("s_waitcnt lgkmcnt(0)" ::: "memory");
@@ -2117,6 +2222,7 @@
       if (e) ec = *e;
       if (ec.residual) ec.residual = (const char*)ec.residual + ooff;
       if (ec.mask_src) ec.mask_src = (const char*)ec.mask_src + ooff;
+      if (ec.accum) ec.accum = (const char*)ec.accum + ((size_t)ph * W + pw) * (ec.ldacc > 0 ? ec.ldacc : d->ldc) * es;
       const char* wp = (const char*)w_dgrad;
       if (sub.ntap == 1) {
         wp += (size_t)sub.wtap[0] * Co * es;
@@ -2177,6 +2283,9 @@
     p.mask_src = (const char*)e->mask_src;
     p.relu = e->relu;
     p.sigmoid = e->sigmoid;
+    p.accum = (const char*)e->accum;
+    p.ldacc = e->ldacc > 0 ? e->ldacc : d->ldc;
+    TD_REQUIRE(!p.accum || (dtype == TD_BF16 && p.ldacc >= d->Nc), "td_conv_gemm: accum is a bf16 operand with ldacc >= Nc");
     if (e->alpha != 0.f) p.alpha = e->alpha;
     if (e->dropout_p > 0.f) {
       TD_REQUIRE(e->dropout_p < 1.f, "td_conv_gemm: dropout_p must be < 1");
@@ -2197,13 +2306,14 @@
   {
     static const int persist = [] { const char* e_ = getenv("TD_PW_PERSIST"); return e_ ? atoi(e_) : 1; }();
     static const int persist_dropout = [] { const char* e_ = getenv("TD_PW_PERSIST_DROPOUT"); return e_ ? atoi(e_) : 1; }();
+    static const int persist_alpha = [] { const char* e_ = getenv("TD_PW_PERSIST_ALPHA"); return e_ ? atoi(e_) : 1; }();
     const bool pw0 = d->R == 1 && d->S == 1 && d->pad == 0 && p.d.out_sp == 1 && !d->aniso &&
                      ((d->stride == 1 && d->Hs == d->Ho && d->Ws == d->Wo) ||
                       (d->stride > 1 && d->mode == 0 && (d->Ho - 1) * d->stride < d->Hs && (d->Wo - 1) * d->stride < d->Ws));
     const int NTp = d->Nc / 128, Pp = 2 * n_cu / 8;
     const bool shape_ok = pw0 && !p.w_ld && dtype == TD_BF16 && p.K % 64 == 0 && p.K <= 256 && d->Nc % 128 == 0 &&
                           (NTp == 1 || NTp == 2 || NTp == 4 || NTp == 8 || NTp == 16) && Pp >= NTp && d->ldc % 8 == 0 && !p.sigmoid &&
-                          p.alpha == 1.f && n_cu % 8 == 0 && (!p.drop_thresh || persist_dropout) && (double)p.M * d->ldc < 2147483000.0;
+                          (p.alpha == 1.f || (persist_alpha && !(p.residual && p.mask_src && p.K == 256))) && n_cu % 8 == 0 && (!p.accum || (!p.residual && !p.mask_src && p.ldacc % 8 == 0)) && (!p.drop_thresh || persist_dropout) && (double)p.M * d->ldc < 2147483000.0;
     const int MTp = cdiv(p.M, 64);
     const int groups = shape_ok ? 8 * (Pp / NTp) : 1;
     if (persist && shape_ok && MTp >= persist_min_tiles() * groups && !(persist == 2 && p.mask_src) && !(persist == 3 && d->mode != 0)) {
@@ -2214,6 +2324,7 @@
         double by = ((double)p.M * p.K + (double)d->Nc * p.K + (double)p.M * d->Nc) * es_;
         if (p.residual) by += (double)p.M * d->Nc * es_;
         if (p.mask_src) by += (double)p.M * d->Nc * es_;
+        if (p.accum) by += (double)p.M * d->Nc * es_;
         prof_set_bytes(by);
       }
       const int nkt = p.K / 64;
@@ -2221,7 +2332,8 @@
       dim3 g2(2 * n_cu);
 #define TD_PWR(NK)                                                                               \
   do {                                                                                           \
-    if (hr && hm) pw_resident2_kernel<NK, true, true><<<g2, 256, 0, st>>>(p, MTp, Pp);          \
+    if (p.accum) pw_resident2_kernel<NK, false, false, true><<<g2, 256, 0, st>>>(p, MTp, Pp);    \
+    else if (hr && hm) pw_resident2_kernel<NK, true, true><<<g2, 256, 0, st>>>(p, MTp, Pp);     \
     else if (hr) pw_resident2_kernel<NK, true, false><<<g2, 256, 0, st>>>(p, MTp, Pp);          \
     else if (hm) pw_resident2_kernel<NK, false, true><<<g2, 256, 0, st>>>(p, MTp, Pp);          \
     else pw_resident2_kernel<NK, false, false><<<g2, 256, 0, st>>>(p, MTp, Pp);                 \
@@ -2251,16 +2363,19 @@
   {
     static const int big_on = [] { const char* e_ = getenv("TD_CONV_BIG"); return e_ ? atoi(e_) : 1; }();
     static const int big_min = [] { const char* e_ = getenv("TD_CONV_BIG_MIN_WG"); return e_ ? atoi(e_) : 160; }();
+    static const int big_dropout = [] { const char* e_ = getenv("TD_CONV_BIG_DROPOUT"); return e_ ? atoi(e_) : 1; }();
     const int bnb = d->Nc % 256 == 0 ? 256 : 128;
     const int wgs = cdiv(p.M, 256) * (d->Nc / bnb);
     if (big_on && dtype == TD_BF16 && (pw || tu) && p.d.out_sp == 1 && !p.use_wtap && !p.w_ld && d->Nc % 128 == 0 && p.K % 64 == 0 && p.K >= 512 && d->ldc % 8 == 0 && !p.sigmoid &&
-        !p.drop_thresh && wgs >= big_min && (double)p.M * d->ldc < 2147483000.0 &&
+        (!p.drop_thresh || (big_dropout && pw && !p.mask_src && !p.residual && p.alpha == 1.f)) &&
+        (!p.accum || (pw && !p.residual && !p.drop_thresh && p.ldacc % 8 == 0)) && wgs >= big_min && (double)p.M * d->ldc < 2147483000.0 &&
         p.K <= 64 * 154 && p.M < (1 << 24)) {
       if (prof) {
         prof_begin(tu ? TD_PROF_GEMM_256 : TD_PROF_GEMM_256_PW, dtype, 2.0 * p.M * d->Nc * p.K, st, p.M, d->Nc, p.K, d->R, d->stride, d->mode);
         double by = ((double)d->N * d->Hs * d->Ws * d->C + (double)d->Nc * p.K + (double)p.M * d->Nc) * 2.0;
         if (p.residual) by += (double)p.M * d->Nc * 2.0;
         if (p.mask_src) by += (double)p.M * d->Nc * 2.0;
+        if (p.accum) by += (double)p.M * d->Nc * 2.0;
         prof_set_bytes(by);
       }
       static const int tap_inner = [] { const char* e_ = getenv("TD_CONV_TAP_INNER"); return e_ ? atoi(e_) : 1; }();
@@ -2269,12 +2384,16 @@
       static const int persist8 = [] { const char* e_ = getenv("TD_CONV_BIG_PERSIST"); return e_ ? atoi(e_) : 1; }();
       if (bnb == 256) {
         const dim3 gp(persist8 && n_cu % 8 == 0 ? std::min((unsigned)n_cu, gb.x) : gb.x);
-        if (tu && p.residual) conv_gemm_big8_kernel<true, true><<<gp, 512, 0, st>>>(p);
+        if (p.accum) conv_gemm_big8_kernel<false, false, 2><<<gp, 512, 0, st>>>(p);
+        else if (p.drop_thresh) conv_gemm_big8_kernel<false, false, 1><<<gp, 512, 0, st>>>(p);
+        else if (tu && p.residual) conv_gemm_big8_kernel<true, true><<<gp, 512, 0, st>>>(p);
         else if (tu) conv_gemm_big8_kernel<true, false><<<gp, 512, 0, st>>>(p);
         else if (p.residual) conv_gemm_big8_kernel<false, true><<<gp, 512, 0, st>>>(p);
         else conv_gemm_big8_kernel<false, false><<<gp, 512, 0, st>>>(p);
       } else {
-        if (tu) conv_gemm_big8n_kernel<true><<<gb, 512, 0, st>>>(p);
+        if (p.accum) conv_gemm_big8n_kernel<false, 2><<<gb, 512, 0, st>>>(p);
+        else if (p.drop_thresh) conv_gemm_big8n_kernel<false, 1><<<gb, 512, 0, st>>>(p);
+        else if (tu) conv_gemm_big8n_kernel<true><<<gb, 512, 0, st>>>(p);
         else conv_gemm_big8n_kernel<false><<<gb, 512, 0, st>>>(p);
       }
       if (prof) prof_end(st);
@@ -2288,6 +2407,7 @@
     double by = ((double)d->N * d->Hs * d->Ws * d->C + (double)d->Nc * p.K + (double)p.M * d->Nc) * es;
     if (e && e->residual) by += rows_out * d->Nc * es;
     if (e && e->mask_src) by += rows_out * d->Nc * es;
+    if (e && e->accum) by += rows_out * d->Nc * es;
     prof_set_bytes(by);
   }
 #define TD_LAUNCH(TT, BMv, BNv)                                                                   \
@@ -2364,6 +2484,9 @@
     p.mask_src = (const char*)e->mask_src;
     p.relu = e->relu;
     p.sigmoid = e->sigmoid;
+    p.accum = (const char*)e->accum;
+    p.ldacc = e->ldacc > 0 ? e->ldacc : x->ldc;
+    TD_REQUIRE(!p.accum || (dtype == TD_BF16 && p.ldacc >= x->N), "td_linear_ex: accum is a bf16 operand with ldacc >= N");
     if (e->alpha != 0.f) p.alpha = e->alpha;
     if (e->dropout_p > 0.f) {
       TD_REQUIRE(e->dropout_p < 1.f, "td_linear_ex: dropout_p must be < 1");
@@ -2386,6 +2509,7 @@
     double by = ((double)p.M * p.K + (double)x->N * p.K + (double)p.M * x->N) * es;
     if (p.residual) by += (double)p.M * x->N * es;
     if (p.mask_src) by += (double)p.M * x->N * es;
+    if (p.accum) by += (double)p.M * x->N * es;
     prof_set_bytes(by);
   }
 #define TD_LX(TT)                                                                                     \
diff --git a/tubedetr_amd/functional.py b/tubedetr_amd/functional.py
--- a/tubedetr_amd/functional.py
+++ b/tubedetr_amd/functional.py
@@ -305,13 +305,17 @@
         _arm()
         x, h, w1d, w2d = ctx.saved_tensors
         p, seed1, seed2 = ctx.cfg
-        defer = _can_defer(*ctx.params)
         g2 = ops.dropout(dy.contiguous(), p, seed2) if p > 0 else dy.contiguous()
-        dW2, db2 = _wgrad(g2, h, defer, want_bias=True)
-        dh = ops.linear_fwd(g2, w2d, mask_src=h, alpha=1.0 / (1.0 - p) if p > 0 else 1.0)
-        dW1, db1 = _wgrad(dh, x, defer, want_bias=True)
-        dx = ops.linear_fwd(dh, w1d) if ctx.needs_input_grad[0] else None
-        return dx, dW1, db1, dW2, db2, None, None, None
+        return _ffn_backward(x, h, w1d, w2d, p, ctx.params, g2, ctx.needs_input_grad[0], None) + (None, None, None)
+
+
+def _ffn_backward(x, h, w1d, w2d, p, params, g2, need_dx, accum):
+    defer = _can_defer(*params)
+    dW2, db2 = _wgrad(g2, h, defer, want_bias=True)
+    dh = ops.linear_fwd(g2, w2d, mask_src=h, alpha=1.0 / (1.0 - p) if p > 0 else 1.0)
+    dW1, db1 = _wgrad(dh, x, defer, want_bias=True)
+    dx = ops.linear_fwd(dh, w1d, accum=accum) if need_dx else None
+    return dx, dW1, db1, dW2, db2
 
 
 def ffn(x, W1, b1, W2, b2, dropout_p=0.0, training=False):
@@ -339,6 +343,91 @@
     return AddLayerNormFn.apply(x, r, gamma, beta, eps)
 
 
+_FOLD_ON = [_os.environ.get("TD_SUBLAYER_FOLD", "1") != "0"]
+
+
+def set_sublayer_fold(on: bool) -> None:
+    _FOLD_ON[0] = bool(on)
+
+
+def _fold_ok(x) -> bool:
+    return (_FOLD_ON[0] and x.dtype == torch.bfloat16 and x.dim() == 2 and x.shape[1] in (256, 768) and x.requires_grad
+            and torch.is_grad_enabled())
+
+
+def _ln_backward_fold(dy, s, mean, rstd, gamma, p, seed):
+    if p > 0:
+        return ops.add_layernorm_bwd(dy.contiguous(), s, mean, rstd, gamma, drop_p=p, drop_seed=seed)
+    ds, dg, db = ops.add_layernorm_bwd(dy.contiguous(), s, mean, rstd, gamma)
+    return ds, dg, db, ds
+
+
+class FFNAddLayerNormFn(Function):
+
+    @staticmethod
+    def forward(ctx, x, W1, b1, W2, b2, gamma, beta, p: float, seed1: int, seed2: int, eps: float):
+        _note_use(ctx.needs_input_grad[1], W1, b1, W2, b2)
+        w1f, w1d, _, _ = prepared(W1, x.dtype)
+        w2f, w2d, _, _ = prepared(W2, x.dtype)
+        h = ops.linear_fwd(x, w1f, b1.detach(), relu=True, dropout_p=p, seed=seed1)
+        f = ops.linear_fwd(h, w2f, b2.detach(), dropout_p=p, seed=seed2)
+        y, s, mean, rstd = ops.add_layernorm_fwd(f, x, gamma.detach(), beta.detach(), eps)
+        ctx.save_for_backward(x, h, w1d, w2d, s, mean, rstd, gamma.detach())
+        ctx.cfg = (p, seed2)
+        ctx.params = (W1, b1, W2, b2)
+        return y
+
+    @staticmethod
+    def backward(ctx, dy):
+        _arm()
+        x, h, w1d, w2d, s, mean, rstd, gamma = ctx.saved_tensors
+        p, seed2 = ctx.cfg
+        ds, dg, db, g2 = _ln_backward_fold(dy, s, mean, rstd, gamma, p, seed2)
+        dx, dW1, db1, dW2, db2 = _ffn_backward(x, h, w1d, w2d, p, ctx.params, g2, True, ds)
+        return dx, dW1, db1, dW2, db2, dg, db, None, None, None, None
+
+
+class SelfAttnAddLayerNormFn(Function):
+
+    @staticmethod
+    def forward(ctx, x, pos, W_in, b_in, W_out, b_out, gamma, beta, key_pad, B, L, H, need_w, p_attn, seed_attn, p_out, seed_out, eps):
+        _note_use(ctx.needs_input_grad[2], W_in, b_in, W_out, b_out)
+        a, wavg, saved, ctx.lean, ctx.kp, ctx.cfg = _mha_forward(x, pos, None, x, W_in, b_in, W_out, b_out, key_pad, B, L, L, H, need_w,
+                                                                 p_attn, seed_attn, p_out, seed_out)
+        y, s, mean, rstd = ops.add_layernorm_fwd(a, x, gamma.detach(), beta.detach(), eps)
+        ctx.save_for_backward(s, mean, rstd, gamma.detach(), *saved)
+        ctx.params = (W_in, b_in, W_out, b_out)
+        return y, wavg
+
+    @staticmethod
+    def backward(ctx, dy, dwavg):
+        _arm()
+        s, mean, rstd, gamma, *saved = ctx.saved_tensors
+        p_out, seed_out = ctx.cfg[-2:]
+        ds, dg, db, g = _ln_backward_fold(dy, s, mean, rstd, gamma, p_out, seed_out)
+        needs = (True, ctx.needs_input_grad[1], False, True)
+        dx, dpos, _, _, dW_in, db_in, dW_out, db_out = _mha_backward(saved, ctx.lean, ctx.kp, ctx.cfg, ctx.params, needs, g, dwavg, ds)
+        return (dx, dpos, dW_in, db_in, dW_out, db_out, dg, db) + (None,) * 10
+
+
+def ffn_add_layernorm(x, W1, b1, W2, b2, gamma, beta, eps=1e-5, dropout_p=0.0, training=False):
+    if not _fold_ok(x):
+        return add_layernorm(ffn(x, W1, b1, W2, b2, dropout_p, training), x, gamma, beta, eps)
+    p = dropout_p if training else 0.0
+    return FFNAddLayerNormFn.apply(x, W1, b1, W2, b2, gamma, beta, p, _seed() if p > 0 else 0, _seed() if p > 0 else 0, eps)
+
+
+def self_attention_add_layernorm(x, pos, W_in, b_in, W_out, b_out, gamma, beta, key_pad, B, L, H, eps=1e-5, need_weights=False, attn_dropout=0.0,
+                                 out_dropout=0.0, training=False):
+    if not _fold_ok(x):
+        a, w = multihead_attention(x, None, x, W_in, b_in, W_out, b_out, key_pad, B, L, L, H, need_weights, attn_dropout, out_dropout, training, q_pos=pos)
+        return add_layernorm(a, x, gamma, beta, eps), w
+    pa = attn_dropout if training else 0.0
+    po = out_dropout if training else 0.0
+    return SelfAttnAddLayerNormFn.apply(x, pos, W_in, b_in, W_out, b_out, gamma, beta, key_pad, B, L, H, need_weights,
+                                        pa, _seed() if pa > 0 else 0, po, _seed() if po > 0 else 0, eps)
+
+
 class AddFn(Function):
 
     @staticmethod
@@ -355,92 +444,109 @@
     @staticmethod
     def forward(ctx, q_in, q_pos, k_in, v_in, W_in, b_in, W_out, b_out, key_pad, B, Lq, Lk, H, need_w, p_attn, seed_attn, p_out, seed_out):
         _note_use(ctx.needs_input_grad[4], W_in, b_in, W_out, b_out)
-        E = q_in.shape[1]
-        dt = q_in.dtype
-        same_qk = k_in is None
-        bi = b_in.detach()
-
-        def proj(x_, w_, b_):
-            return ops.linear_ex(x_, w_, b_, a2=q_pos, w_shared=True) if q_pos is not None else ops.linear_fwd(x_, w_, b_)
-
-        if same_qk:
-            wqk_f, wqk_d, _, _ = prepared(W_in[: 2 * E], dt)
-            qk = proj(q_in, wqk_f, bi[: 2 * E]).view(B, Lq, 2 * E)
-            q, k = qk[..., :E], qk[..., E:]
-            wd_list = (wqk_d,)
-        else:
-            wq_f, wq_d, _, _ = prepared(W_in[:E], dt)
-            wk_f, wk_d, _, _ = prepared(W_in[E : 2 * E], dt)
-            q = proj(q_in, wq_f, bi[:E]).view(B, Lq, E)
-            k = ops.linear_fwd(k_in, wk_f, bi[E : 2 * E]).view(B, Lk, E)
-            wd_list = (wq_d, wk_d)
-        wv_f, wv_d, _, _ = prepared(W_in[2 * E :], dt)
-        v = ops.linear_fwd(v_in, wv_f, bi[2 * E :]).view(B, Lk, E)
-        scale = 1.0 / math.sqrt(E // H)
-        lean = not need_w and ops.mha_lean_ok(q, k, v, H)
-        if lean:
-            ctxv, probs, kp = ops.mha_lean_fwd(q, k, v, key_pad, H, scale, dropout_p=p_attn, seed=seed_attn)
-            wavg = None
-        else:
-            ctxv, probs, wavg = ops.mha_fwd(q, k, v, key_pad, H, scale, need_wavg=need_w, dropout_p=p_attn, seed=seed_attn)
-            kp = None
-        wo_f, wo_d, _, _ = prepared(W_out, dt)
-        out = ops.linear_fwd(ctxv.view(B * Lq, E), wo_f, b_out.detach(), dropout_p=p_out, seed=seed_out)
-        ctx.save_for_backward(q_in, q_pos, k_in, v_in, q, k, v, probs, ctxv, wv_d, wo_d, *wd_list)
-        ctx.lean, ctx.kp = lean, kp
-        ctx.cfg = (B, Lq, Lk, H, E, same_qk, scale, p_attn, seed_attn, p_out, seed_out)
+        out, wavg, saved, ctx.lean, ctx.kp, ctx.cfg = _mha_forward(q_in, q_pos, k_in, v_in, W_in, b_in, W_out, b_out, key_pad, B, Lq, Lk, H, need_w,
+                                                                   p_attn, seed_attn, p_out, seed_out)
+        ctx.save_for_backward(*saved)
         ctx.params = (W_in, b_in, W_out, b_out)
-        return out, (wavg if need_w else None)
+        return out, wavg
 
     @staticmethod
     def backward(ctx, dout, dwavg):
         _arm()
-        q_in, q_pos, k_in, v_in, q, k, v, probs, ctxv, wv_d, wo_d, *wd_list = ctx.saved_tensors
-        B, Lq, Lk, H, E, same_qk, scale, p_attn, seed_attn, p_out, seed_out = ctx.cfg
-        dt = q_in.dtype
-        dev = q_in.device
-        defer = _can_defer(*ctx.params)
+        p_out, seed_out = ctx.cfg[-2:]
         g = ops.dropout(dout.contiguous(), p_out, seed_out) if p_out > 0 else dout.contiguous()
-        if defer:
-            dW_in = torch.empty((3 * E, E), dtype=torch.float32, device=dev)
-            db_in = torch.empty(3 * E, dtype=torch.float32, device=dev)
-        else:
-            dW_in = ops.zeros_f32((3 * E, E), dev)
-            db_in = ops.zeros_f32(3 * E, dev)
-        dW_out, db_out = _wgrad(g, ctxv.view(B * Lq, E), defer, want_bias=True)
-        dctx = ops.linear_fwd(g, wo_d).view(B, Lq, E)
-        if same_qk:
-            dqk = torch.empty((B, Lq, 2 * E), dtype=dt, device=dev)
-            dq, dk = dqk[..., :E], dqk[..., E:]
-        else:
-            dq = torch.empty((B, Lq, E), dtype=dt, device=dev)
-            dk = torch.empty((B, Lk, E), dtype=dt, device=dev)
-        dv = torch.empty((B, Lk, E), dtype=dt, device=dev)
-        dwa = dwavg.contiguous().float() if dwavg is not None else None
-        if ctx.lean:
-            ops.mha_lean_bwd(q, k, v, ctx.kp, ctxv, dctx, probs, H, scale, dq, dk, dv, dropout_p=p_attn, seed=seed_attn)
-        else:
-            ops.mha_bwd(q, k, v, dctx, probs, dwa, H, scale, dq, dk, dv, dropout_p=p_attn, seed=seed_attn)
-        dv2 = dv.view(B * Lk, E)
-        _wgrad(dv2, v_in, defer, want_bias=True, out=dW_in[2 * E :], dbias=db_in[2 * E :])
-        d_v_in = ops.linear_fwd(dv2, wv_d) if ctx.needs_input_grad[3] else None
-        d_q_in = d_k_in = None
-        need_q = ctx.needs_input_grad[0] or (q_pos is not None and ctx.needs_input_grad[1])
-        if same_qk:
-            dqk2 = dqk.view(B * Lq, 2 * E)
-            _wgrad(dqk2, q_in, defer, want_bias=True, out=dW_in[: 2 * E], dbias=db_in[: 2 * E], x2=q_pos)
-            if need_q:
-                d_q_in = ops.linear_fwd(dqk2, wd_list[0])
-        else:
-            dq2, dk2 = dq.view(B * Lq, E), dk.view(B * Lk, E)
-            _wgrad(dq2, q_in, defer, want_bias=True, out=dW_in[:E], dbias=db_in[:E], x2=q_pos)
-            _wgrad(dk2, k_in, defer, want_bias=True, out=dW_in[E : 2 * E], dbias=db_in[E : 2 * E])
-            if need_q:
-                d_q_in = ops.linear_fwd(dq2, wd_list[0])
-            if ctx.needs_input_grad[2]:
-                d_k_in = ops.linear_fwd(dk2, wd_list[1])
-        return (d_q_in if ctx.needs_input_grad[0] else None, d_q_in if (q_pos is not None and ctx.needs_input_grad[1]) else None, d_k_in, d_v_in,
-                dW_in, db_in, dW_out, db_out) + (None,) * 10
+        return _mha_backward(ctx.saved_tensors, ctx.lean, ctx.kp, ctx.cfg, ctx.params, ctx.needs_input_grad[:4], g, dwavg, None) + (None,) * 10
+
+
+def _mha_forward(q_in, q_pos, k_in, v_in, W_in, b_in, W_out, b_out, key_pad, B, Lq, Lk, H, need_w, p_attn, seed_attn, p_out, seed_out):
+    E = q_in.shape[1]
+    dt = q_in.dtype
+    same_qk = k_in is None
+    bi = b_in.detach()
+
+    def proj(x_, w_, b_):
+        return ops.linear_ex(x_, w_, b_, a2=q_pos, w_shared=True) if q_pos is not None else ops.linear_fwd(x_, w_, b_)
+
+    if same_qk:
+        wqk_f, wqk_d, _, _ = prepared(W_in[: 2 * E], dt)
+        qk = proj(q_in, wqk_f, bi[: 2 * E]).view(B, Lq, 2 * E)
+        q, k = qk[..., :E], qk[..., E:]
+        wd_list = (wqk_d,)
+    else:
+        wq_f, wq_d, _, _ = prepared(W_in[:E], dt)
+        wk_f, wk_d, _, _ = prepared(W_in[E : 2 * E], dt)
+        q = proj(q_in, wq_f, bi[:E]).view(B, Lq, E)
+        k = ops.linear_fwd(k_in, wk_f, bi[E : 2 * E]).view(B, Lk, E)
+        wd_list = (wq_d, wk_d)
+    wv_f, wv_d, _, _ = prepared(W_in[2 * E :], dt)
+    v = ops.linear_fwd(v_in, wv_f, bi[2 * E :]).view(B, Lk, E)
+    scale = 1.0 / math.sqrt(E // H)
+    lean = not need_w and ops.mha_lean_ok(q, k, v, H)
+    if lean:
+        ctxv, probs, kp = ops.mha_lean_fwd(q, k, v, key_pad, H, scale, dropout_p=p_attn, seed=seed_attn)
+        wavg = None
+    else:
+        ctxv, probs, wavg = ops.mha_fwd(q, k, v, key_pad, H, scale, need_wavg=need_w, dropout_p=p_attn, seed=seed_attn)
+        kp = None
+    wo_f, wo_d, _, _ = prepared(W_out, dt)
+    out = ops.linear_fwd(ctxv.view(B * Lq, E), wo_f, b_out.detach(), dropout_p=p_out, seed=seed_out)
+    saved = (q_in, q_pos, k_in, v_in, q, k, v, probs, ctxv, wv_d, wo_d, *wd_list)
+    cfg = (B, Lq, Lk, H, E, same_qk, scale, p_attn, seed_attn, p_out, seed_out)
+    return out, (wavg if need_w else None), saved, lean, kp, cfg
+
+
+def _mha_backward(saved, lean, kp_, cfg, params, needs, g, dwavg, accum):
+    q_in, q_pos, k_in, v_in, q, k, v, probs, ctxv, wv_d, wo_d, *wd_list = saved
+    B, Lq, Lk, H, E, same_qk, scale, p_attn, seed_attn, p_out, seed_out = cfg
+    dt = q_in.dtype
+    dev = q_in.device
+    defer = _can_defer(*params)
+    need_pos = q_pos is not None and needs[1]
+    if defer:
+        dW_in = torch.empty((3 * E, E), dtype=torch.float32, device=dev)
+        db_in = torch.empty(3 * E, dtype=torch.float32, device=dev)
+    else:
+        dW_in = ops.zeros_f32((3 * E, E), dev)
+        db_in = ops.zeros_f32(3 * E, dev)
+    dW_out, db_out = _wgrad(g, ctxv.view(B * Lq, E), defer, want_bias=True)
+    dctx = ops.linear_fwd(g, wo_d).view(B, Lq, E)
+    if same_qk:
+        dqk = torch.empty((B, Lq, 2 * E), dtype=dt, device=dev)
+        dq, dk = dqk[..., :E], dqk[..., E:]
+    else:
+        dq = torch.empty((B, Lq, E), dtype=dt, device=dev)
+        dk = torch.empty((B, Lk, E), dtype=dt, device=dev)
+    dv = torch.empty((B, Lk, E), dtype=dt, device=dev)
+    dwa = dwavg.contiguous().float() if dwavg is not None else None
+    if lean:
+        ops.mha_lean_bwd(q, k, v, kp_, ctxv, dctx, probs, H, scale, dq, dk, dv, dropout_p=p_attn, seed=seed_attn)
+    else:
+        ops.mha_bwd(q, k, v, dctx, probs, dwa, H, scale, dq, dk, dv, dropout_p=p_attn, seed=seed_attn)
+    dv2 = dv.view(B * Lk, E)
+    _wgrad(dv2, v_in, defer, want_bias=True, out=dW_in[2 * E :], dbias=db_in[2 * E :])
+    d_v_in = ops.linear_fwd(dv2, wv_d) if (needs[3] and accum is None) else None
+    d_q_in = d_k_in = None
+    need_q = needs[0] or need_pos
+    if same_qk:
+        dqk2 = dqk.view(B * Lq, 2 * E)
+        _wgrad(dqk2, q_in, defer, want_bias=True, out=dW_in[: 2 * E], dbias=db_in[: 2 * E], x2=q_pos)
+        if need_q:
+            d_q_in = ops.linear_fwd(dqk2, wd_list[0], accum=accum if not need_pos else None)
+    else:
+        dq2, dk2 = dq.view(B * Lq, E), dk.view(B * Lk, E)
+        _wgrad(dq2, q_in, defer, want_bias=True, out=dW_in[:E], dbias=db_in[:E], x2=q_pos)
+        _wgrad(dk2, k_in, defer, want_bias=True, out=dW_in[E : 2 * E], dbias=db_in[E : 2 * E])
+        if need_q:
+            d_q_in = ops.linear_fwd(dq2, wd_list[0])
+        if needs[2]:
+            d_k_in = ops.linear_fwd(dk2, wd_list[1])
+    if accum is not None:
+        assert same_qk and need_q and needs[0] and needs[3]
+        d_pos = d_q_in if need_pos else None
+        t = ops.add(accum, d_q_in) if need_pos else d_q_in
+        d_x = ops.linear_fwd(dv2, wv_d, accum=t, out=t if not need_pos else None)
+        return d_x, d_pos, None, None, dW_in, db_in, dW_out, db_out
+    return (d_q_in if needs[0] else None, d_q_in if need_pos else None, d_k_in, d_v_in, dW_in, db_in, dW_out, db_out)
 
 
 class _CrossKVShared:
diff --git a/tubedetr_amd/models/transformer.py b/tubedetr_amd/models/transformer.py
--- a/tubedetr_amd/models/transformer.py
+++ b/tubedetr_amd/models/transformer.py
@@ -42,6 +42,11 @@
         return Fk.multihead_attention(q_in, k_in, v_in, self.in_proj_weight, self.in_proj_bias, self.out_proj.weight,
                                       self.out_proj.bias, key_pad, B, Lq, Lk, self.num_heads, need_weights,
                                       attn_dropout=self.dropout, out_dropout=out_dropout, training=training, q_pos=q_pos)
+
+    def run_self_norm(self, x, norm, key_pad, B, L, need_weights, out_dropout, training, q_pos=None):
+        return Fk.self_attention_add_layernorm(x, q_pos, self.in_proj_weight, self.in_proj_bias, self.out_proj.weight, self.out_proj.bias,
+                                               norm.weight, norm.bias, key_pad, B, L, self.num_heads, norm.eps, need_weights,
+                                               attn_dropout=self.dropout, out_dropout=out_dropout, training=training)
 
 
 class TransformerEncoderLayer(nn.Module):
@@ -57,10 +62,9 @@
         self.p = dropout
 
     def forward(self, src: Tensor, pos: Optional[Tensor], key_pad: Optional[Tensor], B: int, S: int) -> Tensor:
-        a, _ = self.self_attn.run(src, None, src, key_pad, B, S, S, False, self.p, self.training, q_pos=pos)
-        src = Fk.add_layernorm(a, src, self.norm1.weight, self.norm1.bias, self.norm1.eps)
-        f = Fk.ffn(src, self.linear1.weight, self.linear1.bias, self.linear2.weight, self.linear2.bias, self.p, self.training)
-        return Fk.add_layernorm(f, src, self.norm2.weight, self.norm2.bias, self.norm2.eps)
+        src, _ = self.self_attn.run_self_norm(src, self.norm1, key_pad, B, S, False, self.p, self.training, q_pos=pos)
+        return Fk.ffn_add_layernorm(src, self.linear1.weight, self.linear1.bias, self.linear2.weight, self.linear2.bias, self.norm2.weight,
+                                    self.norm2.bias, self.norm2.eps, self.p, self.training)
 
 
 class TransformerEncoder(nn.Module):
@@ -97,10 +101,9 @@
 
     def forward(self, tgt, query_pos, mem, pos, query_mask, memory_mask, b: int, t: int, S: int, kv=None, index: int = 0):
         if self.no_tsa:
-            a, w = self.self_attn.run(tgt, None, tgt, None, b * t, 1, 1, True, self.p, self.training, q_pos=query_pos)
-        else:
-            a, w = self.self_attn.run(tgt, None, tgt, query_mask, b, t, t, True, self.p, self.training, q_pos=query_pos)
-        tgt = Fk.add_layernorm(a, tgt, self.norm1.weight, self.norm1.bias, self.norm1.eps)
+            tgt, w = self.self_attn.run_self_norm(tgt, self.norm1, None, b * t, 1, True, self.p, self.training, q_pos=query_pos)
+        else:
+            tgt, w = self.self_attn.run_self_norm(tgt, self.norm1, query_mask, b, t, True, self.p, self.training, q_pos=query_pos)
         if isinstance(kv, tuple) and len(kv) == 2:
             a, cw = self.cross_attn_image.run_q1(tgt, kv, memory_mask, b * t, S, True, self.p, self.training, q_pos=query_pos)
         elif kv is not None:
@@ -109,8 +112,8 @@
             mem_k = Fk.AddFn.apply(mem, pos) if pos is not None else mem
             a, cw = self.cross_attn_image.run(tgt, mem_k, mem, memory_mask, b * t, 1, S, True, self.p, self.training, q_pos=query_pos)
         tgt = Fk.add_layernorm(a, tgt, self.norm3.weight, self.norm3.bias, self.norm3.eps)
-        f = Fk.ffn(tgt, self.linear1.weight, self.linear1.bias, self.linear2.weight, self.linear2.bias, self.p, self.training)
-        tgt = Fk.add_layernorm(f, tgt, self.norm4.weight, self.norm4.bias, self.norm4.eps)
+        tgt = Fk.ffn_add_layernorm(tgt, self.linear1.weight, self.linear1.bias, self.linear2.weight, self.linear2.bias, self.norm4.weight,
+                                   self.norm4.bias, self.norm4.eps, self.p, self.training)
         return tgt, w, cw
 
 
diff --git a/tubedetr_amd/ops.py b/tubedetr_amd/ops.py
--- a/tubedetr_amd/ops.py
+++ b/tubedetr_amd/ops.py
@@ -95,9 +95,11 @@
     return c.data_ptr() if c is not None else None
 
 
-def _epi(bias=None, residual=None, mask_src=None, relu=False, sigmoid=False, dropout_p=0.0, seed=0, alpha=1.0) -> Epilogue:
+def _epi(bias=None, residual=None, mask_src=None, relu=False, sigmoid=False, dropout_p=0.0, seed=0, alpha=1.0, accum=None) -> Epilogue:
+    if accum is not None:
+        assert accum.dim() == 2 and accum.stride(1) == 1, "accum: row-major 2-D operand expected"
     return Epilogue(ptr(bias), ptr(residual), ptr(mask_src), int(relu), int(sigmoid), float(dropout_p), int(seed) & 0xFFFFFFFF, float(alpha),
-                    _ctr() if dropout_p > 0 else None)
+                    _ctr() if dropout_p > 0 else None, ptr(accum), accum.stride(0) if accum is not None else 0)
 
 
 def conv_gemm_raw(src: Tensor, w: Tensor, out: Tensor, desc: ConvDesc, epi: Optional[Epilogue]):
@@ -237,12 +239,12 @@
 
 
 def linear_fwd(x: Tensor, w: Tensor, bias: Optional[Tensor] = None, *, residual=None, relu=False, sigmoid=False,
-               mask_src=None, dropout_p=0.0, seed=0, alpha=1.0, out: Optional[Tensor] = None) -> Tensor:
+               mask_src=None, dropout_p=0.0, seed=0, alpha=1.0, out: Optional[Tensor] = None, accum: Optional[Tensor] = None) -> Tensor:
     M, K = x.shape
     Nn = w.shape[0]
     assert w.shape[1] == K and w.dtype == x.dtype and x.is_contiguous() and w.is_contiguous()
     y = out if out is not None else torch.empty((M, Nn), dtype=x.dtype, device=x.device)
-    conv_gemm_raw(x, w, y, _desc(1, M, 1, K, M, 1, 1, 1, 1, 0, 0, Nn, Nn), _epi(bias, residual, mask_src, relu, sigmoid, dropout_p, seed, alpha))
+    conv_gemm_raw(x, w, y, _desc(1, M, 1, K, M, 1, 1, 1, 1, 0, 0, Nn, Nn), _epi(bias, residual, mask_src, relu, sigmoid, dropout_p, seed, alpha, accum))
     return y
 
 
@@ -267,7 +269,7 @@
 def linear_ex(a1: Tensor, w: Tensor, bias: Optional[Tensor] = None, *, a2: Optional[Tensor] = None, a1_map: Optional[Tensor] = None,
               a2_map: Optional[Tensor] = None, w_shared: bool = False, out: Optional[Tensor] = None, out_map: Optional[Tensor] = None,
               out_rows: Optional[int] = None, residual: Optional[Tensor] = None, res_map: Optional[Tensor] = None, relu=False, mask_src=None,
-              dropout_p=0.0, seed=0, alpha=1.0) -> Tensor:
+              dropout_p=0.0, seed=0, alpha=1.0, accum: Optional[Tensor] = None) -> Tensor:
     _rows2d(a1)
     K1 = a1.shape[1]
     K2 = _rows2d(a2).shape[1] if a2 is not None else 0
@@ -286,7 +288,7 @@
     x.w_shared = int(bool(w_shared and a2 is not None))
     x.rows1, x.rows2 = a1.shape[0], (a2.shape[0] if a2 is not None else 0)
     x.a1_map, x.a2_map, x.out_map, x.res_map = ptr(a1_map), ptr(a2_map), ptr(out_map), ptr(res_map)
-    epi = _epi(bias, residual, mask_src, relu, False, dropout_p, seed, alpha)
+    epi = _epi(bias, residual, mask_src, relu, False, dropout_p, seed, alpha, accum)
     check(_hip.lib().td_linear_ex(ptr(a1), ptr(a2), ptr(w), ptr(out), C.byref(x), C.byref(epi), dtype_code(a1.dtype), stream_ptr()), "td_linear_ex")
     return out
 
@@ -391,14 +393,17 @@
     return y, (s if r is not None else x), mean, rstd
 
 
-def add_layernorm_bwd(dy: Tensor, s: Tensor, mean: Tensor, rstd: Tensor, gamma: Tensor, extra: Optional[Tensor] = None):
+def add_layernorm_bwd(dy: Tensor, s: Tensor, mean: Tensor, rstd: Tensor, gamma: Tensor, extra: Optional[Tensor] = None, *,
+                      drop_p: float = 0.0, drop_seed: int = 0):
     rows, cols = dy.shape
     ds = torch.empty_like(dy)
+    ds_drop = torch.empty_like(dy) if drop_p > 0 else None
     dgamma = zeros_f32(cols, dy.device)
     dbeta = zeros_f32(cols, dy.device)
     check(_hip.lib().td_add_layernorm_bwd(ptr(dy), ptr(s), ptr(mean), ptr(rstd), ptr(gamma), ptr(extra), ptr(ds), ptr(dgamma), ptr(dbeta),
+                                          ptr(ds_drop), float(drop_p), int(drop_seed) & 0xFFFFFFFF, _ctr() if drop_p > 0 else None,
                                           rows, cols, dtype_code(dy.dtype), stream_ptr()), "td_add_layernorm_bwd")
-    return ds, dgamma, dbeta
+    return (ds, dgamma, dbeta, ds_drop) if drop_p > 0 else (ds, dgamma, dbeta)
 
 
 def colsum(g: Tensor, out: Optional[Tensor] = None) -> Tensor:
```

New measurement: 107.0, median of 6. No clear change (+0.5%).
